# willake/cpu-ray-tracer

Hardware: AMD Instinct MI355X
Metric: Mrays/sec (primary+secondary), 1280x720 64spp path trace — pipelined throughput over 878 consecutive 64-spp windows of one progressive render (single_render = one such render alone) (higher is better)
Workload: dtype f32; 1 GPU; bunny_scene.xml FileScene BVH-SAH path tracer, 1280x720, 64 spp/step (passes=1, depthLimit=5); 1 step = 64 frames = the next spp window of a progressive render; the 878 steps are one crt_render job (14 render kernel launch(es), a wavefront per (tile, 128 consecutive frames), + ordered accumulate), one sync at the end; triangles=4968, parallelism=tile-wave x1

## Files before the change

### cpu-ray-tracer_amd/csrc/abi.cpp

```cpp
#include "../../include/crt_abi.h"
#include "device/launch.h"
#include "device/tile_class.h"
#include "host/grid_resolution.h"

#include <cmath>
#include <cstdarg>
#include <cstddef>
#include <cstdio>
#include <cstdlib>
#include <cstring>
#include <deque>
#include <string>
#include <algorithm>
#include <vector>
#include <chrono>

static_assert(sizeof(crt_bvh_node) == 32 && sizeof(crt_tri) == 112 && sizeof(crt_tlas_node) == 32, "reference layouts");
static_assert(sizeof(crt::NodePair) == 64 && sizeof(crt::LeafTri) == 48 && sizeof(crt::ShadeTri) == 64 && sizeof(crt::TlasNode) == 32 &&
              sizeof(crt::Instance) == 128 && sizeof(crt::Material) == 32 && offsetof(crt::Instance, T) == 64, "device layouts");
static_assert(sizeof(crt_counters) == sizeof(crt::Counters), "counter layout");
static_assert(sizeof(crt_kd_node) == 48 && sizeof(crt::KdNode) == sizeof(crt_kd_node) && sizeof(crt::AltTri) == 48, "flat KD node (uploaded as it comes), alternative accelerators' triangle record");
static_assert(offsetof(crt::PrimDev, red) == 536 && sizeof(crt::PrimDev) == 552, "PrimDev: 134 floats, then the two texel pointers");
static_assert(sizeof(crt::BlasAltDesc) == 72, "BLAS descriptor");
static_assert(sizeof(crt_shadow_ray) == 28 && sizeof(crt_ray) == 28 && sizeof(crt_hit) == 28, "query records");
// ... 887 lines not shown
    c->orderReady = c->orderCopied[k];
    return 0;
}

static uint32_t sky_to_tail(const std::vector<uint8_t>& cls, std::vector<uint32_t>& order)
{
    if (cls.size() != order.size()) return 0u;
    const auto tail = std::stable_partition(order.begin(), order.end(), [&](uint32_t i) { return cls[i] != crt::kTileSky; });
    return (uint32_t)(order.end() - tail);
}

static int update_tile_order(crt_ctx* c)
{
    if (!c->orderDirty || c->tileCount == 0) return 0;
    const crt::Scene& s = c->hScene;
    double R[3], Dn[3], N[3];
    for (int k = 0; k < 3; k++) { R[k] = (double)s.topRight[k] - s.topLeft[k]; Dn[k] = (double)s.bottomLeft[k] - s.topLeft[k]; }
    N[0] = R[1] * Dn[2] - R[2] * Dn[1]; N[1] = R[2] * Dn[0] - R[0] * Dn[2]; N[2] = R[0] * Dn[1] - R[1] * Dn[0];
    const double rr = R[0] * R[0] + R[1] * R[1] + R[2] * R[2], dd = Dn[0] * Dn[0] + Dn[1] * Dn[1] + Dn[2] * Dn[2];
    double E[3]; for (int k = 0; k < 3; k++) E[k] = (double)s.topLeft[k] - s.camPos[k];
    const double num = E[0] * N[0] + E[1] * N[1] + E[2] * N[2];
    auto rect_of = [&](const float* P8, int r[4]) -> bool {
        double u0 = 1e30, u1 = -1e30, v0 = 1e30, v1 = -1e30;
        for (int i = 0; i < 8; i++) {
            const float* P = P8 + 3 * i;
            double d[3] = {P[0] - s.camPos[0], P[1] - s.camPos[1], P[2] - s.camPos[2]};
            const double den = d[0] * N[0] + d[1] * N[1] + d[2] * N[2];
            const double t = den != 0 ? num / den : -1;
            if (!(t > 0) || rr == 0 || dd == 0) return false;
            double Q[3]; for (int k = 0; k < 3; k++) Q[k] = s.camPos[k] + t * d[k] - s.topLeft[k];
            const double u = (Q[0] * R[0] + Q[1] * R[1] + Q[2] * R[2]) / rr, v = (Q[0] * Dn[0] + Q[1] * Dn[1] + Q[2] * Dn[2]) / dd;
            if (u < u0) u0 = u; if (u > u1) u1 = u; if (v < v0) v0 = v; if (v > v1) v1 = v;
        }
        r[0] = (int)floor(u0 * c->cfg.width / 16.0) - 1; r[1] = (int)floor(u1 * c->cfg.width / 16.0) + 1;
        r[2] = (int)floor(v0 * c->cfg.height / 16.0) - 1; r[3] = (int)floor(v1 * c->cfg.height / 16.0) + 1;
        return true;
    };
    float world[24];
    for (int i = 0; i < 8; i++) { world[3 * i] = (i & 1) ? c->meshHi[0] : c->meshLo[0]; world[3 * i + 1] = (i & 2) ? c->meshHi[1] : c->meshLo[1]; world[3 * i + 2] = (i & 4) ? c->meshHi[2] : c->meshLo[2]; }
    int wr[4] = {0, c->tilesX - 1, 0, c->tilesY - 1};
    (void)rect_of(world, wr);
    std::vector<uint32_t> first, second, rest;
    for (uint32_t i = 0; i < c->tileCount; i++) {
        const uint32_t tile = c->tileFirst + i * c->tileStride;
        const int tx = (int)(tile % (uint32_t)c->tilesX), ty = (int)(tile / (uint32_t)c->tilesX);
        const bool inRect = tx >= wr[0] && tx <= wr[1] && ty >= wr[2] && ty <= wr[3];
        if (inRect) first.push_back(i); else rest.push_back(i);
    }
    for (int k = 0; k <= crt_ctx::kLatStages; k++) { c->tuneCount[k] = 0; c->tuneMs[k] = 0; }
    c->latStage = 0; c->latBest = 0; c->latDone = false; c->latWarm = false; c->latConfirming = false; c->latQueue.clear(); c->costPending = false; c->latProbed = false;
    first.insert(first.end(), rest.begin(), rest.end());
    (void)sky_to_tail(c->hostClass, first);
    c->jobCostValid = false; c->jobCostPending = false; c->planValid = false; c->skyWindowTicks = 0;
    { const int r = upload_tile_order(c, first); if (r) return r; }
    c->orderDirty = false;
    return 0;
}

static int update_tile_class(crt_ctx* c)
{
    if (!c->classDirty || c->tileCount == 0) return 0;
    if (!c->dTileClass) HIPCK(c, hipMalloc((void**)&c->dTileClass, (size_t)c->tileCount));
    { const int r = order_behind_ahead(c); if (r) return r; }
    const int k = c->classFlip ^= 1;
    if (!c->hTileClass[k]) {
        HIPCK(c, hipHostMalloc((void**)&c->hTileClass[k], (size_t)c->tileCount, hipHostMallocDefault));
        HIPCK(c, ensure_event(&c->classCopied[k]));
    } else HIPCK(c, hipEventSynchronize(c->classCopied[k]));
    crt::classify_tiles(c->hScene, c->cfg.width, c->cfg.height, (uint32_t)c->tilesX, c->tileFirst, c->tileStride, c->tileCount, c->hTileClass[k]);
    {
        const uint8_t* cls = c->hTileClass[k];
        bool same = c->hostClass.size() == c->tileCount; uint32_t sky = 0;
        for (uint32_t i = 0; i < c->tileCount; i++) { const bool s = cls[i] == crt::kTileSky; sky += s ? 1u : 0u; if (same && s != (c->hostClass[i] == crt::kTileSky)) same = false; }
        c->hostClass.assign(cls, cls + c->tileCount); c->skyTiles = sky;
        if (!same) c->orderDirty = true;
    }
    HIPCK(c, hipMemcpyAsync(c->dTileClass, c->hTileClass[k], (size_t)c->tileCount, hipMemcpyHostToDevice, c->stream));
    HIPCK(c, hipEventRecord(c->classCopied[k], c->stream));
    c->orderReady = c->classCopied[k];
    c->classDirty = false;
    return 0;
}

static size_t sample_bytes_per_window(const crt_ctx* c, uint32_t passes) { return (size_t)c->tileCount * 256u * 64u * passes * 16u; }
static size_t window_bytes(const crt_ctx* c, uint32_t passes) { return sample_bytes_per_window(c, passes) + (c->usePool ? crt_pool_scratch_bytes_per_window(c->tileCount) : 0); }

static uint32_t block_desc(uint32_t tile, uint32_t laneBase, uint32_t lanes, uint32_t window) { uint32_t lg = 0; while ((1u << lg) < lanes) lg++; return tile | (laneBase << 16) | (lg << 22) | (window << 25); }
static const uint32_t kLatLanes[7] = {64u, 32u, 16u, 8u, 4u, 2u, 1u};
static const double kLatG[7] = {1.0, 0.93, 0.88, 0.79, 0.69, 0.57, 0.48};
static int lat_index(uint32_t L) { int k = 0; while (k < 6 && kLatLanes[k] != L) k++; return k; }

static uint8_t next_lanes(uint8_t lanes, uint32_t cost, double T)
{
    int k = lat_index(lanes); const double unit = (double)cost / kLatG[k];
    while (k < 6 && unit * kLatG[k] > T) k++;
    while (k > 0 && unit * kLatG[k - 1] <= 0.9 * T) k--;
    return (uint8_t)kLatLanes[k];
}
extern "C" int crt_debug_next_lanes(const uint8_t* lanes, const uint32_t* cost, uint32_t n, double T, uint8_t* out)
{
    if (!lanes || !cost || !out) return CRT_ERR_INVALID;
    for (uint32_t i = 0; i < n; i++) { if (lanes[i] == 0 || lanes[i] > 64 || (64 % lanes[i]) != 0) return CRT_ERR_INVALID; out[i] = next_lanes(lanes[i], cost[i], T); }
    return CRT_OK;
}

static double solve_block_table(const std::vector<uint8_t>& lanes, const std::vector<uint32_t>& cost, double budget, std::vector<uint8_t>& out)
{
    const size_t n = cost.size();
    double topUnit = 0; for (size_t i = 0; i < n; i++) topUnit = std::max(topUnit, (double)cost[i] / kLatG[lat_index(lanes[i])]);
    out.assign(n, 64);
    if (topUnit <= 0) return 0;
    auto waves = [&](double T) { double w = 0; for (size_t i = 0; i < n; i++) w += 64.0 / next_lanes(lanes[i], cost[i], T); return w; };
    double lo = kLatG[6] * topUnit, hi = topUnit;
    if (waves(lo) > budget) { for (int it = 0; it < 14; it++) { const double mid = 0.5 * (lo + hi); if (waves(mid) <= budget) hi = mid; else lo = mid; } lo = hi; }
    for (size_t i = 0; i < n; i++) out[i] = next_lanes(lanes[i], cost[i], lo);
    return lo;
}
extern "C" int crt_debug_solve_block_table(const uint8_t* lanes, const uint32_t* cost, uint32_t n, double budget, uint8_t* out, double* T)
{
    if (!lanes || !cost || !out) return CRT_ERR_INVALID;
    for (uint32_t i = 0; i < n; i++) if (lanes[i] == 0 || lanes[i] > 64 || (64 % lanes[i]) != 0) return CRT_ERR_INVALID;
    std::vector<uint8_t> L; const double t = solve_block_table(std::vector<uint8_t>(lanes, lanes + n), std::vector<uint32_t>(cost, cost + n), budget, L);
    if (n) memcpy(out, L.data(), n);
    if (T) *T = t;
    return CRT_OK;
}
static double lat_budget(crt_ctx* c)
{
    if (!c->latSlots) c->latSlots = crt_render_resident_waves(c->cfg.device, c->hScene.kind, c->ldsBytes);
    double share = 0.98;
    if (const char* e = hook("CRT_LAT_BUDGET")) { const double v = atof(e); if (v > 0) share = v; }
    return share * (double)c->latSlots;
}

static int upload_block_table(crt_ctx* c, const std::vector<uint8_t>& lanes, const std::vector<uint32_t>& cost)
{
    const uint32_t n = c->tileCount;
    std::vector<uint32_t> order(n);
    for (uint32_t i = 0; i < n; i++) order[i] = i;
    std::stable_sort(order.begin(), order.end(), [&](uint32_t a, uint32_t b) { return cost[a] > cost[b]; });
    std::vector<uint32_t> table; table.reserve((size_t)n * 2);
    for (uint32_t r = 0; r < n; r++) {
        const uint32_t tl = order[r], L = lanes[tl];
        for (uint32_t base = 0; base < 64u; base += L) table.push_back(block_desc(tl, base, L, 0u));
    }
    if (table.size() > 0x7fffffffull) return c->fail(CRT_ERR_INVALID, "block table too large");
    if (hook("CRT_LAT_VERBOSE")) fprintf(stderr, "[crt] latency table: %zu wavefronts for %u tiles (slowest tile of the base stage %.2f ms)\n", table.size(), n, n ? cost[order[0]] * 1e-5 : 0.0);
    if (c->descCap < table.size()) {
        if (c->dBlockDesc) (void)hipFree(c->dBlockDesc);
        if (c->hBlockDesc) (void)hipHostFree(c->hBlockDesc);
        c->dBlockDesc = nullptr; c->hBlockDesc = nullptr; c->descCap = 0;
        const size_t cap = table.size() + table.size() / 2;
        HIPCK(c, hipMalloc((void**)&c->dBlockDesc, cap * 4));
        HIPCK(c, hipHostMalloc((void**)&c->hBlockDesc, cap * 4, hipHostMallocDefault));
        c->descCap = (uint32_t)cap;
    } else if (c->descReady) HIPCK(c, hipEventSynchronize(c->descReady));
    HIPCK(c, ensure_event(&c->descReady));
    memcpy(c->hBlockDesc, table.data(), table.size() * 4);
    { const int r = order_behind_ahead(c); if (r) return r; }
    HIPCK(c, hipMemcpyAsync(c->dBlockDesc, c->hBlockDesc, table.size() * 4, hipMemcpyHostToDevice, c->stream));
    HIPCK(c, hipEventRecord(c->descReady, c->stream));
    c->nBlocks = (uint32_t)table.size();
    return 0;
}

static int next_block_table(crt_ctx* c)
{
// ... 338 lines not shown
static PoolWavePlan plan_pool_waves(const crt_ctx* c, uint32_t windows, uint32_t frames, uint32_t head, uint32_t nSky, double skyTicks, std::vector<uint32_t>& table)
{
    PoolWavePlan p;
    PoolWaveTerms terms;
    const uint32_t S = crt_pool_streams(frames);
    if (!c->jobCostValid || c->cfg.collectStats || head + nSky >= c->tileCount || !pool_wave_terms(terms) || forced_wave_frames(S)) return p;
    const uint32_t nr = c->tileCount - nSky - head;
    p.ranks = nr;
    std::vector<uint32_t> cost(nr), wf, tab;
    double costSum = 0; for (uint32_t v : c->jobCost) costSum += (double)v;
    const double perCost = (c->poolWindowTicks > 0 && costSum > 0) ? c->poolWindowTicks / costSum : 1.0 / 4096.0;
    double startTicks = 0;
    if (sky_behind()) { terms.tailTicks = skyTicks; terms.tailWaves = (double)nSky * (double)((frames + S - 1u) / S); } else startTicks = skyTicks;
    for (uint32_t r = 0; r < head; r++) startTicks += (double)windows * 1.2 * (double)c->jobCost[c->jobOrder[r]] * perCost;
    for (uint32_t r = 0; r < nr; r++) cost[r] = c->jobCost[c->jobOrder[head + r]];
    uint32_t F1 = 0, lw = 0, blocks = 0;
    pool_wave_plan(cost.data(), nr, frames, S, perCost, startTicks, 4096u, terms, wf, &F1, nullptr, &p.aim);
    if (F1) blocks = pool_wave_table(wf, F1, S, tab, &lw);
    if (lw) {
        for (uint32_t r = 0; r < nSky; r++) { tab.push_back(blocks); tab.push_back(S); }
        p.off = (uint32_t)table.size(); p.blocks = blocks; p.longFrames = F1; p.longWaves = lw;
        table.insert(table.end(), tab.begin(), tab.end());
    }
    if (hook("CRT_LAT_VERBOSE")) {
        uint32_t cnt[4] = {0, 0, 0, 0}; double share[4] = {0, 0, 0, 0}, sum = 0;
        for (uint32_t r = 0; r < nr; r++) { int k = 0; while ((S << k) < wf[r]) k++; cnt[k]++; share[k] += cost[r]; sum += cost[r]; }
        fprintf(stderr, "[crt] pool launch of %u ranks x %u frames (%u sky ranks behind them: %.2f ms): aim %.1f ms, most expensive tile %.2f ms, long part %u frames in %u wavefronts, %u of them own more than %u frames (safety %.2f, guard %.1f x 4096, share %.2f); tiles by frames per wavefront (share of the cost):",
                nr, frames, nSky, skyTicks * 1e-5, p.aim * 1e-5, nr ? cost[0] * 1e-5 : 0.0, F1, blocks, lw, S, terms.safety, terms.guard, terms.share);
        for (int k = 0; k < 4; k++) fprintf(stderr, " %u: %u (%.3f)", S << k, cnt[k], sum > 0 ? share[k] / sum : 0.0);
        fprintf(stderr, "\n");
    }
    return p;
}

static double sky_launch_ticks(const crt_ctx* c, uint32_t windows, uint32_t nSky)
{
    return (nSky && c->jobCostValid) ? c->skyWindowTicks * (double)windows : 0.0;
}

static int install_job_plan(crt_ctx* c, uint32_t windows, uint32_t frames, bool pool)
{
    const uint32_t asked = sky_split(c, pool);
    if (c->planValid && c->planWindows == windows && c->planFrames == frames && c->planPool == pool && c->planSkyAsked == asked) return 0;
    uint32_t nSky = asked;
    double skyTicks = sky_launch_ticks(c, windows, nSky);
    std::vector<uint32_t> table; uint32_t head = 0;
    plan_job(c, windows, frames, pool, table, &head, nSky, skyTicks);
    if (head && nSky) {
        nSky = 0; skyTicks = 0;
        plan_job(c, windows, frames, pool, table, &head);
    }
    c->planValid = true; c->planWindows = windows; c->planFrames = frames; c->planPool = pool; c->planSkyAsked = asked; c->planSky = nSky; c->jobHead = head; c->jobBlocks = (uint32_t)table.size();
    c->jobTrialMs[0] = c->jobTrialMs[1] = 0;
    c->jobWaveOff = c->jobWaveBlocks = c->jobLongFrames = c->jobLongWaves = 0;
    if (pool) {
        const PoolWavePlan p = plan_pool_waves(c, windows, frames, head, nSky, skyTicks, table);
        c->jobWaveOff = p.off; c->jobWaveBlocks = p.blocks; c->jobLongFrames = p.longFrames; c->jobLongWaves = p.longWaves;
    }
    if (table.empty()) return 0;
    if (c->jobDescCap < table.size()) {
        if (c->dJobDesc) (void)hipFree(c->dJobDesc);
        if (c->hJobDesc) (void)hipHostFree(c->hJobDesc);
        c->dJobDesc = nullptr; c->hJobDesc = nullptr; c->jobDescCap = 0;
        const size_t cap = table.size() + table.size() / 2;
        HIPCK(c, hipMalloc((void**)&c->dJobDesc, cap * 4));
        HIPCK(c, hipHostMalloc((void**)&c->hJobDesc, cap * 4, hipHostMallocDefault));
        c->jobDescCap = (uint32_t)cap;
    } else if (c->jobDescReady) HIPCK(c, hipEventSynchronize(c->jobDescReady));
    HIPCK(c, ensure_event(&c->jobDescReady));
    memcpy(c->hJobDesc, table.data(), table.size() * 4);
    { const int r = order_behind_ahead(c); if (r) return r; }
    HIPCK(c, hipMemcpyAsync(c->dJobDesc, c->hJobDesc, table.size() * 4, hipMemcpyHostToDevice, c->stream));
    HIPCK(c, hipEventRecord(c->jobDescReady, c->stream));
    return 0;
}

struct Launch {
    hipStream_t st = nullptr; EventPair ev{}; void* slab = nullptr; uint32_t sppFirst = 0, nf = 0, passes = 1, windows = 1;
    const uint32_t* blockDesc = nullptr; uint32_t nBlocks = 0;
    bool wantCost = false, wantJobCost = false, pool = false;
    uint32_t head = 0, jobBlocks = 0; unsigned long long* jobClk = nullptr;
    uint32_t waveFrames = 0, waveBlocks = 0, longFrames = 0, longWaves = 0; const uint32_t* waveTab = nullptr;
    uint32_t sky = 0;
};

static int next_block_table(crt_ctx* c);
static int probe_tile_costs(crt_ctx* c, hipStream_t st);

static int tuner_prepare(crt_ctx* c, Launch& L)
{
    int r;
    const bool gpuIdle = !c->lastRenderEnd || hipEventQuery(c->lastRenderEnd) == hipSuccess;
    if (L.nf <= 64u && L.nf >= 8u && gpuIdle && !c->cfg.collectStats && c->tileCount <= 0x10000u && !hook("CRT_LAT_OFF")) {
        if (c->costPending && hipEventQuery(c->costCopied) == hipSuccess) { c->costPending = false; harvest_tuning(c); if ((r = next_block_table(c))) return r; }
        if (c->latStage == 0 && !c->latProbed && !c->latWarm && !c->costPending && L.nf == 64u && !hook("CRT_LAT_POLICY") && !hook("CRT_LAT_NO_PROBE")) { if ((r = probe_tile_costs(c, L.st))) return r; }
        const int stage = c->latStage;
        if (stage || c->latProbed) { L.blockDesc = c->dBlockDesc; L.nBlocks = c->nBlocks; HIPCK(c, hipStreamWaitEvent(L.st, c->descReady, 0)); }
        L.wantCost = (!c->latDone && !c->costPending) || (c->latDone && hook("CRT_LAT_RECORD"));
        c->evRender.back().mode = c->latDone ? -1 : stage;
        if (L.wantCost && !c->latDone) c->costStage = stage;
    }
    if (L.wantCost) {
        if (!c->dTileCost) {
            HIPCK(c, hipMalloc((void**)&c->dTileCost, (size_t)c->tileCount * 4));
            HIPCK(c, hipHostMalloc((void**)&c->hTileCost, (size_t)c->tileCount * 4, hipHostMallocDefault));
            HIPCK(c, ensure_event(&c->costCopied));
        }
        else HIPCK(c, hipStreamWaitEvent(L.st, c->costCopied, 0));
        HIPCK(c, hipMemsetAsync(c->dTileCost, 0, (size_t)c->tileCount * 4, L.st));
    }
    return 0;
}

static int planner_prepare(crt_ctx* c, Launch& L)
{
    int r;
    if (L.nf > 64u && !c->cfg.collectStats) {
        if (c->jobCostPending && hipEventQuery(c->jobCostCopied) == hipSuccess) { c->jobCostPending = false; if ((r = adopt_job_costs(c))) return r; HIPCK(c, hipStreamWaitEvent(L.st, c->orderReady, 0)); }
        L.wantJobCost = !c->jobCostValid && !c->jobCostPending && L.nf >= 128u;
        if (L.wantJobCost) {
            if (!c->dJobCost) {
                HIPCK(c, hipMalloc((void**)&c->dJobCost, job_cost_bytes(c)));
                HIPCK(c, hipHostMalloc((void**)&c->hJobCost, job_cost_bytes(c), hipHostMallocDefault));
                HIPCK(c, ensure_event(&c->jobCostCopied));
            } else HIPCK(c, hipStreamWaitEvent(L.st, c->jobCostCopied, 0));
            HIPCK(c, hipMemsetAsync(c->dJobCost, 0, job_cost_bytes(c), L.st));
        }
    }
    const bool poolByDefault = c->hScene.poolRefBits == 16u || c->poolMinWaves == 0;
    const uint64_t minWaves = c->poolMinWaves != 65000u ? c->poolMinWaves : (c->jobCostValid ? 43000u : 65000u);
    L.pool = c->usePool && poolByDefault && pool_can_run(c, L.nf) && (uint64_t)c->tileCount * L.windows >= minWaves && (c->poolMinWaves == 0 || L.nf > 64u);
    L.sky = sky_split(c, L.pool);
    if (L.nf > 64u && c->jobCostValid) {
        if ((r = install_job_plan(c, L.windows, L.nf, L.pool))) return r;
        int use = 1;
        if ((c->jobBlocks || c->jobLongWaves) && !hook("CRT_PLAN_NO_TRIAL")) {
            if (c->jobTrialMs[1] > 0 && c->jobTrialMs[0] > 0) use = c->jobTrialMs[1] <= c->jobTrialMs[0] ? 1 : 0;
            else if (c->jobTrialMs[1] > 0 && c->jobTrialMs[0] == 0) use = 0;
            c->evRender.back().mode = 100 + use;
        }
        if (use) L.sky = c->planSky;
        if (use) { L.head = c->jobHead; L.jobBlocks = c->jobBlocks; if (L.pool && c->jobLongWaves) { L.waveTab = c->dJobDesc + c->jobWaveOff; L.waveBlocks = c->jobWaveBlocks; L.longFrames = c->jobLongFrames; L.longWaves = c->jobLongWaves; } }
    }
    if (L.pool) if (const uint32_t S = crt_pool_streams(L.nf); const uint32_t n = forced_wave_frames(S)) {
        L.waveFrames = n; L.waveTab = nullptr; L.waveBlocks = 0;
        L.longWaves = n > S ? (c->tileCount - L.sky - L.head) * (L.nf / n + ((L.nf % n) > S ? 1u : 0u)) : 0u;
    }
    if (L.jobBlocks || L.waveTab) HIPCK(c, hipStreamWaitEvent(L.st, c->jobDescReady, 0));
    if (L.wantJobCost) {
        L.jobClk = reinterpret_cast<unsigned long long*>(reinterpret_cast<char*>(c->dJobCost) + job_cost_clk_offset(c));
        c->recPool = L.pool; c->recWindows = L.windows;
        const uint32_t perWave = L.pool ? std::max(crt_pool_streams(L.nf), L.waveFrames) : 64u;
        c->recWaves = L.pool ? (c->tileCount - L.sky) * ((L.nf + perWave - 1u) / perWave) : c->tileCount * L.windows;
        c->recResident = L.pool ? 4096u : 5120u;
        if (L.pool && c->hScene.poolRefBits == 32u)
            c->recResident = 256u * std::min(16u, (160u * 1024u) / std::max(1u, pool_lds_need(c, L.nf)));
    }
    return 0;
}

static hipError_t launch_render_kernels(crt_ctx* c, const Launch& L)
{
    hipStream_t st = L.st;
    hipError_t le = hipSuccess;
    auto join = [&](hipStream_t other) -> hipError_t {
        if (other == st) return hipSuccess;
        hipError_t e = hipSuccess;
        if (c->splitEvents.size() < 32) { hipEvent_t ne; e = hipEventCreateWithFlags(&ne, hipEventDisableTiming); if (e == hipSuccess) c->splitEvents.push_back(ne); }
        if (e == hipSuccess) { hipEvent_t je = c->splitEvents[c->splitSeq++ % c->splitEvents.size()]; e = hipEventRecord(je, other); if (e == hipSuccess) e = hipStreamWaitEvent(st, je, 0); }
        return e;
    };
    auto launch_table = [&](const uint32_t* desc, uint32_t nBlocks, uint32_t* cost) -> hipError_t {
        return crt_launch_render(&c->hScene, L.slab, c->dCounters, c->dTileClocks, c->dTileOrder, c->tileFirst, c->tileStride, c->tileCount, (uint32_t)c->tilesX,
                                 L.sppFirst, L.nf, L.passes, c->ldsBytes, 0, desc, nBlocks, cost, 0u, nullptr, st);
    };
    if (L.pool) {
        void* scratch = (char*)L.slab + (size_t)L.windows * sample_bytes_per_window(c, L.passes);
        hipStream_t st2 = st;
        const bool skyBehind = sky_behind();
        auto launch_sky = [&](hipStream_t s) -> hipError_t {
            return crt_launch_render_sky(&c->hScene, L.slab, c->dCounters, c->dTileOrder, c->tileCount - L.sky, L.sky, c->tileFirst, c->tileStride, c->tileCount, (uint32_t)c->tilesX,
                                         L.sppFirst, L.nf, L.passes, L.jobClk ? L.jobClk + 3 : nullptr, s);
        };
        if (L.sky && !skyBehind) { le = launch_sky(st); if (le == hipSuccess) c->skyLaunches++; }
        if (le != hipSuccess) return le;
        if (L.jobBlocks) {
            le = launch_table(c->dJobDesc, L.jobBlocks, nullptr);
            st2 = c->streams[(size_t)(c->launchSeq++ % c->streams.size())];
            if (le == hipSuccess && st2 != st) le = hipStreamWaitEvent(st2, L.ev.a, 0);
        }
        if (le == hipSuccess)
            le = crt_launch_render_pool(&c->hScene, L.slab, scratch, c->dCounters, c->dTileClocks, c->dTileOrder, c->tileFirst, c->tileStride, c->tileCount, (uint32_t)c->tilesX,
                                        L.sppFirst, L.nf, L.passes, c->cfg.collectStats, L.jobBlocks ? L.head : 0u, c->tileCount - L.sky, L.waveFrames, L.waveTab, L.waveBlocks, L.longFrames,
                                        L.wantJobCost ? c->dJobCost : nullptr, L.jobClk,
                                        (c->classDirty || hook("CRT_DEBUG_NO_TILE_CLASS")) ? nullptr : c->dTileClass , c->extraLds, st2);
        if (le == hipSuccess) c->lastLongWaves = L.longWaves;
        if (L.jobBlocks && le == hipSuccess) le = join(st2);
        if (L.sky && skyBehind && le == hipSuccess) {
            if (!c->skyStream && !hook("CRT_SKY_PRIORITY")) {
                int least = 0, greatest = 0;
                le = hipDeviceGetStreamPriorityRange(&least, &greatest);
                if (le == hipSuccess) le = hipStreamCreateWithPriority(&c->skyStream, hipStreamNonBlocking, least);
                if (le != hipSuccess) return le;
            }
            hipStream_t st3 = c->skyStream;
            if (hook("CRT_SKY_PRIORITY")) { st3 = c->streams[(size_t)(c->launchSeq++ % c->streams.size())]; if (st3 == st2 && c->streams.size() > 1) st3 = c->streams[(size_t)(c->launchSeq++ % c->streams.size())]; }
            if (st3 != st) le = hipStreamWaitEvent(st3, L.ev.a, 0);
            if (le == hipSuccess) le = launch_sky(st3);
            if (le == hipSuccess) { c->skyLaunches++; le = join(st3); }
        }
    } else if (L.jobBlocks) {
        le = launch_table(c->dJobDesc, L.jobBlocks, nullptr);
    } else if (L.blockDesc && L.nBlocks) {
        le = launch_table(L.blockDesc, L.nBlocks, L.wantCost ? c->dTileCost : nullptr);
    } else {
        le = crt_launch_render(&c->hScene, L.slab, c->dCounters, c->dTileClocks, c->dTileOrder, c->tileFirst, c->tileStride, c->tileCount, (uint32_t)c->tilesX,
                               L.sppFirst, L.nf, L.passes, c->ldsBytes, c->cfg.collectStats, nullptr, 0u,
                               L.wantCost ? c->dTileCost : (L.wantJobCost ? c->dJobCost : nullptr), 0u, L.jobClk, st);
    }
    if (L.jobBlocks && le == hipSuccess) c->splitLaunches++;
    return le;
}

static int probe_tile_costs(crt_ctx* c, hipStream_t st)
{
    const uint32_t n = c->tileCount;
    if (!c->dTileCost) {
        HIPCK(c, hipMalloc((void**)&c->dTileCost, (size_t)n * 4));
        HIPCK(c, hipHostMalloc((void**)&c->hTileCost, (size_t)n * 4, hipHostMallocDefault));
        HIPCK(c, ensure_event(&c->costCopied));
    } else HIPCK(c, hipEventSynchronize(c->costCopied));
    const auto tp0 = std::chrono::steady_clock::now();
    HIPCK(c, crt_launch_probe(&c->hScene, c->tileFirst, c->tileStride, n, (uint32_t)c->tilesX, c->dTileCost, st));
    HIPCK(c, hipMemcpyAsync(c->hTileCost, c->dTileCost, (size_t)n * 4, hipMemcpyDeviceToHost, st));
    HIPCK(c, hipEventRecord(c->costCopied, st));
    HIPCK(c, hipStreamSynchronize(st));
    const auto tp1 = std::chrono::steady_clock::now();
    std::vector<uint32_t>& est = c->latCost[0]; est.assign(c->hTileCost, c->hTileCost + n);
    for (uint32_t i = 0; i < n; i++) est[i] += 18u * crt_probe_paths();
    std::vector<uint8_t>& L = c->latL[0]; L.assign(n, 64);
    solve_block_table(std::vector<uint8_t>(n, 64), est, lat_budget(c), L);
    c->latProbed = true;
    bool any = false; for (uint32_t i = 0; i < n; i++) any = any || L[i] != 64;
    if (!any) { c->latProbed = false; return 0; }
    const auto tp2 = std::chrono::steady_clock::now();
    const int r = upload_block_table(c, L, est);
    if (hook("CRT_LAT_VERBOSE")) { const auto tp3 = std::chrono::steady_clock::now(); auto ms = [](auto a, auto b) { return std::chrono::duration<double, std::milli>(b - a).count(); };
        fprintf(stderr, "[crt] cost probe: launch + wait %.3f ms, table solved in %.3f ms, uploaded in %.3f ms\n", ms(tp0, tp1), ms(tp1, tp2), ms(tp2, tp3)); }
    return r;
}

static int launch_frames(crt_ctx* c, uint32_t sppFirst, uint32_t nf, uint32_t passes, hipStream_t st, crt_ctx::Ahead* ahead)
{
    const size_t windowBytes = window_bytes(c, passes);
    size_t off = 0; int r;
    if ((r = take_region(c, (size_t)((nf + 63u) / 64u) * windowBytes, st, &off))) return r;
    if (c->orderReady) HIPCK(c, hipStreamWaitEvent(st, c->orderReady, 0));
    if ((r = wait_scene(c, st))) return r;
    void* slab = c->pool + off;
    EventPair ev;
    harvest_tuning(c);
    fold_completed(c, c->evRender, &c->foldedRenderMs, &c->foldedLaunches); fold_completed(c, c->evAcc, &c->foldedAccMs, nullptr);
    if ((r = take_event(c, c->evRender, &ev))) return r;
    struct PairGuard { crt_ctx* c; bool armed; ~PairGuard() { if (armed && !c->evRender.empty()) { c->evPool.push_back(c->evRender.back()); c->evRender.pop_back(); } } } pairGuard{c, true};
    Launch L; L.st = st; L.ev = ev; L.slab = slab; L.sppFirst = sppFirst; L.nf = nf; L.passes = passes; L.windows = (nf + 63u) / 64u;
    if ((r = tuner_prepare(c, L))) return r;
    if ((r = planner_prepare(c, L))) return r;
    HIPCK(c, hipEventRecord(ev.a, st));
    const bool pool = L.pool, wantCost = L.wantCost, wantJobCost = L.wantJobCost;
    const hipError_t le = hook("CRT_DEBUG_FAIL_LAUNCH") ? hipErrorInvalidConfiguration  : launch_render_kernels(c, L);
    if (le != hipSuccess) {
        return c->hip(le, pool ? "launch of render_pool_kernel" : "launch of render_tiles_kernel");
    }
    if (pool && L.sky < c->tileCount) c->poolLaunches++;
    HIPCK(c, hipEventRecord(ev.b, st));
    pairGuard.armed = false;
    c->lastRenderEnd = ev.b;
    if (wantJobCost) {
        HIPCK(c, hipMemcpyAsync(c->hJobCost, c->dJobCost, job_cost_bytes(c), hipMemcpyDeviceToHost, st));
        HIPCK(c, hipEventRecord(c->jobCostCopied, st));
        c->jobCostPending = true;
    }
    if (wantCost && !pool && !c->latDone) {
        HIPCK(c, hipMemcpyAsync(c->hTileCost, c->dTileCost, (size_t)c->tileCount * 4, hipMemcpyDeviceToHost, st));
        HIPCK(c, hipEventRecord(c->costCopied, st));
        c->costPending = true;
    }
    crt_ctx::Region reg; reg.off = off; reg.bytes = (size_t)((nf + 63u) / 64u) * windowBytes;
    if (c->freeEvents.empty()) HIPCK(c, hipEventCreateWithFlags(&reg.freed, hipEventDisableTiming));
    else { reg.freed = c->freeEvents.back(); c->freeEvents.pop_back(); }
    if (ahead) {
        hipEvent_t end = nullptr;
        if (c->doneEvents.empty()) { const hipError_t e = hipEventCreateWithFlags(&end, hipEventDisableTiming); if (e != hipSuccess) { c->freeEvents.push_back(reg.freed); return c->hip(e, "hipEventCreate"); } }
        else { end = c->doneEvents.back(); c->doneEvents.pop_back(); }
        const hipError_t e = hipEventRecord(end, st);
        if (e != hipSuccess) { c->doneEvents.push_back(end); c->freeEvents.push_back(reg.freed); return c->hip(e, "hipEventRecord"); }
        reg.held = true;
        c->inflight.push_back(reg);
        *ahead = crt_ctx::Ahead{end, off, (const char*)slab, c->epoch, sppFirst, nf, passes, 0u};
        return 0;
    }
    HIPCK(c, hipStreamWaitEvent(c->stream, ev.b, 0));
    if ((r = take_event(c, c->evAcc, &ev))) return r;
    HIPCK(c, hipEventRecord(ev.a, c->stream));
    HIPCK(c, crt_launch_accumulate(slab, c->dAcc, c->tileFirst, c->tileStride, c->tileCount, (uint32_t)c->tilesX, (uint32_t)c->cfg.width, nf, passes, c->stream));
    HIPCK(c, hipEventRecord(ev.b, c->stream));
    HIPCK(c, hipEventRecord(reg.freed, c->stream));
    c->inflight.push_back(reg);
    return 0;
}

int crt_render(crt_ctx* c, uint32_t spp_first, uint32_t frames, uint32_t passes)
{
    if (!c) return CRT_ERR_INVALID;
    if (!c->haveScene && !c->havePrim) return c->fail(CRT_ERR_STATE, "crt_render before crt_upload_scene");
    if (passes < 1 || passes > 4) return c->fail(CRT_ERR_INVALID, "passes must be 1..4 (the reference's UI range, renderer.cpp:178)");
    HIPCK(c, hipSetDevice(c->cfg.device));
    { int r = discard_ahead(c); if (r) return r; }
    if (c->tileCount == 0 || frames == 0) return CRT_OK;
    { int r = update_tile_class(c); if (r) return r; }
    { int r = update_tile_order(c); if (r) return r; }
    if (c->streams.empty()) {
        int n = c->cfg.renderStreams;
        if (n <= 0) n = 7;
        if (n > 16) n = 16;
        if (c->cfg.collectStats) n = 1;
        c->streams.resize((size_t)n);
        for (auto& st : c->streams) HIPCK(c, hipStreamCreateWithFlags(&st, hipStreamNonBlocking));
    }
    uint32_t maxF = 0;
    { int r = ensure_pool(c, frames, passes, &maxF); if (r) return r; }
    const size_t windowBytes = window_bytes(c, passes);
    if (c->renderAccel != 0 || c->havePrim) {
        for (uint32_t f0 = 0; f0 < frames; f0 += maxF) {
            const uint32_t nf = (frames - f0 < maxF) ? frames - f0 : maxF;
            size_t off = 0; int r;
            if ((r = take_region(c, (size_t)((nf + 63u) / 64u) * windowBytes, c->stream, &off))) return r;
            if ((r = wait_scene(c, c->stream))) return r;
            void* slab = c->pool + off;
            if (c->havePrim) HIPCK(c, crt_launch_render_prim(&c->hScene, &c->prim, slab, c->dCounters, c->tileFirst, c->tileStride, c->tileCount, (uint32_t)c->tilesX, spp_first + f0 * passes, nf, passes, c->stream));
            else HIPCK(c, crt_launch_render_alt(c->renderAccel, &c->hScene, &c->alt, &c->blasAlt[c->renderAccel - 1], slab, c->dCounters, c->tileFirst, c->tileStride, c->tileCount, (uint32_t)c->tilesX, spp_first + f0 * passes, nf, passes, c->stream));
            HIPCK(c, crt_launch_accumulate(slab, c->dAcc, c->tileFirst, c->tileStride, c->tileCount, (uint32_t)c->tilesX, (uint32_t)c->cfg.width, nf, passes, c->stream));
            crt_ctx::Region reg; reg.off = off; reg.bytes = (size_t)((nf + 63u) / 64u) * windowBytes;
            if (c->freeEvents.empty()) HIPCK(c, hipEventCreateWithFlags(&reg.freed, hipEventDisableTiming));
            else { reg.freed = c->freeEvents.back(); c->freeEvents.pop_back(); }
            HIPCK(c, hipEventRecord(reg.freed, c->stream));
            c->inflight.push_back(reg);
        }
        return CRT_OK;
    }
    for (uint32_t f0 = 0; f0 < frames; f0 += maxF) {
        const uint32_t nf = (frames - f0 < maxF) ? frames - f0 : maxF;
        const int r = launch_frames(c, spp_first + f0 * passes, nf, passes, c->streams[(size_t)(c->launchSeq++ % c->streams.size())], nullptr);
        if (r) return r > 0 ? c->fail(CRT_ERR_DEVICE, "slab ring blocked by a render-ahead region") : r;
    }
    return CRT_OK;
}

int crt_sync(crt_ctx* c)
{
    if (!c) return CRT_ERR_INVALID;
    HIPCK(c, hipSetDevice(c->cfg.device));
    HIPCK(c, hipStreamSynchronize(c->stream));
    for (auto st : c->streams) HIPCK(c, hipStreamSynchronize(st));
    if (c->aheadStream) HIPCK(c, hipStreamSynchronize(c->aheadStream));
    return CRT_OK;
}

int crt_clear(crt_ctx* c)
{
    if (!c) return CRT_ERR_INVALID;
    HIPCK(c, hipSetDevice(c->cfg.device));
    HIPCK(c, hipMemsetAsync(c->dAcc, 0, (size_t)c->cfg.width * c->cfg.height * 16, c->stream));
    return CRT_OK;
}

int crt_read_accumulator(crt_ctx* c, float* host)
{
    if (!c || !host) return CRT_ERR_INVALID;
    HIPCK(c, hipSetDevice(c->cfg.device));
    HIPCK(c, hipMemcpyAsync(host, c->dAcc, (size_t)c->cfg.width * c->cfg.height * 16, hipMemcpyDeviceToHost, c->stream));
    HIPCK(c, hipStreamSynchronize(c->stream));
    return CRT_OK;
}

static int read_screen(crt_ctx* c, uint32_t* hostPixels, float* energy)
{
    const int tiles = c->tilesX * c->tilesY;
    if (hostPixels) HIPCK(c, hipMemcpyAsync(hostPixels, c->dPixels, (size_t)c->cfg.width * c->cfg.height * 4, hipMemcpyDeviceToHost, c->stream));
    std::vector<float> sums(tiles);
    HIPCK(c, hipMemcpyAsync(sums.data(), c->dTileSums, (size_t)tiles * 4, hipMemcpyDeviceToHost, c->stream));
    HIPCK(c, hipStreamSynchronize(c->stream));
    if (energy) { float e = 0; for (int i = 0; i < tiles; i++) e += sums[i]; *energy = e; }
    return CRT_OK;
}

int crt_resolve_screen(crt_ctx* c, float scale, uint32_t* hostPixels, float* energy)
{
    if (!c) return CRT_ERR_INVALID;
    HIPCK(c, hipSetDevice(c->cfg.device));
    HIPCK(c, crt_launch_resolve(c->dAcc, c->dPixels, c->dTileSums, c->tileFirst, c->tileStride, c->tileCount, (uint32_t)c->tilesX, (uint32_t)c->cfg.width, scale, c->stream));
    return read_screen(c, hostPixels, energy);
}

static constexpr uint32_t kAheadMaxFrames = 256;

static int launch_ahead(crt_ctx* c, uint32_t sppFirst, uint32_t passes)
{
    if (!c->aheadStream) {
        int least = 0, greatest = 0;
        HIPCK(c, hipDeviceGetStreamPriorityRange(&least, &greatest));
        HIPCK(c, hipStreamCreateWithPriority(&c->aheadStream, hipStreamNonBlocking, least));
    }
    uint32_t nf = c->aheadFrames ? std::min(2u * c->aheadFrames, kAheadMaxFrames) : 64u;
    if (nf > (uint32_t)c->cfg.maxFramesPerLaunch) nf = (uint32_t)c->cfg.maxFramesPerLaunch;
    const uint32_t poolW = (uint32_t)(c->poolBytes / window_bytes(c, passes));
    if (nf > poolW / 2u * 64u) nf = poolW / 2u * 64u;
    if (nf == 0 || c->streams.empty()) return 0;
    hipStream_t st = hook("CRT_AHEAD_NORMAL_PRIORITY") ? c->streams[(size_t)(c->launchSeq++ % c->streams.size())] : c->aheadStream;
    crt_ctx::Ahead a{};
    const int r = launch_frames(c, sppFirst, nf, passes, st, &a);
    if (r < 0) return r;
    if (r > 0) return 0;
    c->ahead.push_back(a); c->aheadFrames = nf;
    return 0;
// ... 1088 lines not shown
    return CRT_OK;
}

static int device_probe(crt_ctx* c, int op, const void* in, void* out, uint32_t n)
{
    static const uint8_t words[18][2] = {{1, 1}, {1, 1}, {2, 1}, {1, 1}, {2, 1}, {6, 7}, {1, 18}, {4, 1}, {5, 3}, {13, 2}, {16, 4}, {2, 2}, {2, 2}, {2, 2}, {2, 2}, {4, 2}, {2, 1}, {5, 3}};
    if (!c || !in || !out || op < 0 || op > 17 || n > (1u << 25)) return CRT_ERR_INVALID;
    if (n == 0) return CRT_OK;
    const size_t inBytes = (size_t)n * words[op][0] * 4, outBytes = (size_t)n * words[op][1] * 4;
    HIPCK(c, hipSetDevice(c->cfg.device));
    char* d = nullptr;
    HIPCK(c, hipMalloc((void**)&d, inBytes + outBytes));
    hipError_t e = hipMemcpyAsync(d, in, inBytes, hipMemcpyHostToDevice, c->stream);
    if (e == hipSuccess) e = (op <= 10 || op == 17) ? crt_launch_probe_f32(op, d, d + inBytes, n, c->stream) : crt_launch_probe_f64(op, d, d + inBytes, n, c->stream);
    if (e == hipSuccess) e = hipMemcpyAsync(out, d + inBytes, outBytes, hipMemcpyDeviceToHost, c->stream);
    if (e == hipSuccess) e = hipStreamSynchronize(c->stream);
    (void)hipFree(d);
    HIPCK(c, e);
    return CRT_OK;
}
extern "C" int crt_debug_device_probe(crt_ctx* c, int op, const void* in, void* out, uint32_t n) { return (op > 16) ? CRT_ERR_INVALID : device_probe(c, op, in, out, n); }
extern "C" int crt_debug_sky_probe(crt_ctx* c, const void* in, void* out, uint32_t n) { return device_probe(c, 17, in, out, n); }

extern "C" int crt_debug_plan_job(const uint32_t* cost, uint32_t n, uint32_t windows, uint32_t frames, int pool, double poolWindowTicks,
                                  uint32_t* table, uint32_t tableCap, uint32_t* head, uint32_t* order)
{
    if (!cost || !n || !table || !head || !order) return CRT_ERR_INVALID;
    crt_ctx c;
    c.tileCount = n; c.jobCostValid = true; c.poolWindowTicks = poolWindowTicks;
    c.streams.assign(2, nullptr);
    c.jobCost.assign(cost, cost + n);
    c.jobOrder.resize(n);
    for (uint32_t i = 0; i < n; i++) c.jobOrder[i] = i;
    std::stable_sort(c.jobOrder.begin(), c.jobOrder.end(), [&](uint32_t a, uint32_t b) { return c.jobCost[a] > c.jobCost[b]; });
    std::vector<uint32_t> t; uint32_t h = 0;
    plan_job(&c, windows, frames, pool != 0, t, &h);
    c.streams.clear();
    if (t.size() > tableCap) return CRT_ERR_INVALID;
    memcpy(table, t.data(), t.size() * 4); memcpy(order, c.jobOrder.data(), (size_t)n * 4); *head = h;
    return (int)t.size();
}

extern "C" long long crt_debug_pool_wave_plan(const uint32_t* cost, uint32_t nr, uint32_t frames, double perCost, double startTicks, uint32_t resident, double safety, double guard,
                                              double share, uint32_t* wf, uint32_t* longFrames, double* start, double* aim)
{
    if (!nr || !frames || !wf || !longFrames) return CRT_ERR_INVALID;
    PoolWaveTerms tm; if (safety > 0) tm.safety = safety; if (guard > 0) tm.guard = guard; if (share > 0) tm.share = share;
    std::vector<uint32_t> w; std::vector<double> st;
    const uint64_t waves = pool_wave_plan(cost, nr, frames, crt_pool_streams(frames), perCost, startTicks, resident, tm, w, longFrames, &st, aim);
    memcpy(wf, w.data(), (size_t)nr * 4);
    if (start) memcpy(start, st.data(), (size_t)nr * 8);
    return (long long)waves;
}
extern "C" int crt_debug_sky_split(const uint32_t* cost, const uint8_t* cls, uint32_t n, uint32_t windows, uint32_t frames, double poolWindowTicks, double skyWindowTicks,
                                   uint32_t* order, uint32_t* skyFirst, uint32_t* head, uint32_t* planRanks, uint32_t* waveTab, uint32_t* tabBlocks, uint32_t* longFrames)
{
    if (!cls || !n || !order || !skyFirst || !head || !planRanks || !waveTab || !tabBlocks || !longFrames) return CRT_ERR_INVALID;
    crt_ctx c;
    c.tileCount = n; c.poolWindowTicks = poolWindowTicks; c.skyWindowTicks = skyWindowTicks;
    c.hostClass.assign(cls, cls + n);
    *head = *planRanks = *tabBlocks = *longFrames = 0;
    if (!cost) {
        c.jobOrder.resize(n); for (uint32_t i = 0; i < n; i++) c.jobOrder[i] = i;
        c.skyTiles = sky_to_tail(c.hostClass, c.jobOrder);
    } else {
        c.jobCost.assign(cost, cost + n); c.jobCostValid = true;
        c.skyTiles = job_order(c.jobCost, c.hostClass, c.jobOrder);
        c.streams.assign(2, nullptr);
        const double skyTicks = c.skyTiles ? skyWindowTicks * (double)windows : 0.0;
        std::vector<uint32_t> table;
        plan_job(&c, windows, frames, true, table, head, c.skyTiles, skyTicks);
        table.clear();
        const PoolWavePlan p = plan_pool_waves(&c, windows, frames, *head, c.skyTiles, skyTicks, table);
        c.streams.clear();
        *planRanks = p.ranks; *tabBlocks = p.blocks; *longFrames = p.longFrames;
        if (table.size() > 2u * (size_t)n) return CRT_ERR_INVALID;
        memcpy(waveTab, table.data(), table.size() * 4);
    }
    memcpy(order, c.jobOrder.data(), (size_t)n * 4);
    *skyFirst = n - c.skyTiles;
    return (int)c.skyTiles;
}
extern "C" int crt_debug_sky_launches(crt_ctx* c) { return c ? (int)c->skyLaunches : -1; }
extern "C" int crt_debug_job_costs(crt_ctx* c, uint32_t* out, double* poolWindowTicks, double* skyWindowTicks)
{
    if (!c || !out) return CRT_ERR_INVALID;
    if (!c->jobCostValid || c->jobCost.size() != c->tileCount) return CRT_ERR_STATE;
    memcpy(out, c->jobCost.data(), (size_t)c->tileCount * 4);
    if (poolWindowTicks) *poolWindowTicks = c->poolWindowTicks;
    if (skyWindowTicks) *skyWindowTicks = c->skyWindowTicks;
    return CRT_OK;
}
extern "C" int crt_debug_pool_long_waves(crt_ctx* c) { return c ? (int)c->lastLongWaves : -1; }
extern "C" void crt_debug_pool_wave_terms(double* out) { const PoolWaveTerms tm; out[0] = tm.poolLong; out[1] = tm.load; out[2] = tm.safety; out[3] = tm.guard; out[4] = tm.share; }

extern "C" int crt_debug_tile_costs(crt_ctx* c, uint32_t* out)
{
    if (!c || !out || !c->dTileCost) return CRT_ERR_INVALID;
    HIPCK(c, hipSetDevice(c->cfg.device));
    HIPCK(c, hipDeviceSynchronize());
    HIPCK(c, hipMemcpy(out, c->dTileCost, (size_t)c->tileCount * 4, hipMemcpyDeviceToHost));
    return CRT_OK;
}

extern "C" int crt_debug_lat_stage(crt_ctx* c, int stage, uint8_t* lanes, uint32_t* cost)
{
    if (!c || stage < 0 || stage > crt_ctx::kLatStages) return CRT_ERR_INVALID;
    if (c->latL[stage].size() != c->tileCount || c->latCost[stage].size() != c->tileCount) return CRT_ERR_STATE;
    if (lanes) memcpy(lanes, c->latL[stage].data(), c->tileCount);
    if (cost) memcpy(cost, c->latCost[stage].data(), (size_t)c->tileCount * 4);
    return c->latStage;
}

extern "C" int crt_debug_tile_stamps(crt_ctx* c, uint64_t* out)
{
    if (!c || !out || !c->dTileClocks) return CRT_ERR_INVALID;
    HIPCK(c, hipSetDevice(c->cfg.device));
    HIPCK(c, hipMemcpyAsync(out, c->dTileClocks + 2 * (size_t)c->tileCount, (size_t)c->tileCount * 128, hipMemcpyDeviceToHost, c->stream));
    HIPCK(c, hipStreamSynchronize(c->stream));
    return CRT_OK;
}

int crt_bind_accumulator(crt_ctx* c, void* p)
{
    if (!c) return CRT_ERR_INVALID;
    if (p && ((uintptr_t)p & 15u)) return c->fail(CRT_ERR_INVALID, "accumulator pointer must be 16-byte aligned");
    HIPCK(c, hipSetDevice(c->cfg.device));
    HIPCK(c, hipStreamSynchronize(c->stream));
    c->dAcc = p ? p : c->dAccOwned;
    return CRT_OK;
}

int crt_accumulator_device_ptr(crt_ctx* c, void** p)
{
    if (!c || !p) return CRT_ERR_INVALID;
    *p = c->dAcc; return CRT_OK;
}

}
```

### cpu-ray-tracer_amd/csrc/device/kernels.hip

```cpp
#include "alt_common.h"
#include "launch.h"
#include "sample_body.h"

namespace crt {

#ifndef CRT_SHADE_BATCH
#define CRT_SHADE_BATCH 24
#endif
#ifndef CRT_SHADE_BATCH_JOB
#define CRT_SHADE_BATCH_JOB 40
#endif
#ifndef CRT_TRI_BATCH
#define CRT_TRI_BATCH 1
#endif
#ifndef CRT_NODE_BATCH
#define CRT_NODE_BATCH 1
#endif

#ifndef CRT_TILES_NODE_STEPS
#define CRT_TILES_NODE_STEPS 2
#endif
#ifndef CRT_MIN_WAVES
#define CRT_MIN_WAVES 5
#endif
template <int KIND, bool COUNT>
__global__ __launch_bounds__(64, CRT_MIN_WAVES) void render_tiles_kernel(const Scene sc, float4* __restrict__ slab,
                                                           Counters* __restrict__ counters, unsigned long long* __restrict__ tileClocks,
                                                           const uint32_t* __restrict__ tileOrder,
                                                           uint32_t tileFirst, uint32_t tileStride, uint32_t tileCount, uint32_t tilesX,
                                                           uint32_t sppFirst, uint32_t frames, uint32_t passes, uint32_t windows,
                                                           const uint32_t* __restrict__ blockDesc, uint32_t* __restrict__ tileCost, uint32_t rankCount, unsigned long long* __restrict__ launchClk)
{
    extern __shared__ uint32_t lds[];
    const uint32_t lane = threadIdx.x;
    const unsigned long long clk0 = (COUNT || tileCost) ? wall_clock64() : 0ull;
    if (launchClk && lane == 0) { atomicMax(&launchClk[0], ~clk0); atomicMax(&launchClk[1], clk0); }
    uint32_t rank, win = 0u, laneBase = 0u, myLanes = 64u;
    if (blockDesc) { const uint32_t d = blockDesc[blockIdx.x]; rank = d & 0xffffu; laneBase = (d >> 16) & 63u; myLanes = 1u << ((d >> 22) & 7u); win = d >> 25; }
    else { rank = blockIdx.x / windows; win = blockIdx.x - rank * windows; }
    if (rank >= (blockDesc ? tileCount : rankCount)) return;
    const uint32_t tl = blockDesc ? rank : (tileOrder ? tileOrder[rank] : rank);
    sppFirst += win * 64u * passes;
    frames = (frames - win * 64u < 64u) ? frames - win * 64u : 64u;
    if (blockDesc) frames = frames > laneBase ? ((frames - laneBase < myLanes) ? frames - laneBase : myLanes) : 0u;
    slab += (size_t)win * ((size_t)tileCount * 256u * 64u * passes);
    const uint32_t tile = tileFirst + tl * tileStride;
    const uint32_t tx = tile % tilesX, ty = tile / tilesX;
    uint32_t* stk = lds + lane;
    const char* __restrict__ geom = sc.geom;

    Cnt cn; cn.rays = cn.primary = cn.interior = cn.leaf = cn.tri = cn.tlas = cn.visits = cn.meshhits = 0;
    uint32_t trips = 0;
    const bool narrowWave = myLanes < 64u;
    const int shadeBatch = narrowWave ? (int)((myLanes * 3u + 7u) / 8u) : (windows >= 8u ? CRT_SHADE_BATCH_JOB : CRT_SHADE_BATCH);
#ifdef CRT_STAMPS
    unsigned long long stT[6] = {0, 0, 0, 0, 0, 0}; uint32_t stN[4] = {0, 0, 0, 0}; uint32_t stL[4] = {0, 0, 0, 0};
#define CRT_STAMP(var) unsigned long long var; asm volatile("s_memtime %0\n\ts_waitcnt lgkmcnt(0)" : "=s"(var) :: "memory")
#else
#define CRT_STAMP(var)
#endif
    const uint32_t items = 256u * passes;
    const f3 nil3 = mk3(0.0f, 0.0f, 0.0f);

    bool live = lane < frames;
    uint64_t liveMask = __builtin_amdgcn_ballot_w64(live);
    uint32_t seed = init_seed(tx + ty * (uint32_t)sc.W + (sppFirst + (laneBase + lane) * passes) * 1799u);
    uint32_t item = 0;
    f3 O = nil3, D = nil3, rD = nil3; bool inside = false; int depth = 0;
    Hit h; h.t = 1e34f; h.u = 0; h.v = 0; h.objIdx = -1; h.triIdx = -1;
    float* fst = reinterpret_cast<float*>(lds + sc.stackDepth * 64u + lane);
    uint32_t cur = kRefDone, sp = 0;
    f3 tO = nil3, tD = nil3, trD = nil3;
    bool rayFinite = true;
    bool fresh = true;
    rec4 q0 = {0, 0, 0, 0}, q1 = q0, q2 = q0, q3 = q0;

#define CRT_TOP() (stk[(sp ? sp - 1u : 0u) * 64u])
    auto record_offsets = [&](bool shade, uint32_t& oa, uint32_t& ob) {
        oa = shade ? sc.shadeOff + (uint32_t)h.triIdx * 64u : (cur & kRefOffsetMask) << 4; ob = oa + 32u;
        if (KIND == 1 && !shade && (cur & kRefTlasBit) != 0u) {
            if (cur & kRefInterior) { oa = sc.instOff + (cur & 0xffffu) * 128u; ob = oa + 32u; }
            else { oa = sc.tlasOff + (cur & 0x7fffu) * 32u; ob = sc.tlasOff + ((cur >> 15) & 0x7fffu) * 32u; }
        }
    };
    auto leave_blas = [&](uint32_t next) -> uint32_t {
        if (KIND == 1 && next == kRefReturn) {
            tO = O; tD = D; trD = rD; rayFinite = finite3(rD);
            const bool pop = sp != 0u; const uint32_t top = CRT_TOP();
            next = pop ? top : kRefDone; sp -= pop ? 1u : 0u;
        }
        return next;
    };

    for (;;) {
        const uint64_t mDone = __builtin_amdgcn_ballot_w64(cur == kRefDone) & liveMask;
        const uint64_t mNode = __builtin_amdgcn_ballot_w64(KIND == 1 ? (((cur >> 31) ^ (cur >> 30)) & 1u) != 0u : (cur & 0xC0000000u) == kRefInterior) & liveMask;
        const uint64_t mTri = __builtin_amdgcn_ballot_w64(cur != kRefDone && (cur & 0xC0000000u) == 0u) & liveMask;
        const uint64_t mTlas = (KIND == 1) ? (__builtin_amdgcn_ballot_w64((cur & 0xC0000000u) == kRefTlasLeaf) & liveMask) : 0ull;
        const bool isDone = live && cur == kRefDone;
        const bool isNode = live && (KIND == 1 ? (((cur >> 31) ^ (cur >> 30)) & 1u) != 0u : (cur & 0xC0000000u) == kRefInterior);
        const bool isTri = live && cur != kRefDone && (cur & 0xC0000000u) == 0u;
        const bool isTlas = (KIND == 1) && live && (cur & 0xC0000000u) == kRefTlasLeaf;
        const int nDone = __popcll(mDone), nNode = __popcll(mNode), nTri = __popcll(mTri);
        const int nTlas = (KIND == 1) ? __popcll(mTlas) : 0;
        if (nDone + nNode + nTri + nTlas == 0) break;
        if (COUNT) trips++;
        const bool bigNode = nNode >= CRT_NODE_BATCH, bigTri = nTri >= CRT_TRI_BATCH, bigShade = nDone >= shadeBatch;
        const bool none = !bigNode && !bigTri && !bigShade && nTlas == 0;
        const bool runTlas = nTlas > 0;
        const bool runNode = bigNode || (none && nNode > 0 && nNode >= nTri && nNode >= nDone);
        const bool runTri = bigTri || (none && nTri > 0 && nTri > nNode && nTri >= nDone);
        const bool runShade = bigShade || (none && nDone > 0 && nDone > nNode && nDone > nTri);
        asm volatile("" : "+v"(q0), "+v"(q1), "+v"(q2), "+v"(q3));
#ifdef CRT_STAMPS
        CRT_STAMP(s0);
        asm volatile("s_waitcnt vmcnt(0)" ::: "memory");
        CRT_STAMP(s1);
        stT[0] += s1 - s0;
        if (runShade) { stN[0]++; stL[0] += nDone; } if (runNode) { stN[1]++; stL[1] += nNode; } if (runTri) { stN[2]++; stL[2] += nTri; }
        stN[3]++;
#endif

        if (runShade && isDone) {
            const kernarg_f cam = scene_floats(offsetof(Scene, camPos));
            const f3 camPos = mk3(cam[0], cam[1], cam[2]);
            const bool first = fresh;
            const bool miss = !first && h.objIdx == -1;
            const bool stop = !first && h.objIdx != -1 && (depth >= sc.depthLimit || h.objIdx == 0);
            const bool surf = !first && !miss && !stop;
            if (!first && h.objIdx >= 2) cn.meshhits++;
            const kernarg_f sk = scene_floats(offsetof(Scene, skyOffset));
            float tu = 0, tv = 0; uint32_t tOff = asu(sk[0]); int tW = (int)asu(sk[1]), tH = (int)asu(sk[2]);
            f3 I = O, N = O, absorb = O; float refl = 0, refr = 0;
            if (miss) {
                const float phi = crt_atan2f(-D.z, D.x) + CRT_PI, theta = crt_acosf(-D.y);
                tu = phi * CRT_INV2PI; tv = theta * CRT_INVPI;
            }
            if (surf) {
                I = O + h.t * D;
                SurfPoint p;
                if (h.objIdx == 1) {
                    const kernarg_f fl = scene_floats(offsetof(Scene, floorN));
                    const kernarg_f fm = scene_floats(offsetof(Scene, floorMat));
                    const rec4 m0 = {fm[0], fm[1], fm[2], fm[3]}, m1 = {fm[4], fm[5], fm[6], fm[7]};
                    p = floor_point(mk3(fl[0], fl[1], fl[2]), fl[4], m0, m1, I);
                } else p = mesh_point<KIND>(q0, q1, q2, q3, h.u, h.v, h.objIdx, geom, sc.instOff, sc.mats);
                N = face_ray(p.N, D);
                tu = p.tu; tv = p.tv; refl = p.refl; refr = p.refr; absorb = p.absorb; tOff = p.tOff; tW = p.tW; tH = p.tH;
            }
            f3 c = mk3(1.0f, 1.0f, 1.0f);
            if (miss || (surf && tW > 0)) c = tex_sample(sc, tOff, tW, tH, tu, tv);
            f3 v = O, medium = O; bool norm = false, newInside = false; Branch branch = kMirror;
            if (surf) {
                medium = medium_of(inside, absorb, h.t);
                const Bounce b = draw_bounce(seed, D, N, inside, refl, refr);
                v = b.v; branch = b.branch; newInside = b.newInside; norm = b.branch == kDiffuse;
            }
            bool gen = first;
            if (miss || stop) {
                f3 L = miss ? c : ((depth >= sc.depthLimit) ? mk3(0, 0, 0) : mk3(24, 24, 22));
                sample_unwind(fst, depth, L);
                uint32_t pix = item, pass = 0;
                if (passes != 1u) { pix = item / passes; pass = item - pix * passes; }
                slab[((size_t)tl * 256u + pix) * (64u * passes) + ((laneBase + lane) * passes + pass)] = make_float4(L.x, L.y, L.z, 0.0f);
                item++;
                gen = true;
                if (item >= items) { live = false; gen = false; }
            }
            if (gen) {
                const uint32_t pix = (passes == 1u) ? item : item / passes;
                const f3 TL = mk3(cam[3], cam[4], cam[5]), TR = mk3(cam[6], cam[7], cam[8]), BL = mk3(cam[9], cam[10], cam[11]);
                v = primary_target(camPos, TL, TR - TL, BL - TL, cam[12], cam[13], tx, ty, pix, seed); norm = true;
                inside = false; depth = 0; fresh = false;
                cn.primary++;
            }
            if (live) {
                const float inv = rcp_exact(sqrt_exact(dot3(v, v)));
                const f3 nv = norm ? v * inv : v;
                if (surf) {
                    const f3 factor = bounce_factor(branch, c, medium, nv, N);
                    float* fd = fst + depth * 192;
                    fd[0] = factor.x; fd[64] = factor.y; fd[128] = factor.z;
                    depth++;
                    O = I + nv * CRT_EPS; inside = newInside;
                } else O = camPos;
                D = nv; rD = rcp_exact3(nv);
                cn.rays++;
                h.t = 1e34f; h.u = 0; h.v = 0; h.objIdx = -1; h.triIdx = -1;
                hit_light_floor(light_floor_from_kernarg<false>(), O, D, h);
                tO = O; tD = D; trD = rD; rayFinite = finite3(rD);
                sp = 0;
                if (sc.rootIsPair) {
                    const kernarg_f rp = scene_floats(offsetof(Scene, rootPair));
                    const rec4 a0 = {rp[0], rp[1], rp[2], rp[3]}, a1 = {rp[4], rp[5], rp[6], rp[7]};
                    const rec4 b0 = {rp[8], rp[9], rp[10], rp[11]}, b1 = {rp[12], rp[13], rp[14], rp[15]};
                    float d1, d2;
                    if (__builtin_amdgcn_ballot_w64(!rayFinite) == 0ull) { d1 = box_fast(a0, a1, O, rD, h.t); d2 = box_fast(b0, b1, O, rD, h.t); }
                    else { d1 = box_exact(a0, a1, O, rD, h.t); d2 = box_exact(b0, b1, O, rD, h.t); }
                    const Ordered o = ordered_step(d1, d2, asu(a0.w), asu(b0.w));
                    stk[0] = o.farRef;
                    sp = o.push ? 1u : 0u;
                    cur = o.hitN ? o.nearRef : kRefDone;
                    if (COUNT) { if (KIND == 0) cn.interior++; else cn.tlas++; }
                } else cur = sc.rootRef;
                if (COUNT && KIND == 0 && (cur & 0xC0000000u) == 0u && cur != kRefDone) cn.leaf++;
            }
        }
        if (runShade) liveMask = __builtin_amdgcn_ballot_w64(live);
#ifdef CRT_STAMPS
        CRT_STAMP(s2); stT[1] += s2 - s1;
#endif
        if (KIND == 1 && runTlas && isTlas) {
            if (COUNT) { cn.tlas++; cn.visits++; }
            to_object_space(q0, q1, q2, O, D, tO, tD, trD);
            rayFinite = finite3(trD);
            stk[sp * 64u] = kRefReturn; sp++;
            const uint32_t next = asu(q3.z);
            if (COUNT && (next & 0xC0000000u) == 0u && next != kRefDone) cn.leaf++;
            cur = next;
        }
#ifdef CRT_STAMPS
        CRT_STAMP(s3);
#endif
        if (runNode) {
            const bool allFinite = __builtin_amdgcn_ballot_w64(isNode && !rayFinite) == 0ull;
            if (isNode) {
                if (COUNT) { if (KIND == 1 && (cur & kRefTlasBit) != 0u) cn.tlas++; else cn.interior++; }
                uint32_t top = CRT_TOP();
                float d1, d2;
                if (allFinite) { d1 = box_fast(q0, q1, tO, trD, h.t); d2 = box_fast(q2, q3, tO, trD, h.t); }
                else { d1 = box_exact(q0, q1, tO, trD, h.t); d2 = box_exact(q2, q3, tO, trD, h.t); }
                const Ordered o = ordered_step(d1, d2, asu(q0.w), asu(q2.w));
                stk[sp * 64u] = o.farRef;
                bool pop = !o.hitN && sp != 0u;
                uint32_t next = o.hitN ? o.nearRef : (pop ? top : kRefDone);
                sp = sp + (o.push ? 1u : 0u) - (pop ? 1u : 0u);
                next = leave_blas(next);
                if (COUNT && (next & 0xC0000000u) == 0u && next != kRefDone) cn.leaf++;
                cur = next;
            }
        }
        bool triNow = isTri;
#if CRT_TILES_NODE_STEPS > 1
        if (runNode) {
            const bool node2 = isNode && (KIND == 1 ? (((cur >> 31) ^ (cur >> 30)) & 1u) != 0u : (cur & 0xC0000000u) == kRefInterior);
            const bool leaf2 = isNode && cur != kRefDone && (cur & 0xC0000000u) == 0u;
            const uint64_t mNode2 = __builtin_amdgcn_ballot_w64(node2);
            if (mNode2 != 0ull) {
                if (node2 || leaf2) {
                    uint32_t oa, ob; record_offsets(false, oa, ob);
                    q0 = ldg(geom, oa); q1 = ldg(geom, oa + 16u); q2 = ldg(geom, ob); q3 = ldg(geom, ob + 16u);
                }
                triNow = isTri || leaf2;
                const bool allFinite2 = __builtin_amdgcn_ballot_w64(node2 && !rayFinite) == 0ull;
                if (node2) {
                    if (COUNT) { if (KIND == 1 && (cur & kRefTlasBit) != 0u) cn.tlas++; else cn.interior++; }
                    uint32_t top = CRT_TOP();
                    float d1, d2;
                    if (allFinite2) { d1 = box_fast(q0, q1, tO, trD, h.t); d2 = box_fast(q2, q3, tO, trD, h.t); }
                    else { d1 = box_exact(q0, q1, tO, trD, h.t); d2 = box_exact(q2, q3, tO, trD, h.t); }
                    const Ordered o = ordered_step(d1, d2, asu(q0.w), asu(q2.w));
                    stk[sp * 64u] = o.farRef;
                    bool pop = !o.hitN && sp != 0u;
                    uint32_t next = o.hitN ? o.nearRef : (pop ? top : kRefDone);
                    sp = sp + (o.push ? 1u : 0u) - (pop ? 1u : 0u);
                    next = leave_blas(next);
                    if (COUNT && (next & 0xC0000000u) == 0u && next != kRefDone) cn.leaf++;
                    cur = next;
                }
            }
        }
#endif
#ifdef CRT_STAMPS
        CRT_STAMP(s4); stT[2] += s4 - s3;
#endif
        if ((runTri || triNow != isTri) && triNow) {
            if (COUNT) cn.tri++;
            uint32_t top = CRT_TOP();
            hit_tri(q0, q1, q2, tO, tD, h);
            const bool more = asu(q2.w) > 1u;
            bool pop = !more && sp != 0u;
            uint32_t next = more ? cur + 3u : (pop ? top : kRefDone);
            sp -= pop ? 1u : 0u;
            next = leave_blas(next);
            if (COUNT && !more && (next & 0xC0000000u) == 0u && next != kRefDone) cn.leaf++;
            cur = next;
        }
#ifdef CRT_STAMPS
        CRT_STAMP(s5); stT[3] += s5 - s4;
#endif
        {
            const bool doneNow = cur == kRefDone;
            uint32_t oa, ob; record_offsets(doneNow, oa, ob);
            const bool nothing = !live || (doneNow && h.objIdx < 2);
            if (nothing) { oa = 0u; ob = 32u; }
            if (__builtin_amdgcn_ballot_w64(!nothing) != 0ull) { q0 = ldg(geom, oa); q1 = ldg(geom, oa + 16u); q2 = ldg(geom, ob); q3 = ldg(geom, ob + 16u); }
        }
#ifdef CRT_STAMPS
        CRT_STAMP(s6); stT[4] += s6 - s5; stT[5] += s6 - s0;
#endif
    }
#undef CRT_TOP

    if (tileCost && lane == 0) atomicMax(&tileCost[tl], (uint32_t)(wall_clock64() - clk0));
    if (launchClk && lane == 0) { const unsigned long long now = wall_clock64(), last = __hip_atomic_load(&launchClk[1], __ATOMIC_RELAXED, __HIP_MEMORY_SCOPE_AGENT), from = last > clk0 ? last : clk0; if (now > from) atomicAdd(&launchClk[2], now - from); }
    if (COUNT && tileClocks && lane == 0 && windows == 1u) {
        tileClocks[2 * tl] = wall_clock64() - clk0;
        tileClocks[2 * tl + 1] = trips;
#ifdef CRT_STAMPS
        unsigned long long* dbg = tileClocks + 2 * (size_t)tileCount + 16 * (size_t)tl;
        for (int i = 0; i < 6; i++) dbg[i] = stT[i];
        for (int i = 0; i < 4; i++) dbg[6 + i] = stN[i];
        for (int i = 0; i < 4; i++) dbg[10 + i] = stL[i];
#endif
    }
    uint32_t vals[8] = {cn.rays, cn.primary, cn.interior, cn.leaf, cn.tri, cn.tlas, cn.visits, cn.meshhits};
#pragma unroll
    for (int i = 0; i < 8; i++) {
        if (!COUNT && i >= 2 && i != 7) continue;
        uint32_t s = wave_sum(vals[i]);
        if (lane == 0 && s) atomicAdd(&counters->v[i], (unsigned long long)s);
    }
}

constexpr uint32_t kAccRowF4 = 65u;
constexpr uint32_t kAccWaveLds = 16u * kAccRowF4 * 16u;
__global__ __launch_bounds__(256) void accumulate_kernel(const float4* __restrict__ slab, float* __restrict__ acc,
                                                          uint32_t tileFirst, uint32_t tileStride, uint32_t tileCount, uint32_t tilesX,
                                                          uint32_t W, uint32_t frames, uint32_t passes)
{
    extern __shared__ float4 accLds[];
    const uint32_t tl = blockIdx.x, lane = threadIdx.x & 63u, wave = threadIdx.x >> 6;
    if (tl >= tileCount) return;
    const uint32_t tile = tileFirst + tl * tileStride;
    const uint32_t x0 = (tile % tilesX) * 16u, y0 = (tile / tilesX) * 16u;
    const uint32_t rowLen = 64u * passes;
    const size_t winStride = (size_t)tileCount * 256u * rowLen;
    float4* my4 = accLds + wave * (16u * kAccRowF4);
    const float* myF = reinterpret_cast<const float*>(my4) + (lane >> 2) * (kAccRowF4 * 4u) + (lane & 3u);
    for (uint32_t r = 0; r < 4u; r++) {
        const uint32_t v = wave * 4u + r;
        float* __restrict__ ap = acc + ((size_t)(x0 + (size_t)(y0 + v) * W)) * 4u + lane;
        float a = *ap;
        const float4* __restrict__ rowBase = slab + ((size_t)tl * 256u + v * 16u) * rowLen;
        for (uint32_t f0 = 0; f0 < frames; f0 += 64u, rowBase += winStride) {
            const uint32_t S = ((frames - f0 < 64u) ? frames - f0 : 64u) * passes;
            for (uint32_t b = 0; b < S; b += 64u) {
                const uint32_t n = (S - b < 64u) ? S - b : 64u;
                float4 t[16];
                if (lane < n) {
#pragma unroll
                    for (int j = 0; j < 16; j++) t[j] = rowBase[(size_t)j * rowLen + b + lane];
#pragma unroll
                    for (int j = 0; j < 16; j++) my4[j * kAccRowF4 + lane] = t[j];
                }
                asm volatile("s_waitcnt lgkmcnt(0)" ::: "memory");
                uint32_t s = 0;
                for (; s + 8u <= n; s += 8u) {
                    float x[8];
#pragma unroll
                    for (int k = 0; k < 8; k++) x[k] = myF[(s + k) * 4u];
#pragma unroll
                    for (int k = 0; k < 8; k++) a += x[k];
                }
                for (; s < n; s++) a += myF[s * 4u];
                asm volatile("s_waitcnt lgkmcnt(0)" ::: "memory");
            }
        }
        *ap = a;
    }
}

struct RayIn { float O[3]; float D[3]; int32_t inside; };
struct HitOut { float t, u, v; int32_t objIdx, triIdx, traversed, tested; };
constexpr uint32_t kQueryRefill = 16u;

__global__ __launch_bounds__(64) void find_nearest_kernel(const Scene sc, const RayIn* __restrict__ rays,
                                                           HitOut* __restrict__ hits, uint32_t n, Counters* __restrict__ counters, uint32_t* __restrict__ cursor)
{
    extern __shared__ uint32_t lds[];
    const uint32_t lane = threadIdx.x;
    const char* __restrict__ g = sc.geom;
    uint32_t* stk = lds + lane;
    uint32_t* tstk = stk + sc.bvhStack * 64;
    Cnt cn; cn.rays = cn.primary = cn.interior = cn.leaf = cn.tri = cn.tlas = cn.visits = cn.meshhits = 0;
    uint32_t mode = 0u;
    uint32_t idx = 0; f3 O = mk3(0, 0, 0), D = O, rD = O, Oo = O, Do = O, rDo = O;
    Hit h; h.t = 1e34f; h.u = 0; h.v = 0; h.objIdx = -1; h.triIdx = -1;
    int traversed = 0, tested = 0;
    uint32_t cur = 0, sp = 0, tcur = 0, tsp = 0, leafAt = 0;
    bool more = true;
    for (;;) {
        const uint64_t mIdle = __builtin_amdgcn_ballot_w64(mode == 0u);
        const uint32_t nIdle = (uint32_t)__popcll(mIdle);
        if (more && nIdle >= kQueryRefill) {
            uint32_t base = 0;
            if (lane == 0) base = atomicAdd(cursor, nIdle);
            base = (uint32_t)__builtin_amdgcn_readfirstlane((int)base);
            more = base + nIdle < n;
            const uint32_t my = base + (uint32_t)__builtin_amdgcn_mbcnt_hi((uint32_t)(mIdle >> 32), __builtin_amdgcn_mbcnt_lo((uint32_t)mIdle, 0u));
            if (mode == 0u && my < n) {
                idx = my;
                const RayIn r = rays[idx];
                O = mk3(r.O[0], r.O[1], r.O[2]); D = mk3(r.D[0], r.D[1], r.D[2]);
                rD = mk3(1 / D.x, 1 / D.y, 1 / D.z);
                h.t = 1e34f; h.u = 0; h.v = 0; h.objIdx = -1; h.triIdx = -1; traversed = 0; tested = 0;
                cn.rays++;
                hit_light_floor(sc, O, D, h);
                if (sc.kind == 0) { Oo = O; Do = D; rDo = rD; cur = sc.rootRef; sp = 0; mode = 1u; }
                else { tcur = sc.rootRef; tsp = 0; mode = 3u; }
            }
        }
        if (__builtin_amdgcn_ballot_w64(mode != 0u) == 0ull) break;
        if (mode == 3u) {
            traversed++; cn.tlas++;
            bool pop = false;
            if ((tcur & kRefTlasLeaf) == kRefTlasLeaf) {
                cn.visits++;
                const uint32_t io = sc.instOff + (tcur & 0xffffu) * 128u;
                const rec4 r0 = ldg(g, io), r1 = ldg(g, io + 16), r2 = ldg(g, io + 32), ids = ldg(g, io + 48);
                to_object_space(r0, r1, r2, O, D, Oo, Do, rDo);
                cur = asu(ids.z); sp = 0; mode = 1u;
            } else {
                const uint32_t o1 = sc.tlasOff + (tcur & 0x7fffu) * 32u, o2 = sc.tlasOff + ((tcur >> 15) & 0x7fffu) * 32u;
                const rec4 alo = ldg(g, o1), ahi = ldg(g, o1 + 16), blo = ldg(g, o2), bhi = ldg(g, o2 + 16);
                float d1 = box_exact(alo, ahi, O, rD, h.t), d2 = box_exact(blo, bhi, O, rD, h.t);
                uint32_t r1 = asu(alo.w), r2 = asu(blo.w);
                if (d1 > d2) { float td = d1; d1 = d2; d2 = td; uint32_t tr = r1; r1 = r2; r2 = tr; }
                if (d1 == 1e30f) pop = true;
                else { tcur = r1; if (d2 != 1e30f) { tstk[tsp * 64] = r2; tsp++; } }
            }
            if (pop) { if (tsp == 0) mode = 4u; else tcur = tstk[(--tsp) * 64]; }
        }
        bool back = false;
        if (mode == 1u) {
            traversed++;
            const uint32_t off = (cur & kRefOffsetMask) << 4;
            if (cur & kRefInterior) {
                cn.interior++;
                const rec4 alo = ldg(g, off), ahi = ldg(g, off + 16), blo = ldg(g, off + 32), bhi = ldg(g, off + 48);
                float d1 = box_exact(alo, ahi, Oo, rDo, h.t), d2 = box_exact(blo, bhi, Oo, rDo, h.t);
                uint32_t r1 = asu(alo.w), r2 = asu(blo.w);
                if (d1 > d2) { float td = d1; d1 = d2; d2 = td; uint32_t tr = r1; r1 = r2; r2 = tr; }
                if (d1 == 1e30f) back = true;
                else { cur = r1; if (d2 != 1e30f) { stk[sp * 64] = r2; sp++; } }
            } else { cn.leaf++; leafAt = off; mode = 2u; }
        }
        if (mode == 2u) {
            const rec4 a = ldg(g, leafAt), b = ldg(g, leafAt + 16), c = ldg(g, leafAt + 32);
            tested++; cn.tri++;
            hit_tri(a, b, c, Oo, Do, h);
            if (asu(c.w) <= 1u) { back = true; mode = 1u; } else leafAt += 48;
// ... 357 lines not shown
            hit_light_floor(sc, O, D, h);
            alt_walk<ACCEL>(sc, alt, O, D, rD, h, stk, traversed, tested);
            if (h.objIdx >= 2) cn.meshhits++;
        }
        travOut[idx] = traversed; testedOut[idx] = tested;
        if (h.objIdx == -1) {
            const f3 res = sky_color(sc, D);
            acc[idx] = make_float4(res.x, res.y, res.z, 0.0f);
            const uint32_t r = (uint32_t)(255.0f * min_std(1.0f, res.x)), g = (uint32_t)(255.0f * min_std(1.0f, res.y)), bb = (uint32_t)(255.0f * min_std(1.0f, res.z));
            pixels[idx] = (r << 16) + (g << 8) + bb;
        } else pixels[idx] = kInspectPending;
    }
    uint32_t vals[8] = {cn.rays, cn.primary, cn.interior, cn.leaf, cn.tri, cn.tlas, cn.visits, cn.meshhits};
#pragma unroll
    for (int k = 0; k < 8; k++) {
        uint32_t s = wave_sum(vals[k]);
        if (lane == 0 && s) atomicAdd(&counters->v[k], (unsigned long long)s);
    }
    inspect_reduce(lane, traversed, tested, sums);
    const int32_t m = wave_max(useTested ? tested : traversed);
    if (lane == 0 && m) atomicMax(&blockMax[idx / kInspectBlock], m);
}

__device__ __forceinline__ f3 traverse_count_color(int32_t traversed, int32_t peak)
{
    const float invMax = 1 / 255.f;
    const f3 green = mk3(179 * invMax, 255 * invMax, 174 * invMax);
    const f3 red = mk3(255 * invMax, 50 * invMax, 50 * invMax);
    if (peak < 10) return green;
    traversed = traversed < 0 ? 0 : (traversed > peak ? peak : traversed);
    const float blend = traversed / (float)peak;
    return mk3(green.x + blend * (red.x - green.x), green.y + blend * (red.y - green.y), green.z + blend * (red.z - green.z));
}

__global__ __launch_bounds__(1024) void inspect_color_kernel(const int32_t* __restrict__ count, const int32_t* __restrict__ blockMax, int32_t peakIn, uint32_t n,
                                                             float4* __restrict__ acc, uint32_t* __restrict__ pixels)
{
    __shared__ int32_t carryPart[16], waveMax[16];
    const uint32_t tid = threadIdx.x, lane = tid & 63u, wave = tid >> 6;
    const uint32_t idx = blockIdx.x * kInspectBlock + tid;
    int32_t c = peakIn;
    for (uint32_t j = tid; j < blockIdx.x; j += kInspectBlock) { const int32_t t = blockMax[j]; c = t > c ? t : c; }
    c = wave_max(c);
    const int32_t own = idx < n ? count[idx] : 0;
    int32_t incl = own;
    for (int o = 1; o < 64; o <<= 1) { const int32_t t = __shfl_up(incl, o, 64); if (lane >= (uint32_t)o && t > incl) incl = t; }
    if (lane == 0) carryPart[wave] = c;
    if (lane == 63) waveMax[wave] = incl;
    __syncthreads();
    int32_t peak = carryPart[0];
#pragma unroll
    for (uint32_t w = 1; w < 16; w++) { const int32_t t = carryPart[w]; peak = t > peak ? t : peak; }
    for (uint32_t w = 0; w < wave; w++) { const int32_t t = waveMax[w]; peak = t > peak ? t : peak; }
    const int32_t before = __shfl_up(incl, 1, 64);
    if (lane > 0 && before > peak) peak = before;
    if (idx < n && pixels[idx] == kInspectPending) {
        const f3 res = traverse_count_color(own, peak);
        acc[idx] = make_float4(res.x, res.y, res.z, 0.0f);
        const uint32_t r = (uint32_t)(255.0f * min_std(1.0f, res.x)), g = (uint32_t)(255.0f * min_std(1.0f, res.y)), bb = (uint32_t)(255.0f * min_std(1.0f, res.z));
        pixels[idx] = (r << 16) + (g << 8) + bb;
    }
}

__global__ __launch_bounds__(64) void resolve_kernel(const float4* __restrict__ acc, uint32_t* __restrict__ pixels, float* __restrict__ tileSums,
                                                      uint32_t tileFirst, uint32_t tileStride, uint32_t tileCount, uint32_t tilesX,
                                                      uint32_t W, float scale)
{
    const uint32_t tl = blockIdx.x * blockDim.x + threadIdx.x;
    if (tl >= tileCount) return;
    const uint32_t tile = tileFirst + tl * tileStride;
    const uint32_t x0 = (tile % tilesX) * 16u, y0 = (tile / tilesX) * 16u;
    float sum = 0;
    for (uint32_t v = 0; v < 16; v++) for (uint32_t u = 0; u < 16; u++) {
        const size_t i = (x0 + u) + (size_t)(y0 + v) * W;
        const float4 a = acc[i];
        const float px = a.x * scale, py = a.y * scale, pz = a.z * scale;
        sum += px + py + pz;
        const uint32_t r = (uint32_t)(255.0f * min_std(1.0f, px)), g = (uint32_t)(255.0f * min_std(1.0f, py)), bb = (uint32_t)(255.0f * min_std(1.0f, pz));
        pixels[i] = (r << 16) + (g << 8) + bb;
    }
    tileSums[tile] = sum;
}

__global__ __launch_bounds__(256) void commit_frame_kernel(const float4* __restrict__ slabWindow, uint32_t frameInWindow, uint32_t passes,
                                                            float4* __restrict__ acc, uint32_t* __restrict__ pixels, float* __restrict__ tileSums,
                                                            uint32_t tileFirst, uint32_t tileStride, uint32_t tileCount, uint32_t tilesX,
                                                            uint32_t W, float scale)
{
    __shared__ float tileE[256];
    const uint32_t tl = blockIdx.x, pix = threadIdx.x;
    if (tl >= tileCount) return;
    const uint32_t tile = tileFirst + tl * tileStride;
    const uint32_t x0 = (tile % tilesX) * 16u, y0 = (tile / tilesX) * 16u;
    const size_t i = (x0 + (pix & 15u)) + (size_t)(y0 + (pix >> 4)) * W;
    const float4* __restrict__ s = slabWindow + ((size_t)tl * 256u + pix) * (64u * passes) + frameInWindow * passes;
    float4 a = acc[i];
    for (uint32_t p = 0; p < passes; p++) { const float4 t = s[p]; a.x += t.x; a.y += t.y; a.z += t.z; a.w += t.w; }
    acc[i] = a;
    const float px = a.x * scale, py = a.y * scale, pz = a.z * scale;
    tileE[pix] = px + py + pz;
    const uint32_t r = (uint32_t)(255.0f * min_std(1.0f, px)), g = (uint32_t)(255.0f * min_std(1.0f, py)), bb = (uint32_t)(255.0f * min_std(1.0f, pz));
    pixels[i] = (r << 16) + (g << 8) + bb;
    __syncthreads();
    if (pix == 0) {
        float sum = 0;
        for (uint32_t k = 0; k < 256u; k++) sum += tileE[k];
        tileSums[tile] = sum;
    }
}

}

namespace crt {
__device__ __forceinline__ bool same_bits(float a, float b) { return asu(a) == asu(b) || (a != a && b != b); }
__global__ __launch_bounds__(256) void check_reciprocals_kernel(unsigned long long* out)
{
    const uint32_t tid = blockIdx.x * 256u + threadIdx.x, nthreads = gridDim.x * 256u;
    unsigned long long n = 0, bad1 = 0, bad2 = 0, bad3 = 0;
    for (uint64_t b = tid; b < (1ull << 32); b += nthreads) {
        const float x = asf((uint32_t)b), want = 1.0f / x;
        n++;
        if (!same_bits(rcp_exact(x), want)) bad1++;
        if (!(__builtin_fabsf(x) < 0.0001f) && !same_bits(rcp_exact_large(x), want)) bad2++;
        const float y = asf((uint32_t)b * 2654435761u), z = asf(((uint32_t)b >> 7) * 40503u + 0x3f000000u);
        const f3 r = rcp_exact3(mk3(x, y, z));
        if (!same_bits(r.x, want) || !same_bits(r.y, 1.0f / y) || !same_bits(r.z, 1.0f / z)) bad3++;
    }
    atomicAdd(&out[0], n); atomicAdd(&out[1], bad1); atomicAdd(&out[2], bad2); atomicAdd(&out[3], bad3);
}
}
extern "C" hipError_t crt_launch_check_reciprocals(unsigned long long* out, hipStream_t stream)
{
    hipLaunchKernelGGL(crt::check_reciprocals_kernel, dim3(4096), dim3(256), 0, stream, out);
    return hipGetLastError();
}

namespace crt {
__global__ __launch_bounds__(256) void check_sqrt_kernel(unsigned long long* out)
{
    const uint32_t tid = blockIdx.x * 256u + threadIdx.x, nthreads = gridDim.x * 256u;
    unsigned long long n = 0, bad = 0;
    for (uint64_t b = tid; b < (1ull << 32); b += nthreads) {
        const float x = asf((uint32_t)b);
        n++;
        if (!same_bits(sqrt_exact(x), __builtin_sqrtf(x))) bad++;
    }
    atomicAdd(&out[0], n); atomicAdd(&out[1], bad);
}
}
extern "C" hipError_t crt_launch_check_sqrt(unsigned long long* out, hipStream_t stream)
{
    hipLaunchKernelGGL(crt::check_sqrt_kernel, dim3(4096), dim3(256), 0, stream, out);
    return hipGetLastError();
}

extern "C" hipError_t crt_launch_render(const crt::Scene* sc, void* slab, crt::Counters* counters, unsigned long long* tileClocks, const uint32_t* tileOrder,
                                        uint32_t tileFirst, uint32_t tileStride, uint32_t tileCount, uint32_t tilesX, uint32_t sppFirst,
                                        uint32_t frames, uint32_t passes, uint32_t ldsBytes, int collectStats, const uint32_t* blockDesc, uint32_t nBlocks, uint32_t* tileCost, uint32_t rankCount, unsigned long long* launchClk, hipStream_t stream)
{
    if (tileCount == 0 || frames == 0) return hipSuccess;
    const uint32_t windows = (frames + 63u) / 64u;
    if ((unsigned long long)tileCount * windows > 0x7fffffffull) return hipErrorInvalidValue;
    if (collectStats || nBlocks == 0u) blockDesc = nullptr;
    if (blockDesc && (tileCount > 0x10000u || windows > 64u)) return hipErrorInvalidValue;
    if (rankCount == 0u || rankCount > tileCount) rankCount = tileCount;
    dim3 grid(blockDesc ? nBlocks : rankCount * windows), block(64);
#define CRT_LAUNCH(K, C) hipLaunchKernelGGL((crt::render_tiles_kernel<K, C>), grid, block, ldsBytes + 15u * 64u * 4u , stream, *sc, (float4*)slab, counters, tileClocks, tileOrder, tileFirst, tileStride, tileCount, tilesX, sppFirst, frames, passes, windows, blockDesc, tileCost, rankCount, launchClk)
    if (sc->kind == 0) { if (collectStats) CRT_LAUNCH(0, true); else CRT_LAUNCH(0, false); }
    else { if (collectStats) CRT_LAUNCH(1, true); else CRT_LAUNCH(1, false); }
#undef CRT_LAUNCH
    return hipGetLastError();
}

extern "C" uint32_t crt_render_resident_waves(int device, int kind, uint32_t ldsBytes)
{
    int perCu = 0, cus = 0;
    const size_t lds = (size_t)ldsBytes + 15u * 64u * 4u;
    hipError_t e = kind == 0 ? hipOccupancyMaxActiveBlocksPerMultiprocessor(&perCu, crt::render_tiles_kernel<0, false>, 64, lds)
                             : hipOccupancyMaxActiveBlocksPerMultiprocessor(&perCu, crt::render_tiles_kernel<1, false>, 64, lds);
    if (e != hipSuccess || hipDeviceGetAttribute(&cus, hipDeviceAttributeMultiprocessorCount, device) != hipSuccess || perCu <= 0 || cus <= 0) { (void)hipGetLastError(); return 5120u; }
    return (uint32_t)perCu * (uint32_t)cus;
}

extern "C" hipError_t crt_launch_accumulate(const void* slab, void* acc, uint32_t tileFirst, uint32_t tileStride, uint32_t tileCount,
                                            uint32_t tilesX, uint32_t W, uint32_t frames, uint32_t passes, hipStream_t stream)
{
    if (tileCount == 0 || frames == 0) return hipSuccess;
    dim3 grid(tileCount), block(256);
    hipLaunchKernelGGL(crt::accumulate_kernel, grid, block, 4u * crt::kAccWaveLds, stream, (const float4*)slab, (float*)acc, tileFirst, tileStride, tileCount, tilesX, W, frames, passes);
    return hipGetLastError();
}

extern "C" hipError_t crt_launch_find_nearest(const crt::Scene* sc, const void* rays, void* hits, uint32_t n, crt::Counters* counters,
                                              uint32_t ldsBytes, uint32_t* cursor, hipStream_t stream)
{
    hipError_t e; if (!crt::query_launch_begin(n, cursor, stream, &e)) return e;
    dim3 grid(crt::query_grid(n, ldsBytes)), block(64);
    hipLaunchKernelGGL(crt::find_nearest_kernel, grid, block, ldsBytes, stream, *sc, (const crt::RayIn*)rays, (crt::HitOut*)hits, n, counters, cursor);
    return hipGetLastError();
}

extern "C" hipError_t crt_launch_is_occluded(const crt::Scene* sc, const void* rays, int32_t* occluded, uint32_t n, uint32_t ldsBytes, uint32_t* cursor, hipStream_t stream)
{
    hipError_t e; if (!crt::query_launch_begin(n, cursor, stream, &e)) return e;
    dim3 grid(crt::query_grid(n, ldsBytes)), block(64);
    hipLaunchKernelGGL(crt::is_occluded_kernel, grid, block, ldsBytes, stream, *sc, (const crt::ShadowRayIn*)rays, occluded, n, cursor);
    return hipGetLastError();
}

extern "C" hipError_t crt_launch_whitted(const crt::Scene* sc, int accel, const crt::AltAccelDev* alt, const crt::TlasAltDev* tl, void* acc, uint32_t* pixels, crt::Counters* counters, uint32_t ldsBytes,
                                         hipStream_t stream)
{
    const uint32_t n = (uint32_t)sc->W * (uint32_t)sc->H;
    dim3 grid((n + 63u) / 64u), block(64);
    if (accel != 0 && sc->kind != 0) {
        const uint32_t bytes = crt::tlas_alt_stack_words(*sc, *tl) * 64u * 4u;
        if (bytes > 64u * 1024u) return hipErrorInvalidValue;
        if (accel == 1) hipLaunchKernelGGL((crt::whitted_kernel<1, crt::TlasAltDev>), grid, block, bytes, stream, *sc, *tl, (float4*)acc, pixels, counters);
        else hipLaunchKernelGGL((crt::whitted_kernel<2, crt::TlasAltDev>), grid, block, bytes, stream, *sc, *tl, (float4*)acc, pixels, counters);
        return hipGetLastError();
    }
    if (accel == 1) hipLaunchKernelGGL(crt::whitted_kernel<1>, grid, block, alt->kdStack * 128u * 4u, stream, *sc, *alt, (float4*)acc, pixels, counters);
    else if (accel == 2) hipLaunchKernelGGL(crt::whitted_kernel<2>, grid, block, 256u, stream, *sc, *alt, (float4*)acc, pixels, counters);
    else { const crt::AltAccelDev none{}; hipLaunchKernelGGL(crt::whitted_kernel<0>, grid, block, ldsBytes, stream, *sc, none, (float4*)acc, pixels, counters); }
    return hipGetLastError();
}

template <int ACCEL, class ALT>
static hipError_t launch_whitted_inspect(const crt::Scene& sc, const ALT& alt, uint32_t ldsBytes, int inspect, int32_t peakIn, float4* acc, uint32_t* pixels, crt::Counters* counters,
                                         int32_t* trav, int32_t* tested, crt::InspectSums* sums, int32_t* blockMax, hipStream_t stream)
{
    const uint32_t n = (uint32_t)sc.W * (uint32_t)sc.H;
    dim3 grid((n + 63u) / 64u), block(64);
    if (inspect == 0) {
        const crt::InspectOut out{trav, tested, sums};
        hipLaunchKernelGGL((crt::whitted_kernel<ACCEL, ALT, crt::InspectOut>), grid, block, ldsBytes, stream, sc, alt, acc, pixels, counters, out);
        return hipGetLastError();
    }
    hipLaunchKernelGGL((crt::inspect_primary_kernel<ACCEL, ALT>), grid, block, ldsBytes, stream, sc, alt, acc, pixels, counters, trav, tested, sums, blockMax, inspect == 2 ? 1 : 0);
    hipError_t e = hipGetLastError();
    if (e != hipSuccess) return e;
    hipLaunchKernelGGL(crt::inspect_color_kernel, dim3((n + crt::kInspectBlock - 1u) / crt::kInspectBlock), dim3(crt::kInspectBlock), 0, stream,
                       inspect == 2 ? tested : trav, blockMax, peakIn, n, acc, pixels);
    return hipGetLastError();
}

extern "C" size_t crt_whitted_inspect_work_bytes(uint32_t pixelCount) { return sizeof(crt::InspectSums) + (size_t)((pixelCount + crt::kInspectBlock - 1u) / crt::kInspectBlock) * 4u; }

extern "C" hipError_t crt_launch_whitted_inspect(const crt::Scene* sc, int accel, const crt::AltAccelDev* alt, const crt::TlasAltDev* tl, int inspect, int32_t peakIn, void* acc, uint32_t* pixels,
                                                 crt::Counters* counters, int32_t* trav, int32_t* tested, void* work, uint32_t ldsBytes, hipStream_t stream)
{
    if (inspect < 0 || inspect > 2 || peakIn < 0 || !trav || !tested || !work) return hipErrorInvalidValue;
    const uint32_t n = (uint32_t)sc->W * (uint32_t)sc->H;
    uint32_t bytes = 0;
    if (accel != 0 && sc->kind != 0) {
        bytes = crt::tlas_alt_stack_words(*sc, *tl) * 64u * 4u;
        if (bytes > 64u * 1024u) return hipErrorInvalidValue;
    }
    if (hipMemsetAsync(work, 0, crt_whitted_inspect_work_bytes(n), stream) != hipSuccess) return hipGetLastError();
    crt::InspectSums* sums = (crt::InspectSums*)work;
    int32_t* blockMax = (int32_t*)(sums + 1);
    if (accel != 0 && sc->kind != 0) {
        if (accel == 1) return launch_whitted_inspect<1>(*sc, *tl, bytes, inspect, peakIn, (float4*)acc, pixels, counters, trav, tested, sums, blockMax, stream);
        return launch_whitted_inspect<2>(*sc, *tl, bytes, inspect, peakIn, (float4*)acc, pixels, counters, trav, tested, sums, blockMax, stream);
    }
    if (accel == 1) return launch_whitted_inspect<1>(*sc, *alt, alt->kdStack * 128u * 4u, inspect, peakIn, (float4*)acc, pixels, counters, trav, tested, sums, blockMax, stream);
    if (accel == 2) return launch_whitted_inspect<2>(*sc, *alt, 256u, inspect, peakIn, (float4*)acc, pixels, counters, trav, tested, sums, blockMax, stream);
    const crt::AltAccelDev none{};
    return launch_whitted_inspect<0>(*sc, none, ldsBytes, inspect, peakIn, (float4*)acc, pixels, counters, trav, tested, sums, blockMax, stream);
}

extern "C" hipError_t crt_launch_resolve(const void* acc, uint32_t* pixels, float* tileSums, uint32_t tileFirst, uint32_t tileStride,
                                         uint32_t tileCount, uint32_t tilesX, uint32_t W, float scale, hipStream_t stream)
{
    if (tileCount == 0) return hipSuccess;
    dim3 grid((tileCount + 63u) / 64u), block(64);
    hipLaunchKernelGGL(crt::resolve_kernel, grid, block, 0, stream, (const float4*)acc, pixels, tileSums, tileFirst, tileStride, tileCount, tilesX, W, scale);
    return hipGetLastError();
}

extern "C" hipError_t crt_launch_commit_frame(const void* slabWindow, uint32_t frameInWindow, uint32_t passes, void* acc, uint32_t* pixels, float* tileSums,
                                              uint32_t tileFirst, uint32_t tileStride, uint32_t tileCount, uint32_t tilesX, uint32_t W, float scale, hipStream_t stream)
{
    if (tileCount == 0) return hipSuccess;
    if (frameInWindow >= 64u || passes < 1u || passes > 4u) return hipErrorInvalidValue;
    hipLaunchKernelGGL(crt::commit_frame_kernel, dim3(tileCount), dim3(256), 0, stream, (const float4*)slabWindow, frameInWindow, passes, (float4*)acc, pixels, tileSums,
                       tileFirst, tileStride, tileCount, tilesX, W, scale);
    return hipGetLastError();
}
```

### cpu-ray-tracer_amd/csrc/device/launch.h

```cpp
#pragma once
#include "layout.h"

#include <hip/hip_runtime.h>

extern "C" {

hipError_t crt_launch_check_reciprocals(unsigned long long* out, hipStream_t stream);
hipError_t crt_launch_check_sqrt(unsigned long long* out, hipStream_t stream);
hipError_t crt_launch_render(const crt::Scene* sc, void* slab, crt::Counters* counters, unsigned long long* tileClocks, const uint32_t* tileOrder, uint32_t tileFirst, uint32_t tileStride,
    uint32_t tileCount, uint32_t tilesX, uint32_t sppFirst, uint32_t frames, uint32_t passes, uint32_t ldsBytes, int collectStats, const uint32_t* blockDesc, uint32_t nBlocks, uint32_t* tileCost,
    uint32_t rankCount, unsigned long long* launchClk, hipStream_t stream);
uint32_t crt_render_resident_waves(int device, int kind, uint32_t ldsBytes);
hipError_t crt_launch_accumulate(const void* slab, void* acc, uint32_t tileFirst, uint32_t tileStride, uint32_t tileCount, uint32_t tilesX, uint32_t W, uint32_t frames, uint32_t passes,
    hipStream_t stream);
hipError_t crt_launch_find_nearest(const crt::Scene* sc, const void* rays, void* hits, uint32_t n, crt::Counters* counters, uint32_t ldsBytes, uint32_t* cursor, hipStream_t stream);
hipError_t crt_launch_is_occluded(const crt::Scene* sc, const void* rays, int32_t* occluded, uint32_t n, uint32_t ldsBytes, uint32_t* cursor, hipStream_t stream);
hipError_t crt_launch_whitted(const crt::Scene* sc, int accel, const crt::AltAccelDev* alt, const crt::TlasAltDev* tl, void* acc, uint32_t* pixels, crt::Counters* counters, uint32_t ldsBytes,
    hipStream_t stream);
size_t crt_whitted_inspect_work_bytes(uint32_t pixelCount);
hipError_t crt_launch_whitted_inspect(const crt::Scene* sc, int accel, const crt::AltAccelDev* alt, const crt::TlasAltDev* tl, int inspect, int32_t peakIn, void* acc, uint32_t* pixels,
    crt::Counters* counters, int32_t* trav, int32_t* tested, void* work, uint32_t ldsBytes, hipStream_t stream);
hipError_t crt_launch_resolve(const void* acc, uint32_t* pixels, float* tileSums, uint32_t tileFirst, uint32_t tileStride, uint32_t tileCount, uint32_t tilesX, uint32_t W, float scale,
    hipStream_t stream);
hipError_t crt_launch_commit_frame(const void* slabWindow, uint32_t frameInWindow, uint32_t passes, void* acc, uint32_t* pixels, float* tileSums, uint32_t tileFirst, uint32_t tileStride,
    uint32_t tileCount, uint32_t tilesX, uint32_t W, float scale, hipStream_t stream);

uint32_t crt_pool_streams(uint32_t frames);
size_t crt_pool_scratch_bytes_per_window(uint32_t tileCount);
hipError_t crt_launch_render_pool(const crt::Scene* sc, void* slab, void* facScratch, crt::Counters* counters, unsigned long long* tileClocks, const uint32_t* tileOrder, uint32_t tileFirst,
    uint32_t tileStride, uint32_t tileCount, uint32_t tilesX, uint32_t sppFirst, uint32_t frames, uint32_t passes, int collectStats, uint32_t rankFirst,
    uint32_t rankEnd , uint32_t waveFrames,
    const uint32_t* waveTab , uint32_t tabBlocks, uint32_t longFrames, uint32_t* tileCost, unsigned long long* launchClk,
    const uint8_t* tileClass , uint32_t extraLds ,
    hipStream_t stream);
uint32_t crt_pool_lds_bytes(uint32_t stackDepth, uint32_t streams, uint32_t refBits );
uint32_t crt_pool_lds_limit(int device);
int crt_debug_pool_stamps(unsigned long long* out, int reset);
int crt_debug_pool_density(unsigned long long* out, int reset);
size_t crt_debug_pool_timeline(unsigned long long* out, size_t cap);

hipError_t crt_launch_render_sky(const crt::Scene* sc, void* slab, crt::Counters* counters, const uint32_t* tileOrder, uint32_t rankFirst, uint32_t skyTiles, uint32_t tileFirst,
    uint32_t tileStride, uint32_t tileCount , uint32_t tilesX, uint32_t sppFirst, uint32_t frames, uint32_t passes,
    unsigned long long* launchClk , hipStream_t stream);

uint32_t crt_probe_paths(void);
hipError_t crt_launch_probe(const crt::Scene* sc, uint32_t tileFirst, uint32_t tileStride, uint32_t tileCount, uint32_t tilesX, uint32_t* tileCost, hipStream_t stream);
hipError_t crt_launch_render_alt(int accel, const crt::Scene* sc, const crt::AltAccelDev* acc, const crt::TlasAltDev* tl, void* slab, crt::Counters* counters, uint32_t tileFirst, uint32_t tileStride,
    uint32_t tileCount, uint32_t tilesX, uint32_t sppFirst, uint32_t frames, uint32_t passes, hipStream_t stream);
hipError_t crt_launch_sample_query(int accel, const crt::Scene* sc, const crt::AltAccelDev* acc, const crt::TlasAltDev* tl, const void* rays, uint32_t* seeds, float* rgb, uint32_t n,
    crt::Counters* counters, uint32_t* cursor, uint32_t* residentLanes, hipStream_t stream);

hipError_t crt_launch_find_nearest_prim(const crt::PrimDev* p, const void* rays, void* hits, uint32_t n, hipStream_t stream);
hipError_t crt_launch_render_prim(const crt::Scene* sc, const crt::PrimDev* p, void* slab, crt::Counters* counters, uint32_t tileFirst, uint32_t tileStride, uint32_t tileCount, uint32_t tilesX,
    uint32_t sppFirst, uint32_t frames, uint32_t passes, hipStream_t stream);
hipError_t crt_launch_sample_query_prim(const crt::Scene* sc, const crt::PrimDev* p, const void* rays, uint32_t* seeds, float* rgb, uint32_t n, crt::Counters* counters, uint32_t* cursor,
    uint32_t* residentLanes, hipStream_t stream);
hipError_t crt_launch_probe_f64(int op, const void* in, void* out, uint32_t n, hipStream_t stream);

hipError_t crt_launch_find_nearest_alt(int kind, const crt::Scene* sc, const crt::AltAccelDev* acc, const void* rays, void* hits, uint32_t n, uint32_t* cursor, hipStream_t stream);
hipError_t crt_launch_is_occluded_alt(int kind, const crt::Scene* sc, const crt::AltAccelDev* acc, const void* rays, int32_t* occluded, uint32_t n, uint32_t* cursor, hipStream_t stream);
hipError_t crt_launch_tlas_alt_query(int kind, bool occl, const crt::Scene* sc, const crt::TlasAltDev* tl, const void* rays, void* out, uint32_t n, uint32_t* cursor, hipStream_t stream);

hipError_t crt_launch_hit_info(const crt::Scene* sc, const void* rays, const void* hits, void* out, uint32_t n, uint32_t objects, uint32_t fileTris, hipStream_t stream);
hipError_t crt_launch_sky_color(const crt::Scene* sc, const void* rays, float* rgb, uint32_t n, hipStream_t stream);
hipError_t crt_launch_refit(char* geom, uint32_t leafOff, uint32_t pairBase, uint32_t triBase, uint32_t triCount, const float* pos, const void* plan, const uint32_t* levelOff, uint32_t levels,
    uint32_t rootCode, float* out, hipStream_t stream);
hipError_t crt_launch_probe_f32(int op, const void* in, void* out, uint32_t n, hipStream_t stream);

uint32_t crt_grid_build_blocks(int device);
size_t crt_grid_scan_chunks(uint32_t cells);
hipError_t crt_launch_grid_bounds(const float* pos, uint32_t triCount, crt::GridBuildState* state, uint32_t maxBlocks, hipStream_t stream);
hipError_t crt_launch_grid_count(const float* pos, uint32_t triCount, const crt::GridParams* g, uint32_t cells, uint32_t* counts, unsigned long long* chunkSums, crt::GridBuildState* state,
    uint32_t maxBlocks, hipStream_t stream);
hipError_t crt_launch_grid_fill(const float* pos, uint32_t triCount, const crt::GridParams* g, uint32_t cells, const uint32_t* cellStart, uint32_t* cursor, int32_t* unsorted, int32_t* refs,
    uint32_t total, const char* geom, uint32_t leafOff, uint32_t triBase, int globalIdx, crt::AltTri* tris, uint32_t maxBlocks, hipStream_t stream);

hipError_t crt_launch_tlas_build(const char* geom, uint32_t instOff, const float* T, const float* rootBox, uint32_t blasCount, uint32_t pairRel, uint32_t instRel, uint32_t poolRefBits,
    void* out, hipStream_t stream);

uint32_t crt_debug_query_grid(void);

}

namespace crt {

inline uint32_t bounded_query_grid(uint32_t grid) { const uint32_t k = crt_debug_query_grid(); return (k != 0u && k < grid) ? k : grid; }

inline uint32_t query_grid(uint32_t n, uint32_t ldsBytes)
{
    uint32_t perCu = ldsBytes ? (160u * 1024u) / ldsBytes : 16u; if (perCu > 16u) perCu = 16u; if (perCu < 4u) perCu = 4u;
    const uint32_t need = (n + 63u) / 64u, fill = 256u * perCu;
    return bounded_query_grid(need < fill ? need : fill);
}

inline bool query_launch_begin(uint32_t n, uint32_t* cursor, hipStream_t stream, hipError_t* status)
{
    *status = hipSuccess;
    if (n == 0) return false;
    if (!cursor) { *status = hipErrorInvalidValue; return false; }
    if (hipMemsetAsync(cursor, 0, 4, stream) != hipSuccess) { *status = hipGetLastError(); return false; }
    return true;
}

}
```

### cpu-ray-tracer_amd/csrc/device/render_pool.hip

```cpp
#include <type_traits>
#include "launch.h"
#include "sample_body.h"

namespace crt {

enum : uint32_t {
    F_OX = 0, F_OY, F_OZ, F_DX, F_DY, F_DZ,
    F_RX, F_RY, F_RZ,
    F_T,
    F_SEED, F_META,
    F_U, F_V,
    F_COUNT,
    F_CUR = F_U, F_PEND = F_V,
    F_TRI = F_RX
};
constexpr uint32_t kMetaItemMask = 0x7ffu, kMetaDepthShift = 11u, kMetaInside = 1u << 14, kMetaFresh = 1u << 15, kMetaObjShift = 16u, kMetaLowMask = 0xffffu;
constexpr uint32_t kQueueMask = 127u;

#ifndef CRT_POOL_MIN_WAVES
#define CRT_POOL_MIN_WAVES 4
#endif
#ifndef CRT_POOL_WIDE_MIN_WAVES
#define CRT_POOL_WIDE_MIN_WAVES 4
#endif
#ifndef CRT_POOL_NODE_STEPS
#define CRT_POOL_NODE_STEPS 2
#endif
#ifndef CRT_POOL_NODE2_MIN
#define CRT_POOL_NODE2_MIN 16
#endif
#ifndef CRT_POOL_STARVE
#define CRT_POOL_STARVE 40
#endif

#ifdef CRT_POOL_STAMPS
__device__ unsigned long long g_poolStamps[16];
#define CRT_PSTAMP(var) unsigned long long var; asm volatile("s_memtime %0\n\ts_waitcnt lgkmcnt(0)" : "=s"(var) :: "memory")
#define CRT_PACC(i, a, b) (pst[i] += (b) - (a))
#else
#define CRT_PSTAMP(var)
#define CRT_PACC(i, a, b)
#endif
#ifdef CRT_POOL_DENS
__device__ unsigned long long g_poolDens[48];
#define CRT_DENS(i, v) (dens[i] += (uint32_t)(v))
#define CRT_DENS_MASK(i, pred) (dens[i] += (uint32_t)__popcll(__builtin_amdgcn_ballot_w64(pred)))
#define CRT_LIVE_BUCKET(n) ((n) >= 112u ? 0u : (n) >= 96u ? 1u : (n) >= 64u ? 2u : 3u)
#else
#define CRT_DENS(i, v)
#define CRT_DENS_MASK(i, pred)
#endif
#ifdef CRT_POOL_TIMELINE
__device__ unsigned long long* g_poolTimeline = nullptr;
#endif
__device__ __forceinline__ bool lane_in(uint64_t m) { return __builtin_amdgcn_inverse_ballot_w64(m); }
__device__ __forceinline__ uint64_t finite3_mask(f3 v)
{
    const float inf = __builtin_inff();
    return __builtin_amdgcn_fcmpf(__builtin_fabsf(v.x), inf, 4) & __builtin_amdgcn_fcmpf(__builtin_fabsf(v.y), inf, 4) & __builtin_amdgcn_fcmpf(__builtin_fabsf(v.z), inf, 4);
}
#define CRT_CTL_SEQ() asm volatile("")
__device__ __forceinline__ bool ctl_free(uint64_t mRes) { CRT_CTL_SEQ(); return mRes != ~0ull; }
__device__ __forceinline__ uint32_t fresh(uint32_t x) { asm("" : "+s"(x)); return x; }
__device__ __forceinline__ uint32_t pop32(uint64_t m) { uint32_t n = (uint32_t)__builtin_popcountll(m); asm("" : "+s"(n)); return n; }
__device__ __forceinline__ uint64_t mask_ne(uint32_t a, uint32_t b) { return __builtin_amdgcn_uicmp(a, b, 33); }
__device__ __forceinline__ uint64_t mask_eq(uint32_t a, uint32_t b) { return __builtin_amdgcn_uicmp(a, b, 32); }
__device__ __forceinline__ uint64_t mask_ult(uint32_t a, uint32_t b) { return __builtin_amdgcn_uicmp(a, b, 36); }
__device__ __forceinline__ uint64_t mask_ule(uint32_t a, uint32_t b) { return __builtin_amdgcn_uicmp(a, b, 37); }
__device__ __forceinline__ uint64_t mask_sge(int a, int b) { return __builtin_amdgcn_sicmp(a, b, 39); }
__device__ __forceinline__ uint32_t rank_in(uint64_t m) { return __builtin_amdgcn_mbcnt_hi((uint32_t)(m >> 32), __builtin_amdgcn_mbcnt_lo((uint32_t)m, 0u)); }

template <int KIND, bool COUNT, int S, int REFBITS = 16>
__global__ __launch_bounds__(64, REFBITS == 32 ? CRT_POOL_WIDE_MIN_WAVES : CRT_POOL_MIN_WAVES) void render_pool_kernel(const Scene sc, float4* __restrict__ slab, float* __restrict__ facScratch, Counters* __restrict__ counters,
                                                             unsigned long long* __restrict__ tileClocks, const uint32_t* __restrict__ tileOrder,
                                                             uint32_t tileFirst, uint32_t tileStride, uint32_t tileCount, uint32_t tilesX,
                                                             uint32_t sppFirst, uint32_t frames, uint32_t passes, uint32_t groups, uint32_t waveFrames, const uint32_t* __restrict__ waveTab, uint32_t tabBlocks, uint32_t longFrames,
                                                             uint32_t rankFirst, uint32_t* __restrict__ tileCost, unsigned long long* __restrict__ launchClk, const uint8_t* __restrict__ tileClass)
{
    extern __shared__ uint32_t lds[];
    const uint32_t lane = threadIdx.x;
#ifdef CRT_POOL_TIMELINE
    const unsigned long long tl0 = wall_clock64();
#endif
    const unsigned long long clk0 = (COUNT || tileCost) ? wall_clock64() : 0ull;
    if (launchClk && lane == 0) { atomicMax(&launchClk[0], ~clk0); atomicMax(&launchClk[1], clk0); }
    uint32_t rank0, grp, wf = waveFrames, first = 0u, limit = frames;
    if (waveTab) {
        if (blockIdx.x < tabBlocks) {
            uint32_t lo = 0u, hi = tileCount - rankFirst;
            while (hi - lo > 1u) { const uint32_t mid = (lo + hi) >> 1; if (waveTab[2u * mid] <= blockIdx.x) lo = mid; else hi = mid; }
            rank0 = lo; grp = blockIdx.x - waveTab[2u * lo]; wf = waveTab[2u * lo + 1u]; limit = longFrames;
        } else { const uint32_t b = blockIdx.x - tabBlocks; rank0 = b / groups; grp = b - rank0 * groups; wf = (uint32_t)S; first = longFrames; }
    } else { rank0 = blockIdx.x / groups; grp = blockIdx.x - rank0 * groups; }
    const uint32_t rank = rank0 + rankFirst;
    if (rank >= tileCount) return;
    const uint32_t tl = tileOrder ? tileOrder[rank] : rank;
    const uint32_t frame0 = first + grp * wf;
    if (frame0 >= limit) return;
    const uint32_t nOwn = (limit - frame0 < wf) ? limit - frame0 : wf;
    const uint32_t nStreams = nOwn < (uint32_t)S ? nOwn : (uint32_t)S;
    const uint32_t tile = tileFirst + tl * tileStride;
    const uint32_t tx = tile % tilesX, ty = tile / tilesX;
    const uint32_t tcls = tileClass ? __builtin_amdgcn_readfirstlane((uint32_t)tileClass[tl]) : 0u;
    auto not_sky = [&]() -> bool { return fresh(tcls) != kTileSky; };
    const char* __restrict__ geom = sc.geom;
    float* __restrict__ fac = facScratch + (size_t)blockIdx.x * (15u * (uint32_t)S);

    constexpr PoolRefForm R = pool_ref_form((uint32_t)REFBITS);
    using StackEntry = std::conditional_t<REFBITS == 32, uint32_t, uint16_t>;
    constexpr uint32_t kEntryB = (uint32_t)sizeof(StackEntry), kLevelB = 64u * kEntryB;
    char* const ldsB = reinterpret_cast<char*>(lds);
    const uint32_t laneB = lane * kEntryB;
    uint32_t* st = lds + (sc.stackDepth + 1u) * (kLevelB / 4u);
    float* stf = reinterpret_cast<float*>(st);
    uint8_t* qEnd = reinterpret_cast<uint8_t*>(st + F_COUNT * S);
    uint8_t* qBnc = qEnd + 128, * qRdy = qEnd + 256;
    uint16_t* slotFrame = reinterpret_cast<uint16_t*>(qEnd + 384);
    auto stk_top = [&](uint32_t at) -> uint32_t { return *reinterpret_cast<const StackEntry*>(ldsB + at); };
    auto stk_put = [&](uint32_t at, uint32_t v) { *reinterpret_cast<StackEntry*>(ldsB + at) = (StackEntry)v; };

    Cnt cn; cn.rays = cn.primary = cn.interior = cn.leaf = cn.tri = cn.tlas = cn.visits = cn.meshhits = 0;
    uint32_t trips = 0;
#ifdef CRT_POOL_DENS
    uint32_t dens[48]; for (int i = 0; i < 48; i++) dens[i] = 0;
    uint32_t live = nStreams; unsigned long long liveClk = wall_clock64();
#endif
    const uint32_t items = 256u * passes;
    const uint32_t rowLen = 64u * passes;
    const f3 nil3 = mk3(0.0f, 0.0f, 0.0f);

    for (uint32_t s = lane; s < nStreams; s += 64u) {
        st[F_SEED * S + s] = stream_seed(tx, ty, (uint32_t)sc.W, sppFirst, frame0 + s, passes);
        st[F_META * S + s] = kMetaFresh;
        qEnd[s] = (uint8_t)s;
        if (S > 64) slotFrame[s] = (uint16_t)s;
    }
    uint32_t nLive = nStreams;
    uint32_t nextFrame = nStreams;
    uint32_t endH = 0, endT = nStreams, bncH = 0, bncT = 0, rdyH = 0, rdyT = 0;

    uint64_t mRes = 0ull;
    uint64_t mFinite = ~0ull;
    uint32_t sid = 0, cur = kRefDone, spB = laneB, metaLo = 0u;
    f3 tO = nil3, tD = nil3, trD = nil3;
    Hit h; h.t = 1e34f; h.u = 0; h.v = 0; h.objIdx = -1; h.triIdx = -1;
    rec4 q0 = {0, 0, 0, 0}, q1 = q0, q2 = q0, q3 = q0;

    auto new_ray = [&](auto primary, uint64_t mAct, uint32_t s, f3 v, bool norm, f3 O, uint32_t seed, uint32_t meta) {
        constexpr bool PRIM = decltype(primary)::value;
        const bool act = lane_in(mAct);
        const bool noLight = PRIM && (tcls & kTileNoLight) != 0u, noFloor = PRIM && (tcls & kTileNoFloor) != 0u, noTree = PRIM && (tcls & kTileNoTree) != 0u;
        f3 D = v, rD = v; Hit nh; nh.t = 1e34f; nh.u = 0; nh.v = 0; nh.objIdx = -1; nh.triIdx = -1;
        uint32_t ncur = kRefDone, pend = 0u;
        if (act) {
            const float inv = rcp_exact(sqrt_exact(dot3(v, v)));
            D = norm ? v * inv : v;
// ... 241 lines not shown
                endH += n;
                uint32_t meta = 0, seed = 0; int obj = -1; f3 D = nil3;
                if (act) { meta = st[F_META * S + s]; seed = st[F_SEED * S + s]; obj = (int)(meta >> kMetaObjShift) - 1; D = mk3(stf[F_DX * S + s], stf[F_DY * S + s], stf[F_DZ * S + s]); }
                const int depth = (int)((meta >> kMetaDepthShift) & 7u);
                uint32_t item = meta & kMetaItemMask;
                const uint64_t mFirst = mask_ne(meta & kMetaFresh, 0u), mEnded = mActE & ~mFirst, mMiss = mEnded & mask_eq(meta >> kMetaObjShift, 0u);
                const bool first = lane_in(mFirst), ended = lane_in(mEnded), miss = lane_in(mMiss);
#ifdef CRT_POOL_DENS
                dens[36u + CRT_LIVE_BUCKET(live)]++;
#endif
                CRT_DENS(9, 1); CRT_DENS(10, n); CRT_DENS_MASK(11, miss); CRT_DENS_MASK(13, act && first); CRT_DENS_MASK(25, ended && depth > 0); CRT_DENS_MASK(26, ended && depth > 1); CRT_DENS_MASK(27, ended && depth > 2);
                if (ended && obj >= 2) cn.meshhits++;
                float fk[15];
#pragma unroll
                for (int k = 0; k < 5; k++) {
                    fk[3 * k] = fk[3 * k + 1] = fk[3 * k + 2] = 0.0f;
                    if (not_sky()) if (ended && depth > k) {
#pragma unroll
                        for (int j = 0; j < 3; j++) fk[3 * k + j] = __hip_atomic_load(fac + (3 * k + j) * S + s, __ATOMIC_RELAXED, __HIP_MEMORY_SCOPE_AGENT);
                    }
                }
                uint32_t skyTexel = 0u;
                if (miss) {
                    float phi, theta; sky_angles(D, phi, theta);
                    const kernarg_f sk = scene_floats(offsetof(Scene, skyOffset));
                    skyTexel = sc.texels[tex_index(asu(sk[0]), (int)asu(sk[1]), (int)asu(sk[2]), phi * CRT_INV2PI, theta * CRT_INVPI)];
                }
                bool gen = act && first;
                size_t sampleAt = 0;
                if (ended) {
                    uint32_t pix = item, pass = 0;
                    if (fresh(passes) != 1u) { pix = item / passes; pass = item - pix * passes; }
                    const uint32_t fr = frame0 + (S > 64 ? (uint32_t)slotFrame[s] : s);
                    sampleAt = slab_position(fr, tileCount, tl, pix, rowLen, passes, pass);
                    item++;
                    gen = item < items;
                }
                uint64_t mGen = mFirst | (mEnded & mask_ult(item, items));
                const uint64_t mDone = mEnded & ~mGen;
                if (mDone != 0ull) {
                    uint64_t mTake = 0ull;
                    if (S > 64) if (nextFrame < nOwn) {
                        const uint32_t f = nextFrame + rank_in(mDone);
                        mTake = mDone & mask_ult(f, nOwn);
                        if (lane_in(mTake)) {
                            slotFrame[s] = (uint16_t)f;
                            seed = stream_seed(tx, ty, (uint32_t)sc.W, sppFirst, frame0 + f, passes);
                            item = 0u;
                        }
                        nextFrame += pop32(mTake);
                        mGen |= mTake;
                    }
                    nLive -= pop32(mDone & ~mTake);
                }
                gen = lane_in(mGen);
#ifdef CRT_POOL_DENS
                {
                    const uint32_t gone = (uint32_t)__popcll(__builtin_amdgcn_ballot_w64(ended) & ~__builtin_amdgcn_ballot_w64(gen));
                    if (gone) { const unsigned long long now = wall_clock64(); dens[44u + CRT_LIVE_BUCKET(live)] += (uint32_t)(now - liveClk); liveClk = now; live -= gone; }
                }
#endif
                const kernarg_f cam = scene_floats(offsetof(Scene, camPos));
                const f3 camPos = mk3(cam[0], cam[1], cam[2]);
                f3 v = camPos;
                if (gen) {
                    const uint32_t pix = (fresh(passes) == 1u) ? item : item / passes;
                    const f3 TL = mk3(cam[3], cam[4], cam[5]);
                    constexpr size_t pc = (offsetof(Scene, primRight) - offsetof(Scene, camPos)) / 4;
                    const f3 right = mk3(cam[pc], cam[pc + 1], cam[pc + 2]), down = mk3(cam[pc + 3], cam[pc + 4], cam[pc + 5]);
                    v = primary_target(camPos, TL, right, down, cam[12], cam[13], tx, ty, pix, seed);
                    cn.primary++;
                }
                CRT_DENS_MASK(12, gen);
                CRT_PSTAMP(e1); CRT_PACC(2, p2b, e1);
                new_ray(std::true_type{}, mGen, s, v, true, camPos, seed, item);
                CRT_PSTAMP(e2); CRT_PACC(3, e1, e2);
                if (ended) {
                    f3 L = miss ? tex_unpack(skyTexel) : ((depth >= sc.depthLimit) ? mk3(0, 0, 0) : mk3(24, 24, 22));
                    if (not_sky()) {
#pragma unroll
                        for (int k = 4; k >= 0; k--)
                            if (depth > k) L = mk3(fk[3 * k], fk[3 * k + 1], fk[3 * k + 2]) * L;
                    }
                    slab[sampleAt] = make_float4(L.x, L.y, L.z, 0.0f);
                }
#ifdef CRT_POOL_STAMPS
                { CRT_PSTAMP(e3); CRT_PACC(4, e2, e3); pst[10]++; }
#endif
                asm volatile("" :: "v"(fk[0]), "v"(fk[1]), "v"(fk[2]), "v"(fk[3]), "v"(fk[4]), "v"(fk[5]), "v"(fk[6]), "v"(fk[7]), "v"(fk[8]), "v"(fk[9]), "v"(fk[10]), "v"(fk[11]), "v"(fk[12]), "v"(fk[13]), "v"(fk[14]), "v"(skyTexel));
            }
            CRT_PSTAMP(p3);
            asm volatile("" ::: "memory");
            if (runBnc != 0u) {
                const uint32_t n = nBnc < 64u ? nBnc : 64u;
                const uint64_t mActB = mask_ult(lane, n);
                const bool act = lane_in(mActB);
                const uint32_t s = act ? qBnc[(bncH + lane) & kQueueMask] : 0u;
                bncH += n;
                f3 O = nil3, D = nil3; float ht = 0, hu = 0, hv = 0; int obj = 1; uint32_t tri = 0, seed = 0, meta = 0;
                if (act) {
                    tri = st[F_TRI * S + s];
                    O = mk3(stf[F_OX * S + s], stf[F_OY * S + s], stf[F_OZ * S + s]);
                    D = mk3(stf[F_DX * S + s], stf[F_DY * S + s], stf[F_DZ * S + s]);
                    ht = stf[F_T * S + s]; hu = stf[F_U * S + s]; hv = stf[F_V * S + s];
                    seed = st[F_SEED * S + s]; meta = st[F_META * S + s]; obj = (int)(meta >> kMetaObjShift) - 1;
                }
                const bool mesh = act && obj >= 2;
#ifdef CRT_POOL_DENS
                dens[40u + CRT_LIVE_BUCKET(live)]++;
#endif
                CRT_DENS(14, 1); CRT_DENS(15, n); CRT_DENS_MASK(16, mesh);
                rec4 s0 = {0, 0, 0, 0}, s1 = s0, s2 = s0, s3 = s0;
                if (mesh) { const uint32_t so = sc.shadeOff + tri * 64u; s0 = ldp<0>(geom, so); s1 = ldp<1>(geom, so); s2 = ldp<2>(geom, so); s3 = ldp<3>(geom, so); cn.meshhits++; }
                const bool inside = (meta & kMetaInside) != 0u;
                const int depth = (int)((meta >> kMetaDepthShift) & 7u);
                const uint32_t item = meta & kMetaItemMask;
                f3 v = O; bool newInside = false;
                if (act) {
                    const f3 I = O + ht * D;
                    SurfPoint p;
                    if (obj == 1) {
                        const kernarg_f fl = scene_floats(offsetof(Scene, floorN));
                        const kernarg_f fm = scene_floats(offsetof(Scene, floorMat));
                        const rec4 m0 = {fm[0], fm[1], fm[2], fm[3]}, m1 = {fm[4], fm[5], fm[6], fm[7]};
                        p = floor_point(mk3(fl[0], fl[1], fl[2]), fl[4], m0, m1, I);
                    } else p = mesh_point<KIND>(s0, s1, s2, s3, hu, hv, obj, geom, sc.instOff, sc.mats);
                    const f3 N = face_ray(p.N, D);
                    uint32_t texel = 0x00ffffffu;
                    if (p.tW > 0) texel = sc.texels[tex_index(p.tOff, p.tW, p.tH, p.tu, p.tv)];
                    const f3 medium = medium_of(inside, p.absorb, ht);
                    CRT_PSTAMP(b1); CRT_PACC(5, p3, b1);
                    const Bounce b = draw_bounce(seed, D, N, inside, p.refl, p.refr);
                    newInside = b.newInside;
                    const f3 c = (p.tW > 0) ? tex_unpack(texel) : mk3(1.0f, 1.0f, 1.0f);
                    CRT_PSTAMP(b2); CRT_PACC(6, b1, b2);
                    const float inv = rcp_exact(sqrt_exact(dot3(b.v, b.v)));
                    const f3 nv = b.branch == kDiffuse ? b.v * inv : b.v;
                    v = nv;
                    const f3 factor = bounce_factor(b.branch, c, medium, nv, N);
                    float* fd = fac + (3 * depth) * S + s;
                    __hip_atomic_store(fd, factor.x, __ATOMIC_RELAXED, __HIP_MEMORY_SCOPE_AGENT);
                    __hip_atomic_store(fd + S, factor.y, __ATOMIC_RELAXED, __HIP_MEMORY_SCOPE_AGENT);
                    __hip_atomic_store(fd + 2 * S, factor.z, __ATOMIC_RELAXED, __HIP_MEMORY_SCOPE_AGENT);
                    O = I + nv * CRT_EPS;
                    CRT_PSTAMP(b3); CRT_PACC(7, b2, b3);
                }
                CRT_PSTAMP(b4);
                new_ray(std::false_type{}, mActB, s, v, false, O, seed, item | ((uint32_t)(depth + 1) << kMetaDepthShift) | (newInside ? kMetaInside : 0u));
#ifdef CRT_POOL_STAMPS
                { CRT_PSTAMP(b5); CRT_PACC(8, b4, b5); pst[11]++; }
#endif
                asm volatile("" :: "v"(s0), "v"(s1), "v"(s2), "v"(s3));
            }
        }
        if (nLive == 0u) break;
    }
#ifdef CRT_POOL_STAMPS
    if (lane == 0) for (int i = 0; i < 12; i++) atomicAdd(&g_poolStamps[i], pst[i]);
#endif
#ifdef CRT_POOL_DENS
    dens[44u + CRT_LIVE_BUCKET(live)] += (uint32_t)(wall_clock64() - liveClk);
    if (lane == 0) for (int i = 0; i < 48; i++) if (dens[i]) atomicAdd(&g_poolDens[i], (unsigned long long)dens[i]);
#endif

#ifdef CRT_POOL_TIMELINE
    if (lane == 0 && g_poolTimeline) { uint32_t hw; asm volatile("s_getreg_b32 %0, hwreg(HW_REG_HW_ID)" : "=s"(hw)); g_poolTimeline[3 * (size_t)blockIdx.x] = tl0; g_poolTimeline[3 * (size_t)blockIdx.x + 1] = wall_clock64(); g_poolTimeline[3 * (size_t)blockIdx.x + 2] = hw; }
#endif
// ... 1 lines not shown
    if (launchClk && lane == 0) { const unsigned long long now = wall_clock64(), last = __hip_atomic_load(&launchClk[1], __ATOMIC_RELAXED, __HIP_MEMORY_SCOPE_AGENT), from = last > clk0 ? last : clk0; if (now > from) atomicAdd(&launchClk[2], now - from); }
    if (COUNT && tileClocks && lane == 0 && nOwn == frames) {
        tileClocks[2 * tl] = wall_clock64() - clk0;
        tileClocks[2 * tl + 1] = trips;
    }
    uint32_t vals[8] = {cn.rays, cn.primary, cn.interior, cn.leaf, cn.tri, cn.tlas, cn.visits, cn.meshhits};
#pragma unroll
    for (int i = 0; i < 8; i++) {
        if (!COUNT && i >= 2 && i != 7) continue;
        uint32_t sum = wave_sum(vals[i]);
        if (lane == 0 && sum) atomicAdd(&counters->v[i], (unsigned long long)sum);
    }
}

}

#ifndef CRT_POOL_STREAMS
#define CRT_POOL_STREAMS 128
#endif
extern "C" uint32_t crt_pool_streams(uint32_t frames) { return frames > 64u ? (uint32_t)CRT_POOL_STREAMS : 64u; }
extern "C" uint32_t crt_pool_lds_bytes(uint32_t stackDepth, uint32_t streams, uint32_t refBits) { return (stackDepth + 1u) * 64u * (refBits / 8u) + crt::F_COUNT * streams * 4u + 3u * 128u + (streams > 64u ? 2u * streams : 0u); }
extern "C" uint32_t crt_pool_lds_limit(int device)
{
    static uint32_t known[64] = {};
    if (device >= 0 && device < 64 && known[device]) return known[device];
    int v = 0;
    if (hipDeviceGetAttribute(&v, hipDeviceAttributeMaxSharedMemoryPerBlock, device) != hipSuccess || v <= 0) { (void)hipGetLastError(); return 0u; }
    const uint32_t limit = (uint32_t)v < 64u * 1024u ? (uint32_t)v : 64u * 1024u;
    if (device >= 0 && device < 64) known[device] = limit;
    return limit;
}
extern "C" size_t crt_pool_scratch_bytes_per_window(uint32_t tileCount) { return (size_t)tileCount * 128u * 15u * 4u; }

#ifdef CRT_POOL_STAMPS
extern "C" int crt_debug_pool_stamps(unsigned long long* out, int reset)
{
    if (out && hipMemcpyFromSymbol(out, HIP_SYMBOL(crt::g_poolStamps), 128) != hipSuccess) return -1;
    if (reset) { unsigned long long z[16] = {}; if (hipMemcpyToSymbol(HIP_SYMBOL(crt::g_poolStamps), z, 128) != hipSuccess) return -1; }
    return 0;
}
#endif
#ifdef CRT_POOL_DENS
extern "C" int crt_debug_pool_density(unsigned long long* out, int reset)
{
    if (out && hipMemcpyFromSymbol(out, HIP_SYMBOL(crt::g_poolDens), 384) != hipSuccess) return -1;
    if (reset) { unsigned long long z[48] = {}; if (hipMemcpyToSymbol(HIP_SYMBOL(crt::g_poolDens), z, 384) != hipSuccess) return -1; }
    return 0;
}
#endif
#ifdef CRT_POOL_TIMELINE
static unsigned long long* g_timelineHost = nullptr; static size_t g_timelineCount = 0;
extern "C" size_t crt_debug_pool_timeline(unsigned long long* out, size_t cap)
{
    const size_t n = g_timelineCount < cap ? g_timelineCount : cap;
    if (out && n) (void)hipMemcpy(out, g_timelineHost, n * 24, hipMemcpyDeviceToHost);
    return g_timelineCount;
}
#endif
extern "C" hipError_t crt_launch_render_pool(const crt::Scene* sc, void* slab, void* facScratch, crt::Counters* counters, unsigned long long* tileClocks, const uint32_t* tileOrder,
                                             uint32_t tileFirst, uint32_t tileStride, uint32_t tileCount, uint32_t tilesX, uint32_t sppFirst,
                                             uint32_t frames, uint32_t passes, int collectStats, uint32_t rankFirst, uint32_t rankEnd, uint32_t waveFrames, const uint32_t* waveTab, uint32_t tabBlocks, uint32_t longFrames,
                                             uint32_t* tileCost, unsigned long long* launchClk, const uint8_t* tileClass, uint32_t extraLds, hipStream_t stream)
{
    if (tileCount == 0 || frames == 0) return hipSuccess;
    if (sc->poolRefBits != 16u && sc->poolRefBits != 32u) return hipErrorInvalidValue;
    const uint32_t S = crt_pool_streams(frames);
    const uint32_t wf = (S == 64u || waveFrames < S) ? S : waveFrames;
    if (wf % S != 0u || wf > 0xff80u) return hipErrorInvalidValue;
    if (S == 64u) waveTab = nullptr;
    if (waveTab && (tabBlocks == 0u || longFrames == 0u || longFrames > frames)) return hipErrorInvalidValue;
    const uint32_t groups = waveTab ? (frames - longFrames + S - 1u) / S : (frames + wf - 1u) / wf;
    if ((unsigned long long)tileCount * ((frames + S - 1u) / S) > 0x7fffffffull) return hipErrorInvalidValue;
    if (rankEnd > tileCount) return hipErrorInvalidValue;
    if (rankFirst >= rankEnd) return hipSuccess;
    dim3 grid(waveTab ? tabBlocks + (rankEnd - rankFirst) * groups : (rankEnd - rankFirst) * groups), block(64);
#ifdef CRT_POOL_TIMELINE
    { static unsigned long long* buf = nullptr; static size_t cap = 0;
      if (cap < (size_t)grid.x) { if (buf) (void)hipFree(buf); (void)hipMalloc((void**)&buf, (size_t)grid.x * 24); cap = grid.x; (void)hipMemcpyToSymbol(HIP_SYMBOL(crt::g_poolTimeline), &buf, sizeof(buf)); }
      (void)hipMemsetAsync(buf, 0, (size_t)grid.x * 24, stream); g_timelineHost = buf; g_timelineCount = grid.x; }
#endif
    const uint32_t ldsBytes = crt_pool_lds_bytes(sc->stackDepth, S, sc->poolRefBits) + extraLds;
    { int dev = 0; if (hipGetDevice(&dev) != hipSuccess) return hipGetLastError(); if (ldsBytes > crt_pool_lds_limit(dev)) return hipErrorInvalidValue; }
#define CRT_LAUNCH(K, C, SS) do { if (sc->poolRefBits == 32u) CRT_LAUNCH_R(K, C, SS, 32); else CRT_LAUNCH_R(K, C, SS, 16); } while (0)
#define CRT_LAUNCH_R(K, C, SS, RB) hipLaunchKernelGGL((crt::render_pool_kernel<K, C, SS, RB>), grid, block, ldsBytes, stream, *sc, (float4*)slab, (float*)facScratch, counters, tileClocks, tileOrder, tileFirst, tileStride, tileCount, tilesX, sppFirst, frames, passes, groups, wf, waveTab, tabBlocks, longFrames, rankFirst, tileCost, launchClk, tileClass)
#define CRT_LAUNCH_S(K, C) do { if (S == 64u) CRT_LAUNCH(K, C, 64); else CRT_LAUNCH(K, C, CRT_POOL_STREAMS); } while (0)
    if (sc->kind == 0) { if (collectStats) CRT_LAUNCH_S(0, true); else CRT_LAUNCH_S(0, false); }
    else { if (collectStats) CRT_LAUNCH_S(1, true); else CRT_LAUNCH_S(1, false); }
#undef CRT_LAUNCH_S
#undef CRT_LAUNCH
#undef CRT_LAUNCH_R
    return hipGetLastError();
}
```

### cpu-ray-tracer_amd/csrc/device/render_seq.hip

```cpp
#include "alt_common.h"
#include "file_surface.h"
#include "launch.h"
#include "sample_query.h"

namespace crt {

template <int KIND>
struct BvhWorld : FileSurface<KIND> {
    __device__ __host__ uint32_t stack_words(const Scene& sc) const { return sc.stackDepth; }
    __device__ __forceinline__ uint32_t trace(const Scene& sc, f3 O, f3 D, f3 rD, Hit& h, uint32_t* stk) const
    {
        Cnt cn; cn.rays = cn.primary = cn.interior = cn.leaf = cn.tri = cn.tlas = cn.visits = cn.meshhits = 0;
        int traversed = 0, tested = 0;
        find_nearest_seq(sc, O, D, rD, h, stk, cn, traversed, tested);
        return cn.interior + cn.tri + cn.tlas;
    }
};

struct KdWorld : FileSurface<0> {
    AltAccelDev acc;
    __device__ __host__ uint32_t stack_words(const Scene&) const { return acc.kdStack * 2u; }
    __device__ __forceinline__ uint32_t trace(const Scene& sc, f3 O, f3 D, f3 rD, Hit& h, uint32_t* stk) const
    {
        int traversed = 0, tested = 0;
        hit_light_floor(sc, O, D, h);
        kd_intersect(acc, O, D, rD, h, stk, traversed, tested);
        return 0u;
    }
};
struct GridWorld : FileSurface<0> {
    AltAccelDev acc;
    __device__ __host__ uint32_t stack_words(const Scene&) const { return 0u; }
    __device__ __forceinline__ uint32_t trace(const Scene& sc, f3 O, f3 D, f3 rD, Hit& h, uint32_t*) const
    {
        int traversed = 0, tested = 0;
        hit_light_floor(sc, O, D, h);
        grid_intersect(acc, O, D, rD, h, traversed, tested);
        return 0u;
    }
};

template <int ACCEL>
struct TlasAltWorld : FileSurface<1> {
    TlasAltDev tl;
    __device__ __host__ uint32_t stack_words(const Scene& sc) const { return tlas_alt_stack_words(sc, tl); }
    __device__ __forceinline__ uint32_t trace(const Scene& sc, f3 O, f3 D, f3 rD, Hit& h, uint32_t* stk) const
    {
        int traversed = 0, tested = 0;
        hit_light_floor(sc, O, D, h);
        tlas_alt_intersect<ACCEL>(sc, tl, O, D, rD, h, stk, traversed, tested);
        return 0u;
    }
};
using TlasKdWorld = TlasAltWorld<1>;
using TlasGridWorld = TlasAltWorld<2>;

}

extern "C" uint32_t crt_probe_paths() { return 64u * crt::kProbeWaves; }
extern "C" hipError_t crt_launch_probe(const crt::Scene* sc, uint32_t tileFirst, uint32_t tileStride, uint32_t tileCount, uint32_t tilesX, uint32_t* tileCost, hipStream_t stream)
{
    if (tileCount == 0 || !tileCost || tileCount > 0x10000u) return hipSuccess;
    const uint32_t nProbe = tileCount * crt::kProbeWaves;
    dim3 grid((nProbe + crt::kSeqWaves - 1u) / crt::kSeqWaves), block(64u * crt::kSeqWaves);
    const uint32_t ldsBytes = crt::seq_lds_bytes(sc->stackDepth);
    if (hipMemsetAsync(tileCost, 0, (size_t)tileCount * 4, stream) != hipSuccess) return hipGetLastError();
    if (sc->kind == 0) hipLaunchKernelGGL((crt::render_seq_kernel<crt::BvhWorld<0>, true>), grid, block, ldsBytes, stream, *sc, crt::BvhWorld<0>{}, (float4*)nullptr, (crt::Counters*)nullptr, tileFirst, tileStride, tileCount, tilesX, 1u, 64u, 1u, nProbe, tileCost);
    else hipLaunchKernelGGL((crt::render_seq_kernel<crt::BvhWorld<1>, true>), grid, block, ldsBytes, stream, *sc, crt::BvhWorld<1>{}, (float4*)nullptr, (crt::Counters*)nullptr, tileFirst, tileStride, tileCount, tilesX, 1u, 64u, 1u, nProbe, tileCost);
    return hipGetLastError();
}

extern "C" hipError_t crt_launch_render_alt(int accel, const crt::Scene* sc, const crt::AltAccelDev* acc, const crt::TlasAltDev* tl, void* slab, crt::Counters* counters, uint32_t tileFirst,
                                            uint32_t tileStride, uint32_t tileCount, uint32_t tilesX, uint32_t sppFirst, uint32_t frames, uint32_t passes, hipStream_t stream)
{
    if (tileCount == 0 || frames == 0) return hipSuccess;
    if (accel != 1 && accel != 2) return hipErrorInvalidValue;
    const uint32_t windows = (frames + 63u) / 64u;
    if ((unsigned long long)tileCount * windows > 0x7fffffffull || tileCount > 0x10000u || windows > 64u) return hipErrorInvalidValue;
    if (sc->kind != 0) {
        if (crt::seq_lds_bytes(crt::tlas_alt_stack_words(*sc, *tl)) > 64u * 1024u) return hipErrorInvalidValue;
        if (accel == 1) return crt::launch_render_seq(sc, crt::TlasKdWorld{{}, *tl}, slab, counters, tileFirst, tileStride, tileCount, tilesX, sppFirst, frames, passes, stream);
        return crt::launch_render_seq(sc, crt::TlasGridWorld{{}, *tl}, slab, counters, tileFirst, tileStride, tileCount, tilesX, sppFirst, frames, passes, stream);
    }
    if (accel == 1) {
        const crt::KdWorld kd{{}, *acc};
        if (crt::seq_lds_bytes(kd.stack_words(*sc)) > 64u * 1024u) return hipErrorInvalidValue;
        return crt::launch_render_seq(sc, kd, slab, counters, tileFirst, tileStride, tileCount, tilesX, sppFirst, frames, passes, stream);
    }
    return crt::launch_render_seq(sc, crt::GridWorld{{}, *acc}, slab, counters, tileFirst, tileStride, tileCount, tilesX, sppFirst, frames, passes, stream);
}

extern "C" hipError_t crt_launch_sample_query(int accel, const crt::Scene* sc, const crt::AltAccelDev* acc, const crt::TlasAltDev* tl, const void* rays, uint32_t* seeds, float* rgb,
                                              uint32_t n, crt::Counters* counters, uint32_t* cursor, uint32_t* residentLanes, hipStream_t stream)
{
    if (accel < 0 || accel > 2) return hipErrorInvalidValue;
    if (accel == 0) {
        if (sc->kind == 0) return crt::launch_sample_query(sc, crt::BvhWorld<0>{}, rays, seeds, rgb, n, counters, cursor, residentLanes, stream);
        return crt::launch_sample_query(sc, crt::BvhWorld<1>{}, rays, seeds, rgb, n, counters, cursor, residentLanes, stream);
    }
    if (sc->kind != 0) {
        if (accel == 1) return crt::launch_sample_query(sc, crt::TlasKdWorld{{}, *tl}, rays, seeds, rgb, n, counters, cursor, residentLanes, stream);
        return crt::launch_sample_query(sc, crt::TlasGridWorld{{}, *tl}, rays, seeds, rgb, n, counters, cursor, residentLanes, stream);
    }
    if (accel == 1) return crt::launch_sample_query(sc, crt::KdWorld{{}, *acc}, rays, seeds, rgb, n, counters, cursor, residentLanes, stream);
    return crt::launch_sample_query(sc, crt::GridWorld{{}, *acc}, rays, seeds, rgb, n, counters, cursor, residentLanes, stream);
}
```

### cpu-ray-tracer_amd/csrc/device/render_sky.hip

```cpp
#include "launch.h"
#include "sample_body.h"

namespace crt {

__global__ __launch_bounds__(64) void render_sky_kernel(const Scene sc, float4* __restrict__ slab, Counters* __restrict__ counters, const uint32_t* __restrict__ tileOrder,
                                                        uint32_t rankFirst, uint32_t skyTiles, uint32_t tileFirst, uint32_t tileStride, uint32_t tileCount, uint32_t tilesX,
                                                        uint32_t sppFirst, uint32_t frames, uint32_t passes, uint32_t groups, unsigned long long* __restrict__ launchClk)
{
    const uint32_t lane = threadIdx.x;
    const uint32_t r = blockIdx.x / groups, grp = blockIdx.x - r * groups;
    if (r >= skyTiles) return;
    const unsigned long long clk0 = launchClk ? wall_clock64() : 0ull;
    const uint32_t tl = tileOrder[rankFirst + r];
    const uint32_t tile = tileFirst + tl * tileStride;
    const uint32_t tx = tile % tilesX, ty = tile / tilesX;
    const uint32_t fr = grp * 64u + lane;
    const uint32_t items = 256u * passes, rowLen = 64u * passes;
    uint32_t paths = 0;
    if (fr < frames) {
        uint32_t seed = stream_seed(tx, ty, (uint32_t)sc.W, sppFirst, fr, passes);
        const f3 camPos = mk3(sc.camPos[0], sc.camPos[1], sc.camPos[2]), TL = mk3(sc.topLeft[0], sc.topLeft[1], sc.topLeft[2]);
        const f3 right = mk3(sc.primRight[0], sc.primRight[1], sc.primRight[2]), down = mk3(sc.primDown[0], sc.primDown[1], sc.primDown[2]);
        uint32_t pix = 0, pass = 0;
#pragma unroll 4
        for (uint32_t item = 0; item < items; item++) {
            const f3 v = primary_target(camPos, TL, right, down, sc.invW, sc.invH, tx, ty, pix, seed);
            const f3 D = v * rcp_exact(sqrt_exact(dot3(v, v)));
            float phi, theta; sky_angles(D, phi, theta);
            const f3 L = tex_unpack(sc.texels[tex_index(sc.skyOffset, sc.skyW, sc.skyH, phi * CRT_INV2PI, theta * CRT_INVPI)]);
            slab[slab_position(fr, tileCount, tl, pix, rowLen, passes, pass)] = make_float4(L.x, L.y, L.z, 0.0f);
            if (++pass == passes) { pass = 0; pix++; }
        }
        paths = items;
    }
    const uint32_t sum = wave_sum(paths);
    if (lane == 0 && sum) { atomicAdd(&counters->v[0], (unsigned long long)sum); atomicAdd(&counters->v[1], (unsigned long long)sum); }
    if (launchClk && lane == 0) { atomicMax(&launchClk[0], ~clk0); atomicMax(&launchClk[1], wall_clock64()); }
}

}

extern "C" hipError_t crt_launch_render_sky(const crt::Scene* sc, void* slab, crt::Counters* counters, const uint32_t* tileOrder, uint32_t rankFirst, uint32_t skyTiles,
                                            uint32_t tileFirst, uint32_t tileStride, uint32_t tileCount, uint32_t tilesX, uint32_t sppFirst, uint32_t frames, uint32_t passes,
                                            unsigned long long* launchClk, hipStream_t stream)
{
    if (skyTiles == 0 || frames == 0) return hipSuccess;
    if (!tileOrder || rankFirst > tileCount || skyTiles > tileCount - rankFirst || passes == 0) return hipErrorInvalidValue;
    const uint32_t groups = (frames + 63u) / 64u;
    if ((unsigned long long)skyTiles * groups > 0x7fffffffull) return hipErrorInvalidValue;
    hipLaunchKernelGGL(crt::render_sky_kernel, dim3(skyTiles * groups), dim3(64), 0, stream, *sc, (float4*)slab, counters, tileOrder, rankFirst, skyTiles, tileFirst, tileStride,
                       tileCount, tilesX, sppFirst, frames, passes, groups, launchClk);
    return hipGetLastError();
}
```

### cpu-ray-tracer_amd/csrc/device/sample_body.h

```cpp
#pragma once
#include "dev_common.h"

namespace crt {

struct SurfPoint { f3 N; float tu, tv, refl, refr; f3 absorb; uint32_t tOff; int tW, tH, mat; };

__device__ __forceinline__ void set_material(SurfPoint& p, rec4 m0, rec4 m1)
{
    p.refl = m0.x; p.refr = m0.y; p.absorb = mk3(m0.z, m0.w, m1.x);
    p.tOff = asu(m1.y); p.tW = (int)asu(m1.z); p.tH = (int)asu(m1.w);
}
__device__ __forceinline__ SurfPoint floor_point(f3 floorN, float floorInvto, rec4 m0, rec4 m1, f3 I)
{
    SurfPoint p; p.N = floorN; p.tu = 0; p.tv = 0; p.mat = 1;
    if (floorN.y == 1) {
        float u = I.x, v = I.z;
        u *= floorInvto; v *= floorInvto;
        p.tu = u - __builtin_floorf(u); p.tv = v - __builtin_floorf(v);
    }
    set_material(p, m0, m1);
    return p;
}
__device__ __forceinline__ SurfPoint floor_point(f3 floorN, float floorInvto, const Material& m, f3 I)
{
// ... 2 lines not shown
}
template <int KIND>
__device__ __forceinline__ SurfPoint mesh_point(rec4 s0, rec4 s1, rec4 s2, rec4 s3, float u, float v, int objIdx, const char* __restrict__ geom, uint32_t instOff, const Material* __restrict__ mats)
{
    SurfPoint p;
    const f3 n0 = mk3(s0.x, s0.y, s0.z), n1 = mk3(s0.w, s1.x, s1.y), n2 = mk3(s1.z, s1.w, s2.x);
    const float w = 1 - u - v;
    const f3 Nn = w * n0 + u * n1 + v * n2;
    p.tu = w * s2.y + u * s2.w + v * s3.y;
    p.tv = w * s2.z + u * s3.x + v * s3.z;
    p.mat = (int)asu(s3.w);
    const rec4* mp = reinterpret_cast<const rec4*>(mats + p.mat);
    set_material(p, mp[0], mp[1]);
    if (KIND == 0) p.N = normalize3(Nn);
    else {
        const uint32_t io = instOff + (uint32_t)(objIdx - 2) * 128u + 64u;
        const rec4 r0 = ldp<0>(geom, io), r1 = ldp<1>(geom, io), r2 = ldp<2>(geom, io);
        p.N = normalize3(mk3(r0.x * Nn.x + r0.y * Nn.y + r0.z * Nn.z + r0.w * 0.0f,
                             r1.x * Nn.x + r1.y * Nn.y + r1.z * Nn.z + r1.w * 0.0f,
                             r2.x * Nn.x + r2.y * Nn.y + r2.z * Nn.z + r2.w * 0.0f));
    }
    return p;
}
__device__ __forceinline__ f3 face_ray(f3 N, f3 D) { return (dot3(N, D) > 0) ? -N : N; }

__device__ __forceinline__ f3 medium_of(bool inside, f3 absorb, float t)
{
    f3 medium = mk3(1, 1, 1);
    if (inside) {
        const f3 ab = absorb * -t;
        medium = mk3(crt_expf(ab.x), crt_expf(ab.y), crt_expf(ab.z));
    }
    return medium;
}
enum Branch : int { kMirror, kDielectric, kDiffuse };
struct Bounce { f3 v; Branch branch; bool newInside; };
__device__ __forceinline__ Bounce draw_bounce(uint32_t& seed, f3 D, f3 N, bool inside, float refl, float refr)
{
    Bounce b; b.newInside = false;
    const float r = rnd(seed);
    if (r < refl) {
        b.v = D - 2.0f * N * dot3(N, D); b.branch = kMirror;
    } else if (r < refl + refr) {
        b.v = D - 2.0f * N * dot3(N, D); b.branch = kDielectric;
        const float n1 = inside ? 1.2f : 1, n2 = inside ? 1 : 1.2f;
        const float eta = n1 / n2, cosi = dot3(-D, N);
        const float cost2 = 1.0f - eta * eta * (1 - cosi * cosi);
        if (cost2 > 0) {
            const float a = n1 - n2, b2 = n1 + n2, R0 = (a * a) / (b2 * b2), cc = 1 - cosi;
            const float Fr = R0 + (1 - R0) * (cc * cc * cc * cc * cc);
            const f3 T = eta * D + ((eta * cosi - sqrt_exact(__builtin_fabsf(cost2))) * N);
            if (rnd(seed) > Fr) { b.v = T; b.newInside = !inside; }
        }
    } else {
        f3 Rr;
        do {
            const float rz = rnd_pm1(seed);
            const float ry = rnd_pm1(seed);
            const float rx = rnd_pm1(seed);
            Rr = mk3(rx, ry, rz);
        } while (dot3(Rr, Rr) > 1);
        if (dot3(Rr, N) < 0) Rr = Rr * -1.0f;
        b.v = Rr; b.branch = kDiffuse;
    }
    return b;
}
__device__ __forceinline__ f3 bounce_factor(Branch branch, f3 c, f3 medium, f3 nv, f3 N)
{
    if (branch != kDiffuse) return c * medium;
    const f3 brdf = c * CRT_INVPI;
    return medium * brdf * 2.0f * CRT_PI * dot3(nv, N);
}
__device__ __forceinline__ void sample_unwind(const float* fst, int depth, f3& L)
{
#pragma unroll
    for (int k = 4; k >= 0; k--)
        if (depth > k) { const float* fd = fst + (uint32_t)(3 * k) * 64u; L = mk3(fd[0], fd[64], fd[128]) * L; }
}

__device__ __forceinline__ uint32_t stream_seed(uint32_t tx, uint32_t ty, uint32_t W, uint32_t sppFirst, uint32_t frame, uint32_t passes)
{
    return init_seed(tx + ty * W + (sppFirst + frame * passes) * 1799u);
}
__device__ __forceinline__ size_t slab_position(uint32_t fr, uint32_t tileCount, uint32_t tl, uint32_t pix, uint32_t rowLen, uint32_t passes, uint32_t pass)
{
    return (((size_t)(fr >> 6) * tileCount + tl) * 256u + pix) * rowLen + ((fr & 63u) * passes + pass);
}
__device__ __forceinline__ f3 primary_target(f3 camPos, f3 TL, f3 right, f3 down, float invW, float invH, uint32_t tx, uint32_t ty, uint32_t pix, uint32_t& seed)
{
    const int x = (int)(tx * 16u + (pix & 15u)), y = (int)(ty * 16u + (pix >> 4));
    const float jy = rnd(seed);
    const float jx = rnd(seed);
    const float u = ((float)x + jx) * invW, vv = ((float)y + jy) * invH;
    const f3 P = TL + u * right + vv * down;
    return P - camPos;
}
template <bool PRIM>
__device__ __forceinline__ LightFloor light_floor_from_kernarg()
{
    const kernarg_f lp = scene_floats(offsetof(Scene, lightInvT));
    const kernarg_f ax = scene_floats(offsetof(Scene, lightAxis));
    LightFloor lf;
#pragma unroll
    for (int i = 0; i < 12; i++) lf.lightInvT[i] = lp[i];
    lf.lightSize = lp[15]; lf.floorN[0] = lp[19]; lf.floorN[1] = lp[20]; lf.floorN[2] = lp[21]; lf.floorD = lp[22];
    lf.lightAxis = asu(ax[0]); lf.floorAxisY = asu(ax[1]);
    lf.preOy = lf.preOx = lf.preOz = lf.preNum = 0.0f;
    if constexpr (PRIM) {
        constexpr size_t pl = (offsetof(Scene, primLight) - offsetof(Scene, lightInvT)) / 4;
        lf.preOy = lp[pl]; lf.preOx = lp[pl + 1]; lf.preOz = lp[pl + 2]; lf.preNum = lp[pl + 3];
    }
    return lf;
}

struct Ordered { uint32_t nearRef, farRef; bool hitN, push; };
__device__ __forceinline__ Ordered ordered_step(float d1, float d2, uint32_t refA, uint32_t refB)
{
    const bool sw = d1 > d2;
    const float dn = sw ? d2 : d1, df = sw ? d1 : d2;
    Ordered o;
    o.nearRef = sw ? refB : refA; o.farRef = sw ? refA : refB;
    o.hitN = dn != 1e30f; o.push = o.hitN && df != 1e30f;
    return o;
}

}
```

### cpu-ray-tracer_amd/csrc/device/seq_sample.h

```cpp
#pragma once
#include "sample_body.h"

namespace crt {

struct Surf { f3 N, c; float refl, refr; f3 absorb; };

constexpr uint32_t kSeqWaves = 4u;
constexpr uint32_t kProbeWaves = 8u;

__device__ __host__ __forceinline__ uint32_t seq_lds_bytes(uint32_t stackWords) { return kSeqWaves * (stackWords + 15u) * 64u * 4u; }

template <class World, bool PROBE>
__device__ __forceinline__ bool sample_step(const Scene& sc, const World& world, uint32_t* stk, float* fst, f3& O, f3& D, bool& inside, int& depth, uint32_t& seed, f3& L,
                                            uint32_t& nRays, uint32_t& nMesh, uint32_t& steps)
{
    const f3 rD = rcp_exact3(D);
    Hit h; h.t = 1e34f; h.u = 0; h.v = 0; h.objIdx = -1; h.triIdx = -1;
    nRays++;
    const uint32_t traceSteps = world.trace(sc, O, D, rD, h, stk);
    if (PROBE) steps += traceSteps + 3u;
    if (World::kMeshHits && h.objIdx >= 2) nMesh++;
    if (h.objIdx == -1) { L = world.miss(sc, D); return true; }
    if (depth >= sc.depthLimit) { L = mk3(0, 0, 0); return true; }
    if (h.objIdx == 0) { L = mk3(24, 24, 22); return true; }
    const f3 I = O + h.t * D;
    const Surf s = world.surface(sc, h, I, D);
    const f3 N = s.N, c = s.c;
    const f3 medium = medium_of(inside, s.absorb, h.t);
    const Bounce b = draw_bounce(seed, D, N, inside, s.refl, s.refr);
    const f3 nv = b.branch == kDiffuse ? b.v * rcp_exact(sqrt_exact(dot3(b.v, b.v))) : b.v;
    const f3 factor = bounce_factor(b.branch, c, medium, nv, N);
    float* fd = fst + (uint32_t)(3 * depth) * 64u;
    fd[0] = factor.x; fd[64] = factor.y; fd[128] = factor.z;
    depth++;
    O = I + nv * CRT_EPS; D = nv; inside = b.newInside;
    return false;
}

template <class World, bool PROBE>
__global__ __launch_bounds__(256, 4) void render_seq_kernel(const Scene sc, const World world, float4* __restrict__ slab, Counters* __restrict__ counters,
                                                           uint32_t tileFirst, uint32_t tileStride, uint32_t tileCount, uint32_t tilesX,
                                                           uint32_t sppFirst, uint32_t frames, uint32_t passes, uint32_t nEntries, uint32_t* __restrict__ tileCost)
{
    extern __shared__ uint32_t ldsAll[];
    const uint32_t lane = threadIdx.x & 63u, wave = threadIdx.x >> 6;
    const uint32_t entry = blockIdx.x * kSeqWaves + wave;
    if (entry >= nEntries) return;
    const uint32_t windows = (frames + 63u) / 64u;
    const uint32_t tl = PROBE ? entry / kProbeWaves : entry / windows, win = PROBE ? 0u : entry % windows;
    if (tl >= tileCount) return;
    sppFirst += win * 64u * passes;
    frames = (frames - win * 64u < 64u) ? frames - win * 64u : 64u;
    if (lane >= frames) return;
    slab += (size_t)win * ((size_t)tileCount * 256u * 64u * passes);
    const uint32_t tile = tileFirst + tl * tileStride;
    const uint32_t tx = tile % tilesX, ty = tile / tilesX;
    const uint32_t stackWords = world.stack_words(sc);
    uint32_t* stk = ldsAll + wave * (stackWords + 15u) * 64u + lane;
    float* fst = reinterpret_cast<float*>(stk + stackWords * 64u);

    uint32_t nRays = 0, nPrimary = 0, nMesh = 0;
    const uint32_t items = PROBE ? 1u : 256u * passes;
    uint32_t seed = init_seed(tx + ty * (uint32_t)sc.W + (sppFirst + lane * passes) * 1799u);
    if (PROBE) seed = init_seed(0x9e3779b9u ^ ((tile * kProbeWaves + entry % kProbeWaves) * 64u + lane));
    uint32_t steps = 0;

    const kernarg_f cam = scene_floats(offsetof(Scene, camPos));
    const f3 camPos = mk3(cam[0], cam[1], cam[2]);
    const f3 TL = mk3(cam[3], cam[4], cam[5]), TR = mk3(cam[6], cam[7], cam[8]), BL = mk3(cam[9], cam[10], cam[11]);
    const float invW = cam[12], invH = cam[13];

    for (uint32_t item = 0; item < items; item++) {
        const uint32_t pix = PROBE ? ((lane * 4u + entry % kProbeWaves) & 255u) : ((passes == 1u) ? item : item / passes);
        const f3 v = primary_target(camPos, TL, TR - TL, BL - TL, invW, invH, tx, ty, pix, seed);
        f3 O = camPos, D = v * rcp_exact(sqrt_exact(dot3(v, v)));
        bool inside = false; int depth = 0;
        nPrimary++;
        f3 L = mk3(0, 0, 0);
        while (!sample_step<World, PROBE>(sc, world, stk, fst, O, D, inside, depth, seed, L, nRays, nMesh, steps)) {}
        sample_unwind(fst, depth, L);
        if (!PROBE) {
            uint32_t pass = 0;
            if (passes != 1u) pass = item - pix * passes;
            slab[((size_t)tl * 256u + pix) * (64u * passes) + (lane * passes + pass)] = make_float4(L.x, L.y, L.z, 0.0f);
        } else if (L.x != L.x) steps++;
    }
    if (PROBE) { const uint32_t sum = wave_sum(steps); if (lane == 0) atomicAdd(&tileCost[tl], sum); return; }
    atomicAdd(&counters->v[0], (unsigned long long)nRays);
    atomicAdd(&counters->v[1], (unsigned long long)nPrimary);
    if (nMesh) atomicAdd(&counters->v[7], (unsigned long long)nMesh);
}

template <class World>
hipError_t launch_render_seq(const Scene* sc, const World& world, void* slab, Counters* counters, uint32_t tileFirst, uint32_t tileStride, uint32_t tileCount, uint32_t tilesX,
                             uint32_t sppFirst, uint32_t frames, uint32_t passes, hipStream_t stream)
{
    const uint32_t entries = tileCount * ((frames + 63u) / 64u);
    hipLaunchKernelGGL((render_seq_kernel<World, false>), dim3((entries + kSeqWaves - 1u) / kSeqWaves), dim3(64u * kSeqWaves), seq_lds_bytes(world.stack_words(*sc)), stream,
                       *sc, world, (float4*)slab, counters, tileFirst, tileStride, tileCount, tilesX, sppFirst, frames, passes, entries, (uint32_t*)nullptr);
    return hipGetLastError();
}

}
```

Baseline: 33130 Mrays/s.

## Shrink sample slab to 12-byte RGB and store sky samples as packed texels

Changes the per-sample slab record from float4 (16 bytes) to a packed 3-float record (12 bytes), and lets sky-only tiles write the raw 4-byte texture texel instead of an unpacked colour. The accumulate kernel gains a texel path that unpacks in LDS while summing, and the tile order decides which ranks hold texels. The aim is to cut slab write and read traffic between the render and accumulate kernels. In exchange, 12-byte stores are not naturally vector-aligned, the accumulate LDS layout is more complex, and a second code path is added.

```diff
diff --git a/cpu-ray-tracer_amd/csrc/abi.cpp b/cpu-ray-tracer_amd/csrc/abi.cpp
--- a/cpu-ray-tracer_amd/csrc/abi.cpp
+++ b/cpu-ray-tracer_amd/csrc/abi.cpp
@@ -993,7 +993,7 @@
     return 0;
 }
 
-static size_t sample_bytes_per_window(const crt_ctx* c, uint32_t passes) { return (size_t)c->tileCount * 256u * 64u * passes * 16u; }
+static size_t sample_bytes_per_window(const crt_ctx* c, uint32_t passes) { return crt_slab_window_bytes(c->tileCount, passes); }
 static size_t window_bytes(const crt_ctx* c, uint32_t passes) { return sample_bytes_per_window(c, passes) + (c->usePool ? crt_pool_scratch_bytes_per_window(c->tileCount) : 0); }
 
 static uint32_t block_desc(uint32_t tile, uint32_t laneBase, uint32_t lanes, uint32_t window) { uint32_t lg = 0; while ((1u << lg) < lanes) lg++; return tile | (laneBase << 16) | (lg << 22) | (window << 25); }
@@ -1498,6 +1498,7 @@
     uint32_t head = 0, jobBlocks = 0; unsigned long long* jobClk = nullptr;
     uint32_t waveFrames = 0, waveBlocks = 0, longFrames = 0, longWaves = 0; const uint32_t* waveTab = nullptr;
     uint32_t sky = 0;
+    bool skyTexels = false;
 };
 
 static int next_block_table(crt_ctx* c);
@@ -1596,7 +1597,7 @@
         const bool skyBehind = sky_behind();
         auto launch_sky = [&](hipStream_t s) -> hipError_t {
             return crt_launch_render_sky(&c->hScene, L.slab, c->dCounters, c->dTileOrder, c->tileCount - L.sky, L.sky, c->tileFirst, c->tileStride, c->tileCount, (uint32_t)c->tilesX,
-                                         L.sppFirst, L.nf, L.passes, L.jobClk ? L.jobClk + 3 : nullptr, s);
+                                         L.sppFirst, L.nf, L.passes, L.skyTexels ? 1 : 0, L.jobClk ? L.jobClk + 3 : nullptr, s);
         };
         if (L.sky && !skyBehind) { le = launch_sky(st); if (le == hipSuccess) c->skyLaunches++; }
         if (le != hipSuccess) return le;
@@ -1682,6 +1683,7 @@
     Launch L; L.st = st; L.ev = ev; L.slab = slab; L.sppFirst = sppFirst; L.nf = nf; L.passes = passes; L.windows = (nf + 63u) / 64u;
     if ((r = tuner_prepare(c, L))) return r;
     if ((r = planner_prepare(c, L))) return r;
+    L.skyTexels = ahead == nullptr;
     HIPCK(c, hipEventRecord(ev.a, st));
     const bool pool = L.pool, wantCost = L.wantCost, wantJobCost = L.wantJobCost;
     const hipError_t le = hook("CRT_DEBUG_FAIL_LAUNCH") ? hipErrorInvalidConfiguration  : launch_render_kernels(c, L);
@@ -1719,7 +1721,8 @@
     HIPCK(c, hipStreamWaitEvent(c->stream, ev.b, 0));
     if ((r = take_event(c, c->evAcc, &ev))) return r;
     HIPCK(c, hipEventRecord(ev.a, c->stream));
-    HIPCK(c, crt_launch_accumulate(slab, c->dAcc, c->tileFirst, c->tileStride, c->tileCount, (uint32_t)c->tilesX, (uint32_t)c->cfg.width, nf, passes, c->stream));
+    const uint32_t texelFirst = (L.pool && L.skyTexels) ? c->tileCount - L.sky : c->tileCount;
+    HIPCK(c, crt_launch_accumulate(slab, c->dAcc, c->dTileOrder, texelFirst, c->tileFirst, c->tileStride, c->tileCount, (uint32_t)c->tilesX, (uint32_t)c->cfg.width, nf, passes, c->stream));
     HIPCK(c, hipEventRecord(ev.b, c->stream));
     HIPCK(c, hipEventRecord(reg.freed, c->stream));
     c->inflight.push_back(reg);
@@ -1756,7 +1759,7 @@
             void* slab = c->pool + off;
             if (c->havePrim) HIPCK(c, crt_launch_render_prim(&c->hScene, &c->prim, slab, c->dCounters, c->tileFirst, c->tileStride, c->tileCount, (uint32_t)c->tilesX, spp_first + f0 * passes, nf, passes, c->stream));
             else HIPCK(c, crt_launch_render_alt(c->renderAccel, &c->hScene, &c->alt, &c->blasAlt[c->renderAccel - 1], slab, c->dCounters, c->tileFirst, c->tileStride, c->tileCount, (uint32_t)c->tilesX, spp_first + f0 * passes, nf, passes, c->stream));
-            HIPCK(c, crt_launch_accumulate(slab, c->dAcc, c->tileFirst, c->tileStride, c->tileCount, (uint32_t)c->tilesX, (uint32_t)c->cfg.width, nf, passes, c->stream));
+            HIPCK(c, crt_launch_accumulate(slab, c->dAcc, nullptr, c->tileCount, c->tileFirst, c->tileStride, c->tileCount, (uint32_t)c->tilesX, (uint32_t)c->cfg.width, nf, passes, c->stream));
             crt_ctx::Region reg; reg.off = off; reg.bytes = (size_t)((nf + 63u) / 64u) * windowBytes;
             if (c->freeEvents.empty()) HIPCK(c, hipEventCreateWithFlags(&reg.freed, hipEventDisableTiming));
             else { reg.freed = c->freeEvents.back(); c->freeEvents.pop_back(); }
@@ -3011,6 +3014,12 @@
     return (int)c.skyTiles;
 }
 extern "C" int crt_debug_sky_launches(crt_ctx* c) { return c ? (int)c->skyLaunches : -1; }
+extern "C" int crt_debug_slab_layout(int texel, uint32_t frames, uint32_t tileCount, uint32_t passes, unsigned long long* pos, unsigned long long* sizes)
+{
+    if (!pos || !sizes || passes < 1 || passes > 4 || tileCount == 0 || frames == 0) return CRT_ERR_INVALID;
+    crt_slab_layout_probe(texel, frames, tileCount, passes, pos, sizes);
+    return CRT_OK;
+}
 extern "C" int crt_debug_job_costs(crt_ctx* c, uint32_t* out, double* poolWindowTicks, double* skyWindowTicks)
 {
     if (!c || !out) return CRT_ERR_INVALID;
diff --git a/cpu-ray-tracer_amd/csrc/device/kernels.hip b/cpu-ray-tracer_amd/csrc/device/kernels.hip
--- a/cpu-ray-tracer_amd/csrc/device/kernels.hip
+++ b/cpu-ray-tracer_amd/csrc/device/kernels.hip
@@ -24,7 +24,7 @@
 #define CRT_MIN_WAVES 5
 #endif
 template <int KIND, bool COUNT>
-__global__ __launch_bounds__(64, CRT_MIN_WAVES) void render_tiles_kernel(const Scene sc, float4* __restrict__ slab,
+__global__ __launch_bounds__(64, CRT_MIN_WAVES) void render_tiles_kernel(const Scene sc, char* __restrict__ slab,
                                                            Counters* __restrict__ counters, unsigned long long* __restrict__ tileClocks,
                                                            const uint32_t* __restrict__ tileOrder,
                                                            uint32_t tileFirst, uint32_t tileStride, uint32_t tileCount, uint32_t tilesX,
@@ -43,7 +43,7 @@
     sppFirst += win * 64u * passes;
     frames = (frames - win * 64u < 64u) ? frames - win * 64u : 64u;
     if (blockDesc) frames = frames > laneBase ? ((frames - laneBase < myLanes) ? frames - laneBase : myLanes) : 0u;
-    slab += (size_t)win * ((size_t)tileCount * 256u * 64u * passes);
+    slab += slab_block_position(win, tileCount, tl, 64u * passes);
     const uint32_t tile = tileFirst + tl * tileStride;
     const uint32_t tx = tile % tilesX, ty = tile / tilesX;
     uint32_t* stk = lds + lane;
@@ -162,7 +162,7 @@
                 sample_unwind(fst, depth, L);
                 uint32_t pix = item, pass = 0;
                 if (passes != 1u) { pix = item / passes; pass = item - pix * passes; }
-                slab[((size_t)tl * 256u + pix) * (64u * passes) + ((laneBase + lane) * passes + pass)] = make_float4(L.x, L.y, L.z, 0.0f);
+                store_sample(slab, slab_sample_offset(laneBase + lane, pix, 64u * passes, passes, pass), L);
                 item++;
                 gen = true;
                 if (item >= items) { live = false; gen = false; }
@@ -323,51 +323,107 @@
     }
 }
 
-constexpr uint32_t kAccRowF4 = 65u;
-constexpr uint32_t kAccWaveLds = 16u * kAccRowF4 * 16u;
-__global__ __launch_bounds__(256) void accumulate_kernel(const float4* __restrict__ slab, float* __restrict__ acc,
+constexpr uint32_t kAccRowW = 64u * 3u + 3u;
+constexpr uint32_t kAccWaveLds = 64u * 65u * 4u;
+__device__ __forceinline__ float texel_channel(uint32_t texel, uint32_t ch) { const f3 L = tex_unpack(texel); return ch == 1u ? L.y : (ch == 2u ? L.z : L.x); }
+
+template <uint32_t PASSES>
+__device__ __forceinline__ void accumulate_texel_rows(const char* __restrict__ slab, float* __restrict__ acc, uint32_t* lds, uint32_t tl, uint32_t tileCount, uint32_t wave, uint32_t lane,
+                                                      uint32_t x0, uint32_t y0, uint32_t W, uint32_t frames, size_t winStride)
+{
+    constexpr uint32_t G = PASSES == 1u ? 4u : (PASSES == 2u ? 2u : 1u), U = 16u * G * PASSES, rowLen = 64u * PASSES, pitch = rowLen + 1u;
+    const uint32_t pj = lane >> 2, ch = lane & 3u;
+    for (uint32_t r = 0; r < 4u; r += G) {
+        const uint32_t v = wave * 4u + r;
+        float* ap[G]; float a0[G], a[G];
+#pragma unroll
+        for (uint32_t g = 0; g < G; g++) { ap[g] = acc + ((size_t)(x0 + (size_t)(y0 + v + g) * W)) * 4u + lane; a0[g] = a[g] = *ap[g]; }
+        const char* __restrict__ base = slab + slab_texel_position(lane, tileCount, tl, v * 16u, rowLen, PASSES, 0u);
+        for (uint32_t f0 = 0; f0 < frames; f0 += 64u, base += winStride) {
+            const uint32_t S = ((frames - f0 < 64u) ? frames - f0 : 64u) * PASSES;
+            uint32_t t[U];
+#pragma unroll
+            for (uint32_t u = 0; u < U; u++) t[u] = load_texel(base, slab_texel_offset(0u, u / PASSES, PASSES, u % PASSES));
+#pragma unroll
+            for (uint32_t u = 0; u < U; u++) lds[(u / PASSES) * pitch + lane * PASSES + u % PASSES] = t[u];
+            asm volatile("s_waitcnt lgkmcnt(0)" ::: "memory");
+            const uint32_t* myT = lds + pj * pitch;
+            uint32_t s = 0;
+            for (; s + 4u <= S; s += 4u) {
+                uint32_t x[G][4];
+#pragma unroll
+                for (uint32_t g = 0; g < G; g++)
+#pragma unroll
+                    for (uint32_t k = 0; k < 4u; k++) x[g][k] = myT[g * 16u * pitch + s + k];
+#pragma unroll
+                for (uint32_t k = 0; k < 4u; k++)
+#pragma unroll
+                    for (uint32_t g = 0; g < G; g++) a[g] += texel_channel(x[g][k], ch);
+            }
+            for (; s < S; s++)
+#pragma unroll
+                for (uint32_t g = 0; g < G; g++) a[g] += texel_channel(myT[g * 16u * pitch + s], ch);
+            asm volatile("s_waitcnt lgkmcnt(0)" ::: "memory");
+        }
+#pragma unroll
+        for (uint32_t g = 0; g < G; g++) *ap[g] = ch == 3u ? a0[g] + 0.0f : a[g];
+    }
+}
+
+__global__ __launch_bounds__(256) void accumulate_kernel(const char* __restrict__ slab, float* __restrict__ acc, const uint32_t* __restrict__ tileOrder, uint32_t texelFirst,
                                                           uint32_t tileFirst, uint32_t tileStride, uint32_t tileCount, uint32_t tilesX,
                                                           uint32_t W, uint32_t frames, uint32_t passes)
 {
-    extern __shared__ float4 accLds[];
-    const uint32_t tl = blockIdx.x, lane = threadIdx.x & 63u, wave = threadIdx.x >> 6;
-    if (tl >= tileCount) return;
+    extern __shared__ float accLds[];
+    const uint32_t rank = blockIdx.x, lane = threadIdx.x & 63u, wave = threadIdx.x >> 6;
+    if (rank >= tileCount) return;
+    const uint32_t tl = tileOrder ? tileOrder[rank] : rank;
     const uint32_t tile = tileFirst + tl * tileStride;
     const uint32_t x0 = (tile % tilesX) * 16u, y0 = (tile / tilesX) * 16u;
     const uint32_t rowLen = 64u * passes;
-    const size_t winStride = (size_t)tileCount * 256u * rowLen;
-    float4* my4 = accLds + wave * (16u * kAccRowF4);
-    const float* myF = reinterpret_cast<const float*>(my4) + (lane >> 2) * (kAccRowF4 * 4u) + (lane & 3u);
+    const size_t winStride = slab_window_bytes(tileCount, passes);
+    float* myLds = accLds + wave * (kAccWaveLds / 4u);
+    if (rank >= texelFirst) {
+        uint32_t* myU = reinterpret_cast<uint32_t*>(myLds);
+        if (passes == 1u) accumulate_texel_rows<1>(slab, acc, myU, tl, tileCount, wave, lane, x0, y0, W, frames, winStride);
+        else if (passes == 2u) accumulate_texel_rows<2>(slab, acc, myU, tl, tileCount, wave, lane, x0, y0, W, frames, winStride);
+        else if (passes == 3u) accumulate_texel_rows<3>(slab, acc, myU, tl, tileCount, wave, lane, x0, y0, W, frames, winStride);
+        else accumulate_texel_rows<4>(slab, acc, myU, tl, tileCount, wave, lane, x0, y0, W, frames, winStride);
+        return;
+    }
+    const uint32_t pj = lane >> 2, ch = lane & 3u, chR = ch == 3u ? 0u : ch;
+    const float* myF = myLds + pj * kAccRowW + chR;
     for (uint32_t r = 0; r < 4u; r++) {
         const uint32_t v = wave * 4u + r;
         float* __restrict__ ap = acc + ((size_t)(x0 + (size_t)(y0 + v) * W)) * 4u + lane;
-        float a = *ap;
-        const float4* __restrict__ rowBase = slab + ((size_t)tl * 256u + v * 16u) * rowLen;
+        const float a0 = *ap;
+        float a = a0;
+        const char* __restrict__ rowBase = slab + slab_position(0u, tileCount, tl, v * 16u, rowLen, passes, 0u);
         for (uint32_t f0 = 0; f0 < frames; f0 += 64u, rowBase += winStride) {
             const uint32_t S = ((frames - f0 < 64u) ? frames - f0 : 64u) * passes;
             for (uint32_t b = 0; b < S; b += 64u) {
                 const uint32_t n = (S - b < 64u) ? S - b : 64u;
-                float4 t[16];
+                Sample3 t[16];
                 if (lane < n) {
 #pragma unroll
-                    for (int j = 0; j < 16; j++) t[j] = rowBase[(size_t)j * rowLen + b + lane];
-#pragma unroll
-                    for (int j = 0; j < 16; j++) my4[j * kAccRowF4 + lane] = t[j];
+                    for (uint32_t j = 0; j < 16u; j++) t[j] = load_sample(rowBase, slab_row_offset(j, rowLen, b + lane));
+#pragma unroll
+                    for (uint32_t j = 0; j < 16u; j++) { float* d = myLds + j * kAccRowW + lane * 3u; d[0] = t[j].x; d[1] = t[j].y; d[2] = t[j].z; }
                 }
                 asm volatile("s_waitcnt lgkmcnt(0)" ::: "memory");
                 uint32_t s = 0;
                 for (; s + 8u <= n; s += 8u) {
                     float x[8];
 #pragma unroll
-                    for (int k = 0; k < 8; k++) x[k] = myF[(s + k) * 4u];
+                    for (int k = 0; k < 8; k++) x[k] = myF[(s + k) * 3u];
 #pragma unroll
                     for (int k = 0; k < 8; k++) a += x[k];
                 }
-                for (; s < n; s++) a += myF[s * 4u];
+                for (; s < n; s++) a += myF[s * 3u];
                 asm volatile("s_waitcnt lgkmcnt(0)" ::: "memory");
             }
         }
-        *ap = a;
+        *ap = ch == 3u ? a0 + 0.0f : a;
     }
 }
 
@@ -891,7 +947,7 @@
     tileSums[tile] = sum;
 }
 
-__global__ __launch_bounds__(256) void commit_frame_kernel(const float4* __restrict__ slabWindow, uint32_t frameInWindow, uint32_t passes,
+__global__ __launch_bounds__(256) void commit_frame_kernel(const char* __restrict__ slabWindow, uint32_t frameInWindow, uint32_t passes,
                                                             float4* __restrict__ acc, uint32_t* __restrict__ pixels, float* __restrict__ tileSums,
                                                             uint32_t tileFirst, uint32_t tileStride, uint32_t tileCount, uint32_t tilesX,
                                                             uint32_t W, float scale)
@@ -902,9 +958,10 @@
     const uint32_t tile = tileFirst + tl * tileStride;
     const uint32_t x0 = (tile % tilesX) * 16u, y0 = (tile / tilesX) * 16u;
     const size_t i = (x0 + (pix & 15u)) + (size_t)(y0 + (pix >> 4)) * W;
-    const float4* __restrict__ s = slabWindow + ((size_t)tl * 256u + pix) * (64u * passes) + frameInWindow * passes;
+    const size_t at = slab_position(frameInWindow, tileCount, tl, pix, 64u * passes, passes, 0u);
     float4 a = acc[i];
-    for (uint32_t p = 0; p < passes; p++) { const float4 t = s[p]; a.x += t.x; a.y += t.y; a.z += t.z; a.w += t.w; }
+    for (uint32_t p = 0; p < passes; p++) { const Sample3 t = load_sample(slabWindow, at + p * kSampleBytes); a.x += t.x; a.y += t.y; a.z += t.z; }
+    a.w += 0.0f;
     acc[i] = a;
     const float px = a.x * scale, py = a.y * scale, pz = a.z * scale;
     tileE[pix] = px + py + pz;
@@ -974,7 +1031,7 @@
     if (blockDesc && (tileCount > 0x10000u || windows > 64u)) return hipErrorInvalidValue;
     if (rankCount == 0u || rankCount > tileCount) rankCount = tileCount;
     dim3 grid(blockDesc ? nBlocks : rankCount * windows), block(64);
-#define CRT_LAUNCH(K, C) hipLaunchKernelGGL((crt::render_tiles_kernel<K, C>), grid, block, ldsBytes + 15u * 64u * 4u , stream, *sc, (float4*)slab, counters, tileClocks, tileOrder, tileFirst, tileStride, tileCount, tilesX, sppFirst, frames, passes, windows, blockDesc, tileCost, rankCount, launchClk)
+#define CRT_LAUNCH(K, C) hipLaunchKernelGGL((crt::render_tiles_kernel<K, C>), grid, block, ldsBytes + 15u * 64u * 4u , stream, *sc, (char*)slab, counters, tileClocks, tileOrder, tileFirst, tileStride, tileCount, tilesX, sppFirst, frames, passes, windows, blockDesc, tileCost, rankCount, launchClk)
     if (sc->kind == 0) { if (collectStats) CRT_LAUNCH(0, true); else CRT_LAUNCH(0, false); }
     else { if (collectStats) CRT_LAUNCH(1, true); else CRT_LAUNCH(1, false); }
 #undef CRT_LAUNCH
@@ -991,12 +1048,27 @@
     return (uint32_t)perCu * (uint32_t)cus;
 }
 
-extern "C" hipError_t crt_launch_accumulate(const void* slab, void* acc, uint32_t tileFirst, uint32_t tileStride, uint32_t tileCount,
+extern "C" size_t crt_slab_window_bytes(uint32_t tileCount, uint32_t passes) { return crt::slab_window_bytes(tileCount, passes); }
+
+extern "C" void crt_slab_layout_probe(int texel, uint32_t frames, uint32_t tileCount, uint32_t passes, unsigned long long* pos, unsigned long long* sizes)
+{
+    for (uint32_t fr = 0; fr < frames; fr++)
+        for (uint32_t tl = 0; tl < tileCount; tl++)
+            for (uint32_t pix = 0; pix < 256u; pix++)
+                for (uint32_t pass = 0; pass < passes; pass++)
+                    *pos++ = texel ? crt::slab_texel_position(fr, tileCount, tl, pix, 64u * passes, passes, pass) : crt::slab_position(fr, tileCount, tl, pix, 64u * passes, passes, pass);
+    sizes[0] = crt::slab_window_bytes(tileCount, passes);
+    sizes[1] = crt::slab_tile_bytes(passes);
+}
+
+extern "C" hipError_t crt_launch_accumulate(const void* slab, void* acc, const uint32_t* tileOrder, uint32_t texelFirst, uint32_t tileFirst, uint32_t tileStride, uint32_t tileCount,
                                             uint32_t tilesX, uint32_t W, uint32_t frames, uint32_t passes, hipStream_t stream)
 {
     if (tileCount == 0 || frames == 0) return hipSuccess;
+    if (passes < 1u || passes > 4u || (texelFirst < tileCount && !tileOrder)) return hipErrorInvalidValue;
     dim3 grid(tileCount), block(256);
-    hipLaunchKernelGGL(crt::accumulate_kernel, grid, block, 4u * crt::kAccWaveLds, stream, (const float4*)slab, (float*)acc, tileFirst, tileStride, tileCount, tilesX, W, frames, passes);
+    hipLaunchKernelGGL(crt::accumulate_kernel, grid, block, 4u * crt::kAccWaveLds, stream, (const char*)slab, (float*)acc, tileOrder, texelFirst, tileFirst, tileStride, tileCount, tilesX, W, frames,
+                       passes);
     return hipGetLastError();
 }
 
@@ -1093,7 +1165,7 @@
 {
     if (tileCount == 0) return hipSuccess;
     if (frameInWindow >= 64u || passes < 1u || passes > 4u) return hipErrorInvalidValue;
-    hipLaunchKernelGGL(crt::commit_frame_kernel, dim3(tileCount), dim3(256), 0, stream, (const float4*)slabWindow, frameInWindow, passes, (float4*)acc, pixels, tileSums,
+    hipLaunchKernelGGL(crt::commit_frame_kernel, dim3(tileCount), dim3(256), 0, stream, (const char*)slabWindow, frameInWindow, passes, (float4*)acc, pixels, tileSums,
                        tileFirst, tileStride, tileCount, tilesX, W, scale);
     return hipGetLastError();
 }
diff --git a/cpu-ray-tracer_amd/csrc/device/launch.h b/cpu-ray-tracer_amd/csrc/device/launch.h
--- a/cpu-ray-tracer_amd/csrc/device/launch.h
+++ b/cpu-ray-tracer_amd/csrc/device/launch.h
@@ -11,8 +11,11 @@
     uint32_t tileCount, uint32_t tilesX, uint32_t sppFirst, uint32_t frames, uint32_t passes, uint32_t ldsBytes, int collectStats, const uint32_t* blockDesc, uint32_t nBlocks, uint32_t* tileCost,
     uint32_t rankCount, unsigned long long* launchClk, hipStream_t stream);
 uint32_t crt_render_resident_waves(int device, int kind, uint32_t ldsBytes);
-hipError_t crt_launch_accumulate(const void* slab, void* acc, uint32_t tileFirst, uint32_t tileStride, uint32_t tileCount, uint32_t tilesX, uint32_t W, uint32_t frames, uint32_t passes,
-    hipStream_t stream);
+size_t crt_slab_window_bytes(uint32_t tileCount, uint32_t passes);
+hipError_t crt_launch_accumulate(const void* slab, void* acc, const uint32_t* tileOrder ,
+    uint32_t texelFirst , uint32_t tileFirst, uint32_t tileStride, uint32_t tileCount,
+    uint32_t tilesX, uint32_t W, uint32_t frames, uint32_t passes, hipStream_t stream);
+void crt_slab_layout_probe(int texel, uint32_t frames, uint32_t tileCount, uint32_t passes, unsigned long long* pos, unsigned long long* sizes);
 hipError_t crt_launch_find_nearest(const crt::Scene* sc, const void* rays, void* hits, uint32_t n, crt::Counters* counters, uint32_t ldsBytes, uint32_t* cursor, hipStream_t stream);
 hipError_t crt_launch_is_occluded(const crt::Scene* sc, const void* rays, int32_t* occluded, uint32_t n, uint32_t ldsBytes, uint32_t* cursor, hipStream_t stream);
 hipError_t crt_launch_whitted(const crt::Scene* sc, int accel, const crt::AltAccelDev* alt, const crt::TlasAltDev* tl, void* acc, uint32_t* pixels, crt::Counters* counters, uint32_t ldsBytes,
@@ -41,6 +44,7 @@
 
 hipError_t crt_launch_render_sky(const crt::Scene* sc, void* slab, crt::Counters* counters, const uint32_t* tileOrder, uint32_t rankFirst, uint32_t skyTiles, uint32_t tileFirst,
     uint32_t tileStride, uint32_t tileCount , uint32_t tilesX, uint32_t sppFirst, uint32_t frames, uint32_t passes,
+    int texels ,
     unsigned long long* launchClk , hipStream_t stream);
 
 uint32_t crt_probe_paths(void);
diff --git a/cpu-ray-tracer_amd/csrc/device/render_pool.hip b/cpu-ray-tracer_amd/csrc/device/render_pool.hip
--- a/cpu-ray-tracer_amd/csrc/device/render_pool.hip
+++ b/cpu-ray-tracer_amd/csrc/device/render_pool.hip
@@ -71,7 +71,7 @@
 __device__ __forceinline__ uint32_t rank_in(uint64_t m) { return __builtin_amdgcn_mbcnt_hi((uint32_t)(m >> 32), __builtin_amdgcn_mbcnt_lo((uint32_t)m, 0u)); }
 
 template <int KIND, bool COUNT, int S, int REFBITS = 16>
-__global__ __launch_bounds__(64, REFBITS == 32 ? CRT_POOL_WIDE_MIN_WAVES : CRT_POOL_MIN_WAVES) void render_pool_kernel(const Scene sc, float4* __restrict__ slab, float* __restrict__ facScratch, Counters* __restrict__ counters,
+__global__ __launch_bounds__(64, REFBITS == 32 ? CRT_POOL_WIDE_MIN_WAVES : CRT_POOL_MIN_WAVES) void render_pool_kernel(const Scene sc, char* __restrict__ slab, float* __restrict__ facScratch, Counters* __restrict__ counters,
                                                              unsigned long long* __restrict__ tileClocks, const uint32_t* __restrict__ tileOrder,
                                                              uint32_t tileFirst, uint32_t tileStride, uint32_t tileCount, uint32_t tilesX,
                                                              uint32_t sppFirst, uint32_t frames, uint32_t passes, uint32_t groups, uint32_t waveFrames, const uint32_t* __restrict__ waveTab, uint32_t tabBlocks, uint32_t longFrames,
@@ -479,7 +479,7 @@
                         for (int k = 4; k >= 0; k--)
                             if (depth > k) L = mk3(fk[3 * k], fk[3 * k + 1], fk[3 * k + 2]) * L;
                     }
-                    slab[sampleAt] = make_float4(L.x, L.y, L.z, 0.0f);
+                    store_sample(slab, sampleAt, L);
                 }
 #ifdef CRT_POOL_STAMPS
                 { CRT_PSTAMP(e3); CRT_PACC(4, e2, e3); pst[10]++; }
@@ -647,7 +647,7 @@
     const uint32_t ldsBytes = crt_pool_lds_bytes(sc->stackDepth, S, sc->poolRefBits) + extraLds;
     { int dev = 0; if (hipGetDevice(&dev) != hipSuccess) return hipGetLastError(); if (ldsBytes > crt_pool_lds_limit(dev)) return hipErrorInvalidValue; }
 #define CRT_LAUNCH(K, C, SS) do { if (sc->poolRefBits == 32u) CRT_LAUNCH_R(K, C, SS, 32); else CRT_LAUNCH_R(K, C, SS, 16); } while (0)
-#define CRT_LAUNCH_R(K, C, SS, RB) hipLaunchKernelGGL((crt::render_pool_kernel<K, C, SS, RB>), grid, block, ldsBytes, stream, *sc, (float4*)slab, (float*)facScratch, counters, tileClocks, tileOrder, tileFirst, tileStride, tileCount, tilesX, sppFirst, frames, passes, groups, wf, waveTab, tabBlocks, longFrames, rankFirst, tileCost, launchClk, tileClass)
+#define CRT_LAUNCH_R(K, C, SS, RB) hipLaunchKernelGGL((crt::render_pool_kernel<K, C, SS, RB>), grid, block, ldsBytes, stream, *sc, (char*)slab, (float*)facScratch, counters, tileClocks, tileOrder, tileFirst, tileStride, tileCount, tilesX, sppFirst, frames, passes, groups, wf, waveTab, tabBlocks, longFrames, rankFirst, tileCost, launchClk, tileClass)
 #define CRT_LAUNCH_S(K, C) do { if (S == 64u) CRT_LAUNCH(K, C, 64); else CRT_LAUNCH(K, C, CRT_POOL_STREAMS); } while (0)
     if (sc->kind == 0) { if (collectStats) CRT_LAUNCH_S(0, true); else CRT_LAUNCH_S(0, false); }
     else { if (collectStats) CRT_LAUNCH_S(1, true); else CRT_LAUNCH_S(1, false); }
diff --git a/cpu-ray-tracer_amd/csrc/device/render_seq.hip b/cpu-ray-tracer_amd/csrc/device/render_seq.hip
--- a/cpu-ray-tracer_amd/csrc/device/render_seq.hip
+++ b/cpu-ray-tracer_amd/csrc/device/render_seq.hip
@@ -65,8 +65,8 @@
     dim3 grid((nProbe + crt::kSeqWaves - 1u) / crt::kSeqWaves), block(64u * crt::kSeqWaves);
     const uint32_t ldsBytes = crt::seq_lds_bytes(sc->stackDepth);
     if (hipMemsetAsync(tileCost, 0, (size_t)tileCount * 4, stream) != hipSuccess) return hipGetLastError();
-    if (sc->kind == 0) hipLaunchKernelGGL((crt::render_seq_kernel<crt::BvhWorld<0>, true>), grid, block, ldsBytes, stream, *sc, crt::BvhWorld<0>{}, (float4*)nullptr, (crt::Counters*)nullptr, tileFirst, tileStride, tileCount, tilesX, 1u, 64u, 1u, nProbe, tileCost);
-    else hipLaunchKernelGGL((crt::render_seq_kernel<crt::BvhWorld<1>, true>), grid, block, ldsBytes, stream, *sc, crt::BvhWorld<1>{}, (float4*)nullptr, (crt::Counters*)nullptr, tileFirst, tileStride, tileCount, tilesX, 1u, 64u, 1u, nProbe, tileCost);
+    if (sc->kind == 0) hipLaunchKernelGGL((crt::render_seq_kernel<crt::BvhWorld<0>, true>), grid, block, ldsBytes, stream, *sc, crt::BvhWorld<0>{}, (char*)nullptr, (crt::Counters*)nullptr, tileFirst, tileStride, tileCount, tilesX, 1u, 64u, 1u, nProbe, tileCost);
+    else hipLaunchKernelGGL((crt::render_seq_kernel<crt::BvhWorld<1>, true>), grid, block, ldsBytes, stream, *sc, crt::BvhWorld<1>{}, (char*)nullptr, (crt::Counters*)nullptr, tileFirst, tileStride, tileCount, tilesX, 1u, 64u, 1u, nProbe, tileCost);
     return hipGetLastError();
 }
 
diff --git a/cpu-ray-tracer_amd/csrc/device/render_sky.hip b/cpu-ray-tracer_amd/csrc/device/render_sky.hip
--- a/cpu-ray-tracer_amd/csrc/device/render_sky.hip
+++ b/cpu-ray-tracer_amd/csrc/device/render_sky.hip
@@ -3,9 +3,9 @@
 
 namespace crt {
 
-__global__ __launch_bounds__(64) void render_sky_kernel(const Scene sc, float4* __restrict__ slab, Counters* __restrict__ counters, const uint32_t* __restrict__ tileOrder,
+__global__ __launch_bounds__(64) void render_sky_kernel(const Scene sc, char* __restrict__ slab, Counters* __restrict__ counters, const uint32_t* __restrict__ tileOrder,
                                                         uint32_t rankFirst, uint32_t skyTiles, uint32_t tileFirst, uint32_t tileStride, uint32_t tileCount, uint32_t tilesX,
-                                                        uint32_t sppFirst, uint32_t frames, uint32_t passes, uint32_t groups, unsigned long long* __restrict__ launchClk)
+                                                        uint32_t sppFirst, uint32_t frames, uint32_t passes, uint32_t groups, uint32_t texels, unsigned long long* __restrict__ launchClk)
 {
     const uint32_t lane = threadIdx.x;
     const uint32_t r = blockIdx.x / groups, grp = blockIdx.x - r * groups;
@@ -27,8 +27,9 @@
             const f3 v = primary_target(camPos, TL, right, down, sc.invW, sc.invH, tx, ty, pix, seed);
             const f3 D = v * rcp_exact(sqrt_exact(dot3(v, v)));
             float phi, theta; sky_angles(D, phi, theta);
-            const f3 L = tex_unpack(sc.texels[tex_index(sc.skyOffset, sc.skyW, sc.skyH, phi * CRT_INV2PI, theta * CRT_INVPI)]);
-            slab[slab_position(fr, tileCount, tl, pix, rowLen, passes, pass)] = make_float4(L.x, L.y, L.z, 0.0f);
+            const uint32_t texel = sc.texels[tex_index(sc.skyOffset, sc.skyW, sc.skyH, phi * CRT_INV2PI, theta * CRT_INVPI)];
+            if (texels) store_texel(slab, slab_texel_position(fr, tileCount, tl, pix, rowLen, passes, pass), texel);
+            else store_sample(slab, slab_position(fr, tileCount, tl, pix, rowLen, passes, pass), tex_unpack(texel));
             if (++pass == passes) { pass = 0; pix++; }
         }
         paths = items;
@@ -42,13 +43,13 @@
 
 extern "C" hipError_t crt_launch_render_sky(const crt::Scene* sc, void* slab, crt::Counters* counters, const uint32_t* tileOrder, uint32_t rankFirst, uint32_t skyTiles,
                                             uint32_t tileFirst, uint32_t tileStride, uint32_t tileCount, uint32_t tilesX, uint32_t sppFirst, uint32_t frames, uint32_t passes,
-                                            unsigned long long* launchClk, hipStream_t stream)
+                                            int texels, unsigned long long* launchClk, hipStream_t stream)
 {
     if (skyTiles == 0 || frames == 0) return hipSuccess;
     if (!tileOrder || rankFirst > tileCount || skyTiles > tileCount - rankFirst || passes == 0) return hipErrorInvalidValue;
     const uint32_t groups = (frames + 63u) / 64u;
     if ((unsigned long long)skyTiles * groups > 0x7fffffffull) return hipErrorInvalidValue;
-    hipLaunchKernelGGL(crt::render_sky_kernel, dim3(skyTiles * groups), dim3(64), 0, stream, *sc, (float4*)slab, counters, tileOrder, rankFirst, skyTiles, tileFirst, tileStride,
-                       tileCount, tilesX, sppFirst, frames, passes, groups, launchClk);
+    hipLaunchKernelGGL(crt::render_sky_kernel, dim3(skyTiles * groups), dim3(64), 0, stream, *sc, (char*)slab, counters, tileOrder, rankFirst, skyTiles, tileFirst, tileStride,
+                       tileCount, tilesX, sppFirst, frames, passes, groups, texels ? 1u : 0u, launchClk);
     return hipGetLastError();
 }
diff --git a/cpu-ray-tracer_amd/csrc/device/sample_body.h b/cpu-ray-tracer_amd/csrc/device/sample_body.h
--- a/cpu-ray-tracer_amd/csrc/device/sample_body.h
+++ b/cpu-ray-tracer_amd/csrc/device/sample_body.h
@@ -108,10 +108,36 @@
 {
     return init_seed(tx + ty * W + (sppFirst + frame * passes) * 1799u);
 }
-__device__ __forceinline__ size_t slab_position(uint32_t fr, uint32_t tileCount, uint32_t tl, uint32_t pix, uint32_t rowLen, uint32_t passes, uint32_t pass)
+
+constexpr uint32_t kSampleBytes = 12u, kTexelBytes = 4u;
+struct Sample3 { float x, y, z; };
+__host__ __device__ __forceinline__ size_t slab_tile_bytes(uint32_t passes) { return (size_t)(256u * 64u * kSampleBytes) * passes; }
+__host__ __device__ __forceinline__ size_t slab_window_bytes(uint32_t tileCount, uint32_t passes) { return (size_t)tileCount * slab_tile_bytes(passes); }
+__host__ __device__ __forceinline__ size_t slab_block_position(uint32_t window, uint32_t tileCount, uint32_t tl, uint32_t rowLen)
 {
-    return (((size_t)(fr >> 6) * tileCount + tl) * 256u + pix) * rowLen + ((fr & 63u) * passes + pass);
+    return ((size_t)window * tileCount + tl) * (256u * kSampleBytes) * rowLen;
 }
+__host__ __device__ __forceinline__ uint32_t slab_row_offset(uint32_t pix, uint32_t rowLen, uint32_t sampleInRow) { return (pix * rowLen + sampleInRow) * kSampleBytes; }
+__host__ __device__ __forceinline__ uint32_t slab_sample_offset(uint32_t frameInWindow, uint32_t pix, uint32_t rowLen, uint32_t passes, uint32_t pass)
+{
+    return slab_row_offset(pix, rowLen, frameInWindow * passes + pass);
+}
+__host__ __device__ __forceinline__ uint32_t slab_texel_offset(uint32_t frameInWindow, uint32_t pix, uint32_t passes, uint32_t pass)
+{
+    return ((pix * passes + pass) * 64u + frameInWindow) * kTexelBytes;
+}
+__host__ __device__ __forceinline__ size_t slab_position(uint32_t fr, uint32_t tileCount, uint32_t tl, uint32_t pix, uint32_t rowLen, uint32_t passes, uint32_t pass)
+{
+    return slab_block_position(fr >> 6, tileCount, tl, rowLen) + slab_sample_offset(fr & 63u, pix, rowLen, passes, pass);
+}
+__host__ __device__ __forceinline__ size_t slab_texel_position(uint32_t fr, uint32_t tileCount, uint32_t tl, uint32_t pix, uint32_t rowLen, uint32_t passes, uint32_t pass)
+{
+    return slab_block_position(fr >> 6, tileCount, tl, rowLen) + slab_texel_offset(fr & 63u, pix, passes, pass);
+}
+__device__ __forceinline__ void store_sample(char* __restrict__ slab, size_t at, f3 L) { Sample3 s; s.x = L.x; s.y = L.y; s.z = L.z; *reinterpret_cast<Sample3*>(slab + at) = s; }
+__device__ __forceinline__ Sample3 load_sample(const char* __restrict__ slab, size_t at) { return *reinterpret_cast<const Sample3*>(slab + at); }
+__device__ __forceinline__ void store_texel(char* __restrict__ slab, size_t at, uint32_t texel) { *reinterpret_cast<uint32_t*>(slab + at) = texel; }
+__device__ __forceinline__ uint32_t load_texel(const char* __restrict__ slab, size_t at) { return *reinterpret_cast<const uint32_t*>(slab + at); }
 __device__ __forceinline__ f3 primary_target(f3 camPos, f3 TL, f3 right, f3 down, float invW, float invH, uint32_t tx, uint32_t ty, uint32_t pix, uint32_t& seed)
 {
     const int x = (int)(tx * 16u + (pix & 15u)), y = (int)(ty * 16u + (pix >> 4));
diff --git a/cpu-ray-tracer_amd/csrc/device/seq_sample.h b/cpu-ray-tracer_amd/csrc/device/seq_sample.h
--- a/cpu-ray-tracer_amd/csrc/device/seq_sample.h
+++ b/cpu-ray-tracer_amd/csrc/device/seq_sample.h
@@ -38,7 +38,7 @@
 }
 
 template <class World, bool PROBE>
-__global__ __launch_bounds__(256, 4) void render_seq_kernel(const Scene sc, const World world, float4* __restrict__ slab, Counters* __restrict__ counters,
+__global__ __launch_bounds__(256, 4) void render_seq_kernel(const Scene sc, const World world, char* __restrict__ slab, Counters* __restrict__ counters,
                                                            uint32_t tileFirst, uint32_t tileStride, uint32_t tileCount, uint32_t tilesX,
                                                            uint32_t sppFirst, uint32_t frames, uint32_t passes, uint32_t nEntries, uint32_t* __restrict__ tileCost)
 {
@@ -52,7 +52,7 @@
     sppFirst += win * 64u * passes;
     frames = (frames - win * 64u < 64u) ? frames - win * 64u : 64u;
     if (lane >= frames) return;
-    slab += (size_t)win * ((size_t)tileCount * 256u * 64u * passes);
+    if (!PROBE) slab += slab_block_position(win, tileCount, tl, 64u * passes);
     const uint32_t tile = tileFirst + tl * tileStride;
     const uint32_t tx = tile % tilesX, ty = tile / tilesX;
     const uint32_t stackWords = world.stack_words(sc);
@@ -82,7 +82,7 @@
         if (!PROBE) {
             uint32_t pass = 0;
             if (passes != 1u) pass = item - pix * passes;
-            slab[((size_t)tl * 256u + pix) * (64u * passes) + (lane * passes + pass)] = make_float4(L.x, L.y, L.z, 0.0f);
+            store_sample(slab, slab_sample_offset(lane, pix, 64u * passes, passes, pass), L);
         } else if (L.x != L.x) steps++;
     }
     if (PROBE) { const uint32_t sum = wave_sum(steps); if (lane == 0) atomicAdd(&tileCost[tl], sum); return; }
@@ -97,7 +97,7 @@
 {
     const uint32_t entries = tileCount * ((frames + 63u) / 64u);
     hipLaunchKernelGGL((render_seq_kernel<World, false>), dim3((entries + kSeqWaves - 1u) / kSeqWaves), dim3(64u * kSeqWaves), seq_lds_bytes(world.stack_words(*sc)), stream,
-                       *sc, world, (float4*)slab, counters, tileFirst, tileStride, tileCount, tilesX, sppFirst, frames, passes, entries, (uint32_t*)nullptr);
+                       *sc, world, (char*)slab, counters, tileFirst, tileStride, tileCount, tilesX, sppFirst, frames, passes, entries, (uint32_t*)nullptr);
     return hipGetLastError();
 }
 
```

New measurement: 34030 Mrays/s, median of 6. +2.7%, better.
